# uber-research/UPSNet

Hardware: NVIDIA H100
Metric: panoptic images/sec at 1024x2048 (higher is better)
Workload: dtype bf16x3

## Files before the change

### include/upsnet_b200.h

```cpp
#ifndef UPSNET_B200_H_
#define UPSNET_B200_H_

#include <stddef.h>
#include <stdint.h>

#ifdef __cplusplus
extern "C" {
#endif

#define UPSNET_E_BADARG (-1)
#define UPSNET_E_UNSUPPORTED (-2)
#define UPSNET_E_WORKSPACE (-3)

#define UPSNET_LAYOUT_NCHW 0
#define UPSNET_LAYOUT_NHWC 1
#define UPSNET_LAYOUT_FLAT_PAIR 2

#define UPSNET_DTYPE_F32 0
#define UPSNET_DTYPE_BF16 1
#define UPSNET_DTYPE_PAIR 2

#define UPSNET_EPI_RELU 1
#define UPSNET_EPI_RES_UP2 2
#define UPSNET_EPI_STEM_PAIR 8
#define UPSNET_EPI_NO_TMA 4
#define UPSNET_EPI_PAIR_GROUP(G) ((((G) / 64) & 0xfff) << 8)
#define UPSNET_EPI_SIGMOID_FROM(c) ((((c) + 1) & 0x3ff) << 20)

#define UPSNET_PREC_FP32_SIMT 0
#define UPSNET_PREC_BF16X3 1
#define UPSNET_PREC_BF16 2

int upsnet_version(int *n_sm);

int upsnet_roi_align_forward(const void *feat, int B, int C, int H, int W, int layout, int dtype,
                             const float *rois, int R, int PH, int PW, int sampling_ratio,
                             float spatial_scale, void *out, void *stream);

int upsnet_roi_align_fpn_forward(const void *const feats[4], const int Hs[4], const int Ws[4],
                                 const float scales[4], int B, int C, int layout, int dtype,
                                 const float *rois, int R, int PH, int PW, int sampling_ratio,
                                 void *out, int *levels_out, void *stream);

int upsnet_nms_workspace_bytes(int S, int max_seg_len, size_t *bytes);
int upsnet_nms_segmented(const float *boxes, const int *seg_offsets, int S, int max_seg_len,
                         float thresh, int *keep_out, int *keep_cnt, void *workspace,
                         size_t workspace_bytes, void *stream);
int upsnet_nms_host(int *keep_out, int *num_out, const float *boxes_host, int boxes_num,
                    int boxes_dim, float thresh, int device_id);

int upsnet_dcn_forward(const float *x, const float *offset, const float *mask,
                       const float *weight, const float *bias, float *y, int N, int Cin, int H,
                       int W, int Cout, int kh, int kw, int stride_h, int stride_w, int pad_h,
                       int pad_w, int dil_h, int dil_w, int deformable_groups, int epi_flags,
                       int precision, void *stream);

int upsnet_conv2d_forward(const float *x, const float *weight, const float *bias,
                          const float *residual, float *y, int N, int Cin, int H, int W,
                          int Cout, int kh, int kw, int stride_h, int stride_w, int pad_h,
                          int pad_w, int dil_h, int dil_w, int epi_flags, int precision,
                          void *stream);

int upsnet_igemm_packed_weight_bytes(int Cout, int Cin, int kh, int kw, size_t *bytes);
int upsnet_igemm_pack_weight(const float *weight, int Cout, int Cin, int kh, int kw, void *packed,
                             void *stream);
int upsnet_igemm_forward(const void *x_nhwc, const float *offset, const float *mask,
                         const void *packed, const float *bias, const void *residual, void *y,
                         int N, int H, int W, int Cin, int Cout, int kh, int kw, int stride_h,
                         int stride_w, int pad_h, int pad_w, int dil_h, int dil_w, int out_layout,
                         int x_dtype, int y_dtype, int epi_flags, int precision, void *stream);
int upsnet_tma_set_tile_n(int bn);

int upsnet_dcn_packed_weight_bytes(int Cout, int Cin, int kh, int kw, size_t *bytes);
int upsnet_dcn_pack_weight(const float *weight, int Cout, int Cin, int kh, int kw, void *packed, void *stream);
int upsnet_dcn_pair_forward(const void *x_pair, const float *offset, const float *mask, const void *packed,
                            const float *bias, void *y_pair, int N, int H, int W, int Cin, int Cout, int kh, int kw,
                            int pad_h, int pad_w, int dil_h, int dil_w, int epi_flags, void *stream);
int upsnet_dcn_set_tile_n(int bn);

int upsnet_panoptic_workspace_bytes(int n, int H, int W, int num_thing, size_t *bytes);
int upsnet_panoptic_workspace_min_bytes(int n, int H, int W, int num_thing, size_t *bytes);
int upsnet_panoptic_head(const float *fcn, int S, int H, int W, const float *boxes,
                         const float *cls_prob, const float *mask_logit, const int64_t *cls_idx,
                         int n, const int *n_dev, int num_stuff, double fraction_threshold, int64_t *keep_out,
                         int *k_out, int64_t *labels, int64_t *sem_labels, void *workspace,
                         size_t workspace_bytes, void *stream);
int upsnet_panoptic_head_up4(const float *score, int S, int Hs, int Ws, const float *boxes,
                             const float *cls_prob, const float *mask_logit, const int64_t *cls_idx,
                             int n, const int *n_dev, int num_stuff, double fraction_threshold, int64_t *keep_out,
                             int *k_out, int64_t *labels, int64_t *sem_labels, void *workspace,
                             size_t workspace_bytes, void *stream);

int upsnet_mask_removal(const float *boxes, const float *cls_prob, const float *mask_logit,
                        const int64_t *cls_idx, int n, const int *n_dev, int H, int W, int num_thing,
                        double fraction_threshold, int64_t *keep_out, int *k_out, float *mask_energy,
                        void *workspace, size_t workspace_bytes, void *stream);

int upsnet_stem_workspace_bytes(int N, int H, int W, int kh, int kw, int pad, size_t *bytes);
int upsnet_stem_packed_weight_bytes(int Cout, int kh, size_t *bytes);
int upsnet_stem_pack_weight(const float *weight, int Cout, int Cin, int kh, int kw, void *packed,
                            void *stream);
int upsnet_stem_forward(const float *x, const void *packed_w, const float *bias, void *y, int N, int Cin,
                        int H, int W, int Cout, int kh, int kw, int pad, int epi_flags, void *workspace,
                        size_t workspace_bytes, void *stream);

int upsnet_maxpool2d_nhwc(const void *x, void *y, int N, int H, int W, int C, int k, int stride,
                          int pad, int dtype, void *stream);

int upsnet_upsample_bilinear_nchw(const float *x, float *y, int planes, int H, int W, int factor,
                                  void *stream);

int upsnet_fcn_score_fuse(const float *s2, const float *s3, const float *s4, const float *s5, float *out,
                          int planes, int H, int W, void *stream);

int upsnet_rpn_decode(const float *const *deltas, const long long *const *top_idx, const int *k,
                      const int *hs, const int *ws, const int *strides, const double *base_anchors,
                      int L, int A, float im_h, float im_w, float *boxes_out, void *stream);

int upsnet_rpn_topk_workspace_bytes(int L, size_t *bytes);
int upsnet_rpn_topk(const float *const *probs, const int *hs, const int *ws, int L, int A,
                    int pre_nms_top_n, float *out_scores, long long *out_idx, void *workspace,
                    size_t workspace_bytes, void *stream);

int upsnet_rpn_collect(const int *keep, const int *keep_cnt, const int *seg_offsets, const float *boxes,
                       const float *scores, int S, int max_seg_len, int post_nms_top_n, float *rois,
                       float *out_scores, unsigned char *valid, void *stream);

int upsnet_maskroi_prepare(const float *rois, const unsigned char *roi_valid, const float *bbox_delta,
                           const float *cls_prob, int R, int C, int class_agnostic, float score_thresh,
                           const float weights[4], float im_h, float im_w, float *sc_out, int *cls_out,
                           float *bx_out, int *offs_out, void *stream);

int upsnet_maskroi_finish(const int *keep, const int *keep_cnt, const int *seg_offsets, const float *sc,
                          const int *cls, const float *bx, int nseg, int max_seg_len, int top_n, int cap,
                          float *out_sc, float *out_bx, long long *out_cls, int *n_out, void *stream);

int upsnet_unified_pan_workspace_bytes(int num_seg_classes, size_t *bytes);
int upsnet_unified_pan_result(const long long *seg, const long long *pan, const long long *cls_inds, int k,
                              const int *k_dev, int H, int W, int num_seg_classes, int num_classes,
                              int stuff_area_limit, unsigned char *pan_2ch, int *err_out, void *workspace,
                              size_t workspace_bytes, void *stream);

int upsnet_prep_image(const unsigned char *image_hwc, int h, int w, double scale, int out_h, int out_w, int pad_h,
                      int pad_w, const double pixel_means[3], float *blob, void *stream);

int upsnet_label_restore(const long long *src0, const long long *src1, int Hp, int Wp, int h, int w, double fx,
                         int out_h, int out_w, long long *dst0, long long *dst1, void *stream);

#define UPSNET_PQ_MAX_GT 4096
#define UPSNET_PQ_MAX_PAIRS 65536
#define UPSNET_PQ_MAX_PRED 2048
#define UPSNET_PQ_E_PRED_CATEGORY 1
#define UPSNET_PQ_E_GT_COUNT 2
#define UPSNET_PQ_E_PAIRS 4
#define UPSNET_PQ_E_GT_TABLE 8
#define UPSNET_PQ_E_PRED_COUNT 16
#define UPSNET_PQ_E_MATCHES 32
int upsnet_pq_workspace_bytes(size_t *bytes);
int upsnet_pq_update(const unsigned char *pan_2ch, const unsigned char *gt_rgb, int H, int W, const long long *gt_table,
                     int num_gt, const unsigned char *cat_flags, long long *acc_counts, double *acc_iou, int *err,
                     void *workspace, size_t workspace_bytes, void *stream);

#define UPSNET_SSEG_MAX_CLASSES 224
int upsnet_sseg_update(const void *pred, int pred_bytes, int pred_pitch, const int *row_src, const int *col_src,
                       const unsigned char *gt, int H, int W, int num_classes, long long *acc, void *stream);

#define UPSNET_COCOEVAL_MAX_DET 2048
#define UPSNET_COCOEVAL_MAX_GT 1024
#define UPSNET_COCOEVAL_MAX_GT_CAT 192
#define UPSNET_COCOEVAL_MAX_CATEGORIES 256
#define UPSNET_COCOEVAL_MAX_IMAGES (1 << 17)
#define UPSNET_COCOEVAL_E_DET_COUNT 1
#define UPSNET_COCOEVAL_E_GT_COUNT 2
#define UPSNET_COCOEVAL_E_GT_CAT 4
#define UPSNET_COCOEVAL_E_CLASS 8
#define UPSNET_COCOEVAL_E_RECORDS 16
#define UPSNET_COCOEVAL_E_RLE_SIZE 32
typedef struct {
  float score;
  int category;
  int image;
  int rank;
  unsigned long long matched, ignored;
} upsnet_coco_record;
int upsnet_cocoeval_workspace_bytes(int n, int cap, long long gt_counts_total, size_t *bytes);
int upsnet_cocoeval_image(int segm, const float *boxes, const float *scores, const int64_t *cls_inds, int n,
                          const int *n_dev, const uint32_t *counts, int cap, const int *run_len, int H, int W,
                          const double *gt_table, int num_gt, const uint32_t *gt_counts, const int64_t *gt_offsets,
                          int num_categories, const int *class_to_k, int image_slot, upsnet_coco_record *records,
                          int record_cap, int *n_records, long long *npig, int *err, void *workspace,
                          size_t workspace_bytes, void *stream);
int upsnet_cocoeval_accumulate_workspace_bytes(int n_records, size_t *bytes);
int upsnet_cocoeval_accumulate(const upsnet_coco_record *records, int n_records, const int *image_rank,
                               const long long *npig, int num_categories, double *precision, double *recall,
                               double *scores, void *workspace, size_t workspace_bytes, void *stream);

#define UPSNET_COMBINED_MAX_DET 2048
#define UPSNET_COMBINED_E_RUN_LEN 1
#define UPSNET_COMBINED_E_RLE_SIZE 2
#define UPSNET_COMBINED_E_DET_COUNT 4
int upsnet_combined_pan_workspace_bytes(int n, int H, int W, size_t *bytes);
int upsnet_combined_pan_result(const void *sem, int sem_elem_size, int H, int W, const float *scores,
                               const int64_t *cls_inds, int n, const int *n_dev, const uint32_t *counts, int cap,
                               const int *run_len, int num_seg_classes, int num_classes, float score_threshold,
                               float fraction_threshold, int stuff_area_limit, unsigned char *pan_2ch, int *err,
                               void *workspace, size_t workspace_bytes, void *stream);

int upsnet_im_post_workspace_bytes(int n, int cap, size_t *bytes);
int upsnet_im_post_rle(const float *mask_probs, int C, int M, const float *boxes, const int64_t *cls_inds, int n,
                       const int *n_dev, int H, int W, uint32_t *counts, int cap, int *run_len, int *overflow,
                       void *workspace, size_t workspace_bytes, void *stream);

int upsnet_dcn_im2col(const float *x, const float *offset, const float *mask, int Cin, int H, int W, int kh, int kw,
                      int stride_h, int stride_w, int pad_h, int pad_w, int dil_h, int dil_w, float *col, void *stream);
int upsnet_dcn_col2im(const float *dcol, const float *offset, const float *mask, int Cin, int H, int W, int kh, int kw,
                      int stride_h, int stride_w, int pad_h, int pad_w, int dil_h, int dil_w, float *dx, void *stream);
int upsnet_dcn_col2im_coord(const float *dcol, const float *x, const float *offset, const float *mask, int Cin, int H,
                            int W, int kh, int kw, int stride_h, int stride_w, int pad_h, int pad_w, int dil_h, int dil_w,
                            float *doffset, float *dmask, void *stream);

int upsnet_roi_align_backward(const float *dout, const float *rois, int R, int B, int C, int H, int W, int PH, int PW,
                              int sampling_ratio, float spatial_scale, float *dfeat, void *stream);

#ifdef __cplusplus
}
#endif
#endif
```

### upsnet_b200/_lib.py

```python
import ctypes as C
import os

import torch

_HERE = os.path.dirname(os.path.abspath(__file__))
LIB_PATH = os.path.join(_HERE, "libupsnet_b200.so")
_lib = None

LAYOUT_NCHW, LAYOUT_NHWC = 0, 1
EPI_RELU = 1
EPI_RES_UP2 = 2
EPI_NO_TMA = 4
EPI_STEM_PAIR = 8


def EPI_SIGMOID_FROM(c):
    return ((int(c) + 1) & 0x3ff) << 20
PREC_FP32_SIMT, PREC_BF16X3, PREC_BF16 = 0, 1, 2
DTYPE_F32, DTYPE_BF16, DTYPE_PAIR = 0, 1, 2
LAYOUT_FLAT_PAIR = 2

_ERR = {-1: "bad argument", -2: "unsupported configuration", -3: "workspace too small"}


class UpsnetError(RuntimeError):
    pass


def lib():
    global _lib
    if _lib is None:
        if not os.path.exists(LIB_PATH):
            from . import build as _build
            _build.build()
        L = C.CDLL(LIB_PATH)
        vp, i, f, d, sz = C.c_void_p, C.c_int, C.c_float, C.c_double, C.c_size_t
        L.upsnet_version.argtypes = [C.POINTER(i)]
        L.upsnet_roi_align_forward.argtypes = [vp, i, i, i, i, i, i, vp, i, i, i, i, f, vp, vp]
        L.upsnet_roi_align_fpn_forward.argtypes = [C.POINTER(vp), C.POINTER(i), C.POINTER(i), C.POINTER(f),
                                                   i, i, i, i, vp, i, i, i, i, vp, vp, vp]
        L.upsnet_nms_workspace_bytes.argtypes = [i, i, C.POINTER(sz)]
        L.upsnet_nms_segmented.argtypes = [vp, vp, i, i, f, vp, vp, vp, sz, vp]
        L.upsnet_nms_host.argtypes = [vp, vp, vp, i, i, f, i]
        L.upsnet_dcn_forward.argtypes = [vp] * 6 + [i] * 16 + [vp]
        L.upsnet_conv2d_forward.argtypes = [vp] * 5 + [i] * 15 + [vp]
        L.upsnet_igemm_packed_weight_bytes.argtypes = [i, i, i, i, C.POINTER(sz)]
        L.upsnet_igemm_pack_weight.argtypes = [vp, i, i, i, i, vp, vp]
        L.upsnet_igemm_forward.argtypes = [vp] * 7 + [i] * 18 + [vp]
        L.upsnet_dcn_packed_weight_bytes.argtypes = [i, i, i, i, C.POINTER(sz)]
        L.upsnet_dcn_pack_weight.argtypes = [vp, i, i, i, i, vp, vp]
        L.upsnet_dcn_pair_forward.argtypes = [vp] * 6 + [i] * 12 + [vp]
        L.upsnet_dcn_set_tile_n.argtypes = [i]
        L.upsnet_tma_set_tile_n.argtypes = [i]
        L.upsnet_panoptic_workspace_bytes.argtypes = [i, i, i, i, C.POINTER(sz)]
        L.upsnet_panoptic_workspace_min_bytes.argtypes = [i, i, i, i, C.POINTER(sz)]
        L.upsnet_panoptic_head.argtypes = [vp, i, i, i, vp, vp, vp, vp, i, vp, i, d, vp, vp, vp, vp, vp, sz, vp]
        L.upsnet_panoptic_head_up4.argtypes = [vp, i, i, i, vp, vp, vp, vp, i, vp, i, d, vp, vp, vp, vp, vp, sz, vp]
        L.upsnet_mask_removal.argtypes = [vp, vp, vp, vp, i, vp, i, i, i, d, vp, vp, vp, vp, sz, vp]
        L.upsnet_rpn_decode.argtypes = [C.POINTER(vp), C.POINTER(vp), C.POINTER(i), C.POINTER(i), C.POINTER(i),
                                        C.POINTER(i), vp, i, i, f, f, vp, vp]
        L.upsnet_maskroi_prepare.argtypes = [vp, vp, vp, vp, i, i, i, f, C.POINTER(f), f, f, vp, vp, vp, vp, vp]
        L.upsnet_maskroi_finish.argtypes = [vp] * 6 + [i] * 4 + [vp] * 5
        L.upsnet_maxpool2d_nhwc.argtypes = [vp, vp] + [i] * 8 + [vp]
        L.upsnet_upsample_bilinear_nchw.argtypes = [vp, vp, i, i, i, i, vp]
        L.upsnet_rpn_topk_workspace_bytes.argtypes = [i, C.POINTER(sz)]
        L.upsnet_stem_workspace_bytes.argtypes = [i] * 6 + [C.POINTER(sz)]
        L.upsnet_stem_packed_weight_bytes.argtypes = [i, i, C.POINTER(sz)]
        L.upsnet_stem_pack_weight.argtypes = [vp, i, i, i, i, vp, vp]
        L.upsnet_stem_forward.argtypes = [vp] * 4 + [i] * 9 + [vp, sz, vp]
        L.upsnet_rpn_collect.argtypes = [vp] * 5 + [i] * 3 + [vp] * 4
        L.upsnet_rpn_topk.argtypes = [C.POINTER(vp), C.POINTER(i), C.POINTER(i), i, i, i, vp, vp, vp, sz, vp]
        L.upsnet_dcn_im2col.argtypes = [vp, vp, vp] + [i] * 11 + [vp, vp]
        L.upsnet_dcn_col2im.argtypes = [vp, vp, vp] + [i] * 11 + [vp, vp]
        L.upsnet_dcn_col2im_coord.argtypes = [vp, vp, vp, vp] + [i] * 11 + [vp, vp, vp]
        L.upsnet_roi_align_backward.argtypes = [vp, vp] + [i] * 8 + [f, vp, vp]
        L.upsnet_fcn_score_fuse.argtypes = [vp, vp, vp, vp, vp, i, i, i, vp]
        L.upsnet_unified_pan_workspace_bytes.argtypes = [i, C.POINTER(sz)]
        L.upsnet_unified_pan_result.argtypes = [vp, vp, vp, i, vp, i, i, i, i, i, vp, vp, vp, sz, vp]
        L.upsnet_im_post_workspace_bytes.argtypes = [i, i, C.POINTER(sz)]
        L.upsnet_im_post_rle.argtypes = [vp, i, i, vp, vp, i, vp, i, i, vp, i, vp, vp, vp, sz, vp]
        L.upsnet_prep_image.argtypes = [vp, i, i, d, i, i, i, i, C.POINTER(d), vp, vp]
        L.upsnet_label_restore.argtypes = [vp, vp, i, i, i, i, d, i, i, vp, vp, vp]
        L.upsnet_pq_workspace_bytes.argtypes = [C.POINTER(sz)]
        L.upsnet_pq_update.argtypes = [vp, vp, i, i, vp, i, vp, vp, vp, vp, vp, sz, vp]
        L.upsnet_sseg_update.argtypes = [vp, i, i, vp, vp, vp, i, i, i, vp, vp]
        L.upsnet_cocoeval_workspace_bytes.argtypes = [i, i, C.c_longlong, C.POINTER(sz)]
        L.upsnet_cocoeval_image.argtypes = [i, vp, vp, vp, i, vp, vp, i, vp, i, i, vp, i, vp, vp, i, vp, i, vp, i, vp, vp,
                                            vp, vp, sz, vp]
        L.upsnet_cocoeval_accumulate_workspace_bytes.argtypes = [i, C.POINTER(sz)]
        L.upsnet_cocoeval_accumulate.argtypes = [vp, i, vp, vp, i, vp, vp, vp, vp, sz, vp]
        L.upsnet_combined_pan_workspace_bytes.argtypes = [i, i, i, C.POINTER(sz)]
        L.upsnet_combined_pan_result.argtypes = [vp, i, i, i, vp, vp, i, vp, vp, i, vp, i, i, f, f, i, vp, vp, vp, sz, vp]
        _lib = L
    return _lib


EXPORTED_SYMBOLS = [
    "upsnet_version", "upsnet_roi_align_forward", "upsnet_roi_align_fpn_forward",
    "upsnet_nms_workspace_bytes", "upsnet_nms_segmented", "upsnet_nms_host", "upsnet_dcn_forward",
    "upsnet_conv2d_forward", "upsnet_igemm_packed_weight_bytes", "upsnet_igemm_pack_weight",
    "upsnet_igemm_forward", "upsnet_panoptic_workspace_bytes", "upsnet_panoptic_workspace_min_bytes", "upsnet_panoptic_head", "upsnet_panoptic_head_up4", "upsnet_mask_removal",
    "upsnet_rpn_decode", "upsnet_maskroi_prepare", "upsnet_maskroi_finish", "upsnet_maxpool2d_nhwc", "upsnet_upsample_bilinear_nchw", "upsnet_rpn_topk_workspace_bytes", "upsnet_rpn_topk", "upsnet_rpn_collect", "upsnet_stem_workspace_bytes",
    "upsnet_stem_packed_weight_bytes", "upsnet_stem_pack_weight", "upsnet_stem_forward",
    "upsnet_dcn_im2col", "upsnet_dcn_col2im", "upsnet_dcn_col2im_coord", "upsnet_roi_align_backward",
    "upsnet_dcn_packed_weight_bytes", "upsnet_dcn_pack_weight", "upsnet_dcn_pair_forward", "upsnet_dcn_set_tile_n", "upsnet_tma_set_tile_n",
    "upsnet_fcn_score_fuse", "upsnet_unified_pan_workspace_bytes", "upsnet_unified_pan_result", "upsnet_prep_image", "upsnet_im_post_workspace_bytes", "upsnet_im_post_rle",
    "upsnet_label_restore", "upsnet_pq_workspace_bytes", "upsnet_pq_update",
    "upsnet_sseg_update", "upsnet_cocoeval_workspace_bytes", "upsnet_cocoeval_image",
    "upsnet_cocoeval_accumulate_workspace_bytes", "upsnet_cocoeval_accumulate",
    "upsnet_combined_pan_workspace_bytes", "upsnet_combined_pan_result",
]


def check(rc, what):
    if rc == 0:
        return
    if rc < 0:
        raise UpsnetError("%s: %s (%d)" % (what, _ERR.get(rc, "error"), rc))
    raise UpsnetError("%s: CUDA error %d" % (what, rc))


def stream_ptr(device=None):
    return C.c_void_p(torch.cuda.current_stream(device).cuda_stream)


def ptr(t):
    return C.c_void_p(t.data_ptr()) if t is not None else C.c_void_p(None)


def require_cuda(*tensors):
    for t in tensors:
        if t is not None and not t.is_cuda:
            raise UpsnetError("upsnet_b200 ops are CUDA-only (sm_90a); got a %s tensor" % t.device)


def f32c(t):
    if t.dtype != torch.float32:
        t = t.float()
    return t.contiguous()
```

### upsnet_b200/csrc/capi.cu

```cuda
#include "common.cuh"
#include "tc_params.cuh"

namespace ups {
struct ConvParams {
  const float* x; const float* offset; const float* mask; const float* weight;
  const float* bias; const float* residual; float* y;
  int N, Cin, H, W, Cout, kh, kw, sh, sw, ph, pw, dh, dw, dg, Ho, Wo, relu;
};
int launch_igemm_simt(const ConvParams& p, cudaStream_t stream);

}

extern "C" int upsnet_version(int* n_sm) {
  if (n_sm) {
    int dev = 0, sms = 0;
    if (cudaGetDevice(&dev) == cudaSuccess &&
        cudaDeviceGetAttribute(&sms, cudaDevAttrMultiProcessorCount, dev) == cudaSuccess)
      *n_sm = sms;
    else
      *n_sm = -1;
  }
  return 90;
}

static int conv_common(const float* x, const float* offset, const float* mask, const float* weight,
                       const float* bias, const float* residual, float* y, int N, int Cin, int H,
                       int W, int Cout, int kh, int kw, int sh, int sw, int ph, int pw, int dh,
                       int dw, int dg, int epi_flags, int precision, void* stream) {
  if (!x || !weight || !y) return UPSNET_E_BADARG;
  if (N <= 0 || Cin <= 0 || H <= 0 || W <= 0 || Cout <= 0 || kh <= 0 || kw <= 0 || sh <= 0 ||
      sw <= 0 || ph < 0 || pw < 0 || dh <= 0 || dw <= 0 || dg <= 0 || Cin % dg != 0)
    return UPSNET_E_BADARG;
  ups::ConvParams p;
  p.x = x; p.offset = offset; p.mask = mask; p.weight = weight; p.bias = bias;
  p.residual = residual; p.y = y;
  p.N = N; p.Cin = Cin; p.H = H; p.W = W; p.Cout = Cout; p.kh = kh; p.kw = kw; p.sh = sh;
  p.sw = sw; p.ph = ph; p.pw = pw; p.dh = dh; p.dw = dw; p.dg = dg;
  p.Ho = ups::conv_out_size(H, ph, dh, kh, sh);
  p.Wo = ups::conv_out_size(W, pw, dw, kw, sw);
  p.relu = (epi_flags & UPSNET_EPI_RELU) ? 1 : 0;
  if (p.Ho <= 0 || p.Wo <= 0) return UPSNET_E_BADARG;
  if ((size_t)Cin * H * W >= (1ull << 31)) return UPSNET_E_UNSUPPORTED;
  switch (precision) {
    case UPSNET_PREC_FP32_SIMT:
      return ups::launch_igemm_simt(p, (cudaStream_t)stream);
    default:
      return UPSNET_E_UNSUPPORTED;
  }
}

extern "C" int upsnet_dcn_forward(const float* x, const float* offset, const float* mask,
                                  const float* weight, const float* bias, float* y, int N, int Cin,
                                  int H, int W, int Cout, int kh, int kw, int stride_h,
                                  int stride_w, int pad_h, int pad_w, int dil_h, int dil_w,
                                  int deformable_groups, int epi_flags, int precision,
                                  void* stream) {
  if (!offset) return UPSNET_E_BADARG;
  return conv_common(x, offset, mask, weight, bias, nullptr, y, N, Cin, H, W, Cout, kh, kw,
                     stride_h, stride_w, pad_h, pad_w, dil_h, dil_w, deformable_groups, epi_flags,
                     precision, stream);
}

extern "C" int upsnet_conv2d_forward(const float* x, const float* weight, const float* bias,
                                     const float* residual, float* y, int N, int Cin, int H, int W,
                                     int Cout, int kh, int kw, int stride_h, int stride_w,
                                     int pad_h, int pad_w, int dil_h, int dil_w, int epi_flags,
                                     int precision, void* stream) {
  return conv_common(x, nullptr, nullptr, weight, bias, residual, y, N, Cin, H, W, Cout, kh, kw,
                     stride_h, stride_w, pad_h, pad_w, dil_h, dil_w, 1, epi_flags, precision,
                     stream);
}

extern "C" int upsnet_igemm_packed_weight_bytes(int Cout, int Cin, int kh, int kw, size_t* bytes) {
  if (!bytes || Cout <= 0 || Cin <= 0 || kh <= 0 || kw <= 0) return UPSNET_E_BADARG;
  if (!ups::tc_supported(Cin, kh, kw, 1)) return UPSNET_E_UNSUPPORTED;
  *bytes = ups::tc_packed_weight_bytes(Cout, Cin, kh, kw);
  return 0;
}

extern "C" int upsnet_igemm_pack_weight(const float* weight, int Cout, int Cin, int kh, int kw,
                                        void* packed, void* stream) {
  if (!weight || !packed || Cout <= 0 || Cin <= 0 || kh <= 0 || kw <= 0) return UPSNET_E_BADARG;
  if (!ups::tc_supported(Cin, kh, kw, 1)) return UPSNET_E_UNSUPPORTED;
  return ups::tc_pack_weight(weight, Cout, Cin, kh, kw, packed, (cudaStream_t)stream);
}

extern "C" int upsnet_igemm_forward(const void* x_nhwc, const float* offset, const float* mask,
                                    const void* packed, const float* bias, const void* residual,
                                    void* y, int N, int H, int W, int Cin, int Cout, int kh, int kw,
                                    int stride_h, int stride_w, int pad_h, int pad_w, int dil_h,
                                    int dil_w, int out_layout, int x_dtype, int y_dtype, int epi_flags,
                                    int precision, void* stream) {
  if (!x_nhwc || !packed || !y) return UPSNET_E_BADARG;
  if (N <= 0 || Cin <= 0 || H <= 0 || W <= 0 || Cout <= 0 || kh <= 0 || kw <= 0 || stride_h <= 0 ||
      stride_w <= 0 || pad_h < 0 || pad_w < 0 || dil_h <= 0 || dil_w <= 0)
    return UPSNET_E_BADARG;
  if (precision != UPSNET_PREC_BF16X3 && precision != UPSNET_PREC_BF16) return UPSNET_E_BADARG;
  if (out_layout != UPSNET_LAYOUT_NCHW && out_layout != UPSNET_LAYOUT_NHWC) return UPSNET_E_BADARG;
  if (mask && !offset) return UPSNET_E_BADARG;
  if ((size_t)H * W >= (1ull << 31)) return UPSNET_E_UNSUPPORTED;
  ups::TcParams p{};
  p.x = x_nhwc; p.offset = offset; p.mask = mask; p.bias = bias; p.residual = residual; p.y = y;
  p.N = N; p.H = H; p.W = W; p.Cin = Cin; p.Cout = Cout; p.kh = kh; p.kw = kw; p.sh = stride_h;
  p.sw = stride_w; p.ph = pad_h; p.pw = pad_w; p.dh = dil_h; p.dw = dil_w;
  p.Ho = ups::conv_out_size(H, pad_h, dil_h, kh, stride_h);
  p.Wo = ups::conv_out_size(W, pad_w, dil_w, kw, stride_w);
  if (p.Ho <= 0 || p.Wo <= 0) return UPSNET_E_BADARG;
  p.relu = (epi_flags & UPSNET_EPI_RELU) ? 1 : 0;
  p.out_nhwc = out_layout == UPSNET_LAYOUT_NHWC;
  p.res_up2 = (epi_flags & UPSNET_EPI_RES_UP2) ? 1 : 0;
  p.no_tma = (epi_flags & UPSNET_EPI_NO_TMA) ? 1 : 0;
  if (p.res_up2 && (!residual || !p.out_nhwc || (p.Ho & 1) || (p.Wo & 1))) return UPSNET_E_BADARG;
  p.x3 = precision == UPSNET_PREC_BF16X3;
  if (x_dtype < UPSNET_DTYPE_F32 || x_dtype > UPSNET_DTYPE_PAIR || y_dtype < UPSNET_DTYPE_F32 || y_dtype > UPSNET_DTYPE_PAIR)
    return UPSNET_E_BADARG;
  p.x_bf16 = x_dtype == UPSNET_DTYPE_BF16;
  p.y_bf16 = y_dtype == UPSNET_DTYPE_BF16;
  p.x_pair = x_dtype == UPSNET_DTYPE_PAIR;
  p.y_pair = y_dtype == UPSNET_DTYPE_PAIR;
  p.pair_group = 64 * ((epi_flags >> 8) & 0xfff);
  p.sig_from = ((epi_flags >> 20) & 0x3ff) - 1;
  if (p.sig_from >= 0 && (p.y_pair || p.y_bf16 || p.residual)) return UPSNET_E_UNSUPPORTED;
  if (p.x_bf16 && p.x3) return UPSNET_E_UNSUPPORTED;
  if ((p.x_pair || p.y_pair) && !p.x3) return UPSNET_E_UNSUPPORTED;
  if (p.y_pair && !p.out_nhwc) return UPSNET_E_BADARG;
  return ups::launch_igemm_tc(p, packed, (cudaStream_t)stream);
}
```

### upsnet_b200/csrc/detection.cu

```cuda
#include <cfloat>

#include "common.cuh"

namespace ups {

__device__ __forceinline__ float4 decode_clip(float x1, float y1, float x2, float y2, float dx, float dy, float dw, float dh,
                                              float xform_clip, float im_h, float im_w) {
  const float w = __fadd_rn(__fsub_rn(x2, x1), 1.0f), h = __fadd_rn(__fsub_rn(y2, y1), 1.0f);
  const float cx = __fadd_rn(x1, __fmul_rn(0.5f, w)), cy = __fadd_rn(y1, __fmul_rn(0.5f, h));
  dw = fminf(dw, xform_clip);
  dh = fminf(dh, xform_clip);
  const float pcx = __fadd_rn(__fmul_rn(dx, w), cx), pcy = __fadd_rn(__fmul_rn(dy, h), cy);
  const float pw = __fmul_rn(expf(dw), w), ph = __fmul_rn(expf(dh), h);
  float4 o;
  o.x = __fsub_rn(pcx, __fmul_rn(0.5f, pw));
  o.y = __fsub_rn(pcy, __fmul_rn(0.5f, ph));
  o.z = __fsub_rn(__fadd_rn(pcx, __fmul_rn(0.5f, pw)), 1.0f);
  o.w = __fsub_rn(__fadd_rn(pcy, __fmul_rn(0.5f, ph)), 1.0f);
  const float mx = __fsub_rn(im_w, 1.0f), my = __fsub_rn(im_h, 1.0f);
  o.x = fminf(fmaxf(o.x, 0.f), mx);
  o.y = fminf(fmaxf(o.y, 0.f), my);
  o.z = fminf(fmaxf(o.z, 0.f), mx);
  o.w = fminf(fmaxf(o.w, 0.f), my);
  return o;
// ... 473 lines not shown
    acc += p.lv[l].k;
    if (p.lv[l].blocks > max_blocks) max_blocks = p.lv[l].blocks;
  }
  cudaStream_t st = (cudaStream_t)stream;
  UPS_CUDA(cudaMemsetAsync(p.hist, 0, (size_t)L * kTkBins * 4, st));
  UPS_CUDA(cudaMemsetAsync(p.ticket, 0, (size_t)L * 4 * 4, st));
  const dim3 grid((unsigned)max_blocks, (unsigned)L);
  const int shifts[5] = {43, 32, 22, 11, 0}, nbits[5] = {11, 11, 10, 11, 11};
  for (int ps = 0; ps < 5; ++ps) {
    topk_pass_kernel<<<grid, kTkThreads, 0, st>>>(p, shifts[ps], nbits[ps], ps == 0 ? 1 : 0);
    UPS_CHECK_LAUNCH();
  }
  topk_gather_kernel<<<grid, kTkThreads, 0, st>>>(p);
  UPS_CHECK_LAUNCH();
  topk_sort_kernel<<<L, 1024, 0, st>>>(p);
  UPS_CHECK_LAUNCH();
  return 0;
}

namespace ups {

constexpr int kColMaxCand = 8192, kColMaxPost = 2048, kColBins = 4096;

__global__ void __launch_bounds__(1024, 1)
rpn_collect_kernel(const int* __restrict__ keep, const int* __restrict__ cnt, const int* __restrict__ offs,
                   const float* __restrict__ boxes, const float* __restrict__ scores, int S, int max_len, int post,
                   float* __restrict__ rois, float* __restrict__ out_scores, unsigned char* __restrict__ ok) {
  extern __shared__ unsigned long long ck[];
  unsigned long long* sel = ck + kColMaxCand;
  __shared__ unsigned int hist[kColBins];
  __shared__ int seg_base[kMaxLevels + 1];
  __shared__ unsigned long long s_prefix;
  __shared__ int s_need, s_nsel;
  const int tid = threadIdx.x;
  if (tid == 0) {
    int acc = 0;
    for (int s = 0; s < S; ++s) { seg_base[s] = acc; acc += min(min(max(cnt[s], 0), max_len), post); }
    seg_base[S] = min(acc, kColMaxCand);
    s_nsel = 0;
  }
  __syncthreads();
  const int C = seg_base[S];
  for (int s = 0; s < S; ++s) {
    const int b = seg_base[s], n = min(seg_base[s + 1], kColMaxCand) - b, o = offs[s];
    for (int j = tid; j < n; j += 1024) {
      const int g = keep[(size_t)s * max_len + j] + o;
      ck[b + j] = ((unsigned long long)orderable(scores[g]) << 13) | (unsigned long long)(8191 - (b + j));
    }
  }
  __syncthreads();
  unsigned long long kth = 0ull;
  if (C > post) {
    if (tid == 0) { s_prefix = 0ull; s_need = post; }
    __syncthreads();
    for (int pass = 0; pass < 4; ++pass) {
      const int shift = 36 - 12 * pass;
      const unsigned long long mask_hi = pass == 0 ? 0ull : (~0ull << (shift + 12));
      for (int b = tid; b < kColBins; b += 1024) hist[b] = 0;
      __syncthreads();
      const unsigned long long pref = s_prefix;
      for (int i = tid; i < C; i += 1024)
        if ((ck[i] & mask_hi) == pref) atomicAdd(&hist[(unsigned int)(ck[i] >> shift) & (kColBins - 1)], 1u);
      __syncthreads();
      if (tid < 32) {
        const int need = s_need, per = kColBins / 32;
        unsigned int mine = 0;
        for (int b = 0; b < per; ++b) mine += hist[kColBins - 1 - (tid * per + b)];
        unsigned int incl = mine;
#pragma unroll
        for (int o = 1; o < 32; o <<= 1) {
          const unsigned int y = __shfl_up_sync(0xffffffffu, incl, o);
          if (tid >= o) incl += y;
        }
        const unsigned int excl = incl - mine;
        if (excl < (unsigned int)need && incl >= (unsigned int)need) {
          unsigned int acc = excl;
          int d = 0;
          for (int b = 0; b < per; ++b) {
            const int bin = kColBins - 1 - (tid * per + b);
            if (acc + hist[bin] >= (unsigned int)need) { d = bin; break; }
            acc += hist[bin];
          }
          s_need = need - (int)acc;
          s_prefix = pref | ((unsigned long long)d << shift);
        }
      }
      __syncthreads();
    }
    kth = s_prefix;
  }
  for (int i = tid; i < C; i += 1024)
    if (ck[i] >= kth) {
      const int pos = atomicAdd(&s_nsel, 1);
      if (pos < kColMaxPost) sel[pos] = ck[i];
    }
  __syncthreads();
  const int nsel = min(s_nsel, min(post, kColMaxPost));
  int sortN = 64;
  while (sortN < nsel) sortN <<= 1;
  for (int i = nsel + tid; i < sortN; i += 1024) sel[i] = 0ull;
  __syncthreads();
  for (int k = 2; k <= sortN; k <<= 1)
    for (int j = k >> 1; j > 0; j >>= 1) {
      for (int t = tid; t < sortN / 2; t += 1024) {
        const int lo = ((t / j) * (j << 1)) + (t % j), hi = lo + j;
        const unsigned long long a = sel[lo], b = sel[hi];
        const bool desc = (lo & k) == 0;
        if ((a < b) == desc) { sel[lo] = b; sel[hi] = a; }
      }
      __syncthreads();
    }
  for (int i = tid; i < post; i += 1024) {
    float4 bx = make_float4(0.f, 0.f, 0.f, 0.f);
    float sc = 0.f;
    unsigned char live = 0;
    if (i < nsel) {
      const int fp = 8191 - (int)(sel[i] & 8191ull);
      int s = 0;
      while (s + 1 < S && fp >= seg_base[s + 1]) ++s;
      const int g = keep[(size_t)s * max_len + (fp - seg_base[s])] + offs[s];
      bx = reinterpret_cast<const float4*>(boxes)[g];
      sc = scores[g];
      live = 1;
    }
    rois[(size_t)i * 5] = 0.f;
    rois[(size_t)i * 5 + 1] = bx.x; rois[(size_t)i * 5 + 2] = bx.y;
    rois[(size_t)i * 5 + 3] = bx.z; rois[(size_t)i * 5 + 4] = bx.w;
    out_scores[i] = sc;
    ok[i] = live;
  }
}

}

extern "C" int upsnet_rpn_collect(const int* keep, const int* keep_cnt, const int* seg_offsets, const float* boxes,
                                  const float* scores, int S, int max_seg_len, int post_nms_top_n, float* rois,
                                  float* out_scores, unsigned char* valid, void* stream) {
  using namespace ups;
  if (!keep || !keep_cnt || !seg_offsets || !boxes || !scores || !rois || !out_scores || !valid) return UPSNET_E_BADARG;
  if (S <= 0 || S > kMaxLevels || max_seg_len <= 0 || post_nms_top_n <= 0) return UPSNET_E_BADARG;
  if (post_nms_top_n > kColMaxPost || (long long)S * (max_seg_len < post_nms_top_n ? max_seg_len : post_nms_top_n) > kColMaxCand)
    return UPSNET_E_UNSUPPORTED;
  if (((uintptr_t)boxes) & 15) return UPSNET_E_BADARG;
  const size_t smem = (size_t)(kColMaxCand + kColMaxPost) * 8;
  static ups::PerDeviceOnce configured;
  if (configured.need()) {
    UPS_CUDA(cudaFuncSetAttribute(rpn_collect_kernel, cudaFuncAttributeMaxDynamicSharedMemorySize, (int)smem));
  }
  rpn_collect_kernel<<<1, 1024, smem, (cudaStream_t)stream>>>(keep, keep_cnt, seg_offsets, boxes, scores, S, max_seg_len,
                                                               post_nms_top_n, rois, out_scores, valid);
  UPS_CHECK_LAUNCH();
  return 0;
}
```

### upsnet_b200/csrc/igemm_tma.cu

```cuda
#include <cuda.h>
#include <cuda_bf16.h>
#include <cstdlib>

#include "common.cuh"
#include "tc_ptx.cuh"
#include "tc_params.cuh"

namespace ups {

constexpr int TM_EPI_WARPS = 8;
constexpr int TM_WARP_TMA = 8, TM_WARP_RES = 9;
constexpr int TM_THREADS = 10 * 32;
constexpr int TM_MAX_STAGES = 8;
constexpr int TM_SLAB_BYTES = 128 * 128;
constexpr int TM_MMA_BF16 = 0, TM_MMA_WIDE = 1;

struct TmaGeom {
  const float* bias;
  int N, Ho, Wo, Cout, Cin;
  int kw, KHW, ph, pw, dh, dw;
  int bw, bh, bn;
  int tiles_w, tiles_h, tiles_n, n_tiles;
  int BN, stages, relu, has_res;
  int res_up2;
  int direct, y_bf16, out_nhwc;
  void* y;
  int stem;
  int sig_from;
  int x3;
  int x_lo;
  int w_lo;
  int pg;
  int res_inplace;
  int opairs;
  int wide;
};

__device__ __forceinline__ int pair_chan(int n, int G) { return (n / G) * 2 * G + (n % G); }

struct TmaSmem {
  uint32_t stages, out, res, acc, a_bytes, b_bytes, stage_bytes, total;
  uint32_t a_half, b_half;
  uint32_t oslabs, res_slab;
};
template <int N, int W>
__device__ __forceinline__ void acc_stage_sw(const float (&d)[N / 2], float* buf, int row0) {
  const int t = threadIdx.x & 127, l = t & 31;
  const int r = row0 + 16 * (t >> 5) + (l >> 2);
#pragma unroll
  for (int i = 0; i < W / 8; ++i) {
    const int c = 8 * i + 2 * (l & 3);
#pragma unroll
    for (int h = 0; h < 2; ++h) {
      const int rr = r + 8 * h;
      const int pc = ((((c >> 2) ^ (rr & 7))) << 2) | (c & 3);
      *reinterpret_cast<float2*>(buf + (size_t)rr * W + pc) = make_float2(d[4 * i + 2 * h], d[4 * i + 2 * h + 1]);
    }
  }
}
__device__ __forceinline__ void acc_ld16_sw(uint32_t rowaddr, int row, int col, uint32_t (&r)[16]) {
#pragma unroll
  for (int i = 0; i < 4; ++i) {
    const uint32_t a = rowaddr + ((uint32_t)(((col >> 2) + i) ^ (row & 7)) << 4);
    asm volatile("ld.shared.v4.b32 {%0, %1, %2, %3}, [%4];"
                 : "=r"(r[4 * i]), "=r"(r[4 * i + 1]), "=r"(r[4 * i + 2]), "=r"(r[4 * i + 3]) : "r"(a));
  }
}
__host__ __device__ inline TmaSmem tma_smem_layout(int BN, int stages, bool has_res, bool direct, bool x3, bool res_up2,
                                                  bool res_inplace, int opairs) {
  TmaSmem s;
  const uint32_t mul = x3 ? 2u : 1u;
  s.a_half = 128 * 128; s.b_half = (uint32_t)BN * 128;
  s.a_bytes = s.a_half * mul;
  s.b_bytes = s.b_half * mul;
  s.stage_bytes = s.a_bytes + s.b_bytes;
  s.stages = 1024;
  s.out = s.stages + s.stage_bytes * (uint32_t)stages;
  s.res_slab = (x3 && res_up2) ? 4096u : (uint32_t)TM_SLAB_BYTES;
  if (x3) {
    s.oslabs = direct ? 0u : (res_inplace ? 2u * (uint32_t)(BN / 64) : (uint32_t)opairs);
    s.res = s.out + s.oslabs * 2u * TM_SLAB_BYTES;
    s.acc = s.res + ((has_res && !res_inplace) ? 2u * (uint32_t)(BN / 64) * 2u * s.res_slab : 0u);
  } else {
    s.oslabs = 0;
    const uint32_t out_slabs = direct ? 0 : (BN == 64 ? 1 : 2);
    s.res = s.out + out_slabs * TM_SLAB_BYTES;
    s.acc = s.res + (has_res ? 2u * (uint32_t)(BN / 64) * TM_SLAB_BYTES : 0u);
  }
  s.total = s.acc + ((x3 && !direct) ? 0u : 128u * (uint32_t)BN * 4u);
  return s;
}

template <int N, int MMA>
__global__ void __launch_bounds__(TM_THREADS, 1)
igemm_tma_kernel(const __grid_constant__ CUtensorMap tm_x, const __grid_constant__ CUtensorMap tm_w,
                 const __grid_constant__ CUtensorMap tm_y, const __grid_constant__ CUtensorMap tm_r, const TmaGeom g) {
  extern __shared__ __align__(1024) uint8_t smem_dyn[];
  const uint32_t raw = smem_u32(smem_dyn);
  const uint32_t base = (raw + 1023u) & ~1023u;
  uint8_t* sm = smem_dyn + (base - raw);
  const TmaSmem L = tma_smem_layout(g.BN, g.stages, g.has_res != 0, g.direct != 0, g.x3 != 0, g.res_up2 != 0, g.res_inplace != 0,
                                    g.opairs);
  const uint32_t bar_full = base, bar_empty = base + 8 * TM_MAX_STAGES;
  const uint32_t bar_rfull = bar_empty + 8 * TM_MAX_STAGES, bar_rempty = bar_rfull + 16;

  const int tid = threadIdx.x, warp = tid >> 5, lane = tid & 31;
  const int cchunks = g.Cin / 64;
  const int num_kb = g.KHW * cchunks;
  const long long m_tiles = (long long)g.tiles_w * g.tiles_h * g.tiles_n;
  const long long num_tiles = m_tiles * g.n_tiles;
  const uint32_t box_bytes = (uint32_t)(g.bw * g.bh * g.bn) * 128u;

  if (tid == 0) {
    for (int s = 0; s < g.stages; ++s) {
      mbar_init(bar_full + 8 * s, 1);
      mbar_init(bar_empty + 8 * s, TM_EPI_WARPS);
    }
    for (int b = 0; b < 2; ++b) {
      mbar_init(bar_rfull + 8 * b, 1);
      mbar_init(bar_rempty + 8 * b, g.res_inplace ? 1 : TM_EPI_WARPS);
    }
    fence_mbar_init();
  } else if (warp == TM_WARP_TMA && lane == 0) {
    prefetch_tmap(&tm_x);
    prefetch_tmap(&tm_w);
    prefetch_tmap(&tm_y);
    if (g.has_res || (g.stem && g.x3)) prefetch_tmap(&tm_r);
  }
  __syncthreads();

  if (warp == TM_WARP_TMA) {
    if (lane == 0) {
      uint32_t s = 0, ph = 0;
      uint32_t a_dst = base + L.stages;
      const uint32_t tx_bytes = (g.x3 ? 2u * box_bytes : box_bytes) + L.b_bytes;
      for (long long tile = blockIdx.x; tile < num_tiles; tile += gridDim.x) {
        const int nt = (int)(tile % g.n_tiles);
        const long long mt = tile / g.n_tiles;
        const int w0 = (int)(mt % g.tiles_w) * g.bw;
        const int h0 = (int)((mt / g.tiles_w) % g.tiles_h) * g.bh;
        const int i0 = (int)(mt / ((long long)g.tiles_w * g.tiles_h)) * g.bn;
        const int n0 = nt * g.BN;
        int kbr = 0, cc = 0, kj = 0;
        int cw = w0 - g.pw, ch = h0 - g.ph;
        for (int kb = 0; kb < num_kb; ++kb) {
          const uint32_t bf = bar_full + 8 * s;
          mbar_wait(bar_empty + 8 * s, ph ^ 1u);
          mbar_arrive_expect_tx(bf, tx_bytes);
          if (g.stem)
            tma_load_5d(a_dst, &tm_x, bf, 0, w0, kbr & 1, h0 + (kbr >> 1), i0);
          else
            tma_load_4d(a_dst, &tm_x, bf, cc * 64, cw, ch, i0);
          tma_load_2d(a_dst + L.a_bytes, &tm_w, bf, kbr * 64, n0);
          if (g.x3) {
            if (g.stem)
              tma_load_5d(a_dst + L.a_half, &tm_r, bf, 0, w0, kbr & 1, h0 + (kbr >> 1), i0);
            else
              tma_load_4d(a_dst + L.a_half, &tm_x, bf, g.x_lo + cc * 64, cw, ch, i0);
            tma_load_2d(a_dst + L.a_bytes + L.b_half, &tm_w, bf, kbr * 64, g.w_lo + n0);
          }
          ++kbr;
          if (++cc == cchunks) {
            cc = 0; cw += g.dw;
            if (++kj == g.kw) { kj = 0; cw = w0 - g.pw; ch += g.dh; }
          }
          a_dst += L.stage_bytes;
          if (++s == (uint32_t)g.stages) { s = 0; ph ^= 1u; a_dst = base + L.stages; }
        }
      }
    }
    __syncwarp();
  } else if (warp == TM_WARP_RES) {
    if (lane == 0 && g.has_res) {
      uint32_t ti_local = 0;
      const int slabs = g.BN / 64;
      for (long long tile = blockIdx.x; tile < num_tiles; tile += gridDim.x, ++ti_local) {
        const int nt = (int)(tile % g.n_tiles);
        const long long mt = tile / g.n_tiles;
        const int w0 = (int)(mt % g.tiles_w) * g.bw;
        const int h0 = (int)((mt / g.tiles_w) % g.tiles_h) * g.bh;
        const int i0 = (int)(mt / ((long long)g.tiles_w * g.tiles_h)) * g.bn;
        const uint32_t rb = ti_local & 1u, ruse = ti_local >> 1;
        const uint32_t rdst = base + L.res + rb * (uint32_t)slabs * TM_SLAB_BYTES;
        mbar_wait(bar_rempty + 8 * rb, (ruse & 1u) ^ 1u);
        if (g.x3) {
          const uint32_t lo_off = g.res_inplace ? (uint32_t)TM_SLAB_BYTES : L.res_slab;
          const uint32_t pdst = g.res_inplace ? base + L.out + rb * (uint32_t)slabs * 2u * TM_SLAB_BYTES
                                              : base + L.res + rb * (uint32_t)slabs * 2u * L.res_slab;
          mbar_arrive_expect_tx(bar_rfull + 8 * rb, (g.res_up2 ? box_bytes / 4 : box_bytes) * (uint32_t)slabs * 2u);
          for (int s = 0; s < slabs; ++s) {
            const int c = pair_chan(nt * g.BN + s * 64, g.pg);
            tma_load_4d(pdst + (uint32_t)s * 2u * lo_off, &tm_r, bar_rfull + 8 * rb, c, w0 >> g.res_up2, h0 >> g.res_up2, i0);
            tma_load_4d(pdst + (uint32_t)s * 2u * lo_off + lo_off, &tm_r, bar_rfull + 8 * rb, c + g.pg, w0 >> g.res_up2,
                        h0 >> g.res_up2, i0);
          }
          continue;
        }
        mbar_arrive_expect_tx(bar_rfull + 8 * rb, (g.res_up2 ? box_bytes / 4 : box_bytes) * (uint32_t)slabs);
        for (int s = 0; s < slabs; ++s)
          tma_load_4d(rdst + s * TM_SLAB_BYTES, &tm_r, bar_rfull + 8 * rb, nt * g.BN + s * 64, w0 >> g.res_up2,
                      h0 >> g.res_up2, i0);
      }
    }
    __syncwarp();
  } else {
    const int wg = warp >> 2;
    const uint32_t dhi = wg_desc_hi(1024);
    const uint32_t a_row0 = (uint32_t)wg * 64u * 128u;
    const uint32_t ah16 = L.a_half >> 4;
    float* accbuf = reinterpret_cast<float*>(sm + L.acc);
    constexpr int SW = MMA == TM_MMA_WIDE ? N / 2 : N;
    const bool staged = MMA != TM_MMA_WIDE || g.direct;
    float d[N / 2];
    uint32_t s = 0, ph = 0;
    auto mainloop = [&]() {
      int prev = -1;
      for (int kb = 0; kb < num_kb; ++kb) {
        mbar_wait(bar_full + 8 * s, ph);
        const uint32_t st0 = base + L.stages + s * L.stage_bytes;
        const uint32_t a = wg_desc_lo(st0 + a_row0), b = wg_desc_lo(st0 + L.a_bytes);
        wgmma_fence();
#pragma unroll
        for (uint32_t k = 0; k < 4; ++k) {
          const uint32_t acc = (kb | k) ? 1u : 0u;
          if constexpr (MMA == TM_MMA_WIDE) {
            Wgmma<N>::mma(d, wg_desc(a + 2 * k, dhi), wg_desc(b + 2 * k, dhi), acc);
            Wgmma<N / 2>::mma(*reinterpret_cast<float(*)[N / 4]>(&d[0]), wg_desc(a + ah16 + 2 * k, dhi), wg_desc(b + 2 * k, dhi), 1u);
          } else {
            Wgmma<N>::mma(d, wg_desc(a + 2 * k, dhi), wg_desc(b + 2 * k, dhi), acc);
          }
        }
        wgmma_commit();
        wgmma_wait<1>();
        wgmma_fence_acc(d);
        if (prev >= 0 && lane == 0) mbar_arrive(bar_empty + 8 * prev);
        prev = (int)s;
        if (++s == (uint32_t)g.stages) { s = 0; ph ^= 1u; }
      }
      wgmma_wait<0>();
      wgmma_fence_acc(d);
      if (prev >= 0 && lane == 0) mbar_arrive(bar_empty + 8 * prev);
      if constexpr (MMA == TM_MMA_WIDE) {
#pragma unroll
        for (int i = 0; i < N / 4; ++i) { d[i] += d[N / 4 + i]; d[N / 4 + i] = 0.f; }
      }
      if (staged) {
        named_bar(3, 256);
        acc_stage_sw<N, SW>(d, accbuf, wg * 64);
        named_bar(3, 256);
      }
    };
    const int q = warp & 3, half = warp >> 2;
    const int row = q * 32 + lane;
    const uint32_t trow = smem_u32(accbuf + (size_t)row * SW);
    const int units = g.BN / 32;
    const int upw = units >= 4 ? units / 2 : 1;
    const int bar_id = g.BN == 64 ? 1 : 1 + half;
    const int bar_cnt = g.BN == 64 ? 256 : 128;
    const bool leader = (g.BN == 64 ? warp == 0 : q == 0) && lane == 0;
    const uint32_t out_slab = base + L.out + (g.BN == 64 ? 0u : (uint32_t)half * TM_SLAB_BYTES);
    const uint32_t sw_row = (uint32_t)row * 128u;
    const uint32_t rx = (uint32_t)(row & 7);
// ... 121 lines not shown
          float o[32];
  #pragma unroll
          for (int e = 0; e < 16; ++e) { o[e] = __uint_as_float(v0[e]); o[16 + e] = __uint_as_float(v1[e]); }
          if (g.bias) {
            const float4* bp = reinterpret_cast<const float4*>(g.bias + n0 + u * 32);
  #pragma unroll
            for (int e = 0; e < 8; ++e) {
              const float4 b4 = __ldg(bp + e);
              o[4 * e] += b4.x; o[4 * e + 1] += b4.y; o[4 * e + 2] += b4.z; o[4 * e + 3] += b4.w;
            }
          }
          if (g.has_res) {
            const uint32_t rs = base + L.res + (buf * (uint32_t)(g.BN / 64) + (uint32_t)slab) * TM_SLAB_BYTES + rs_row;
  #pragma unroll
            for (int c = 0; c < 4; ++c) {
              const uint4 rv = lds128(rs + (((jb + c) ^ rrx) << 4));
              const uint32_t rw[4] = {rv.x, rv.y, rv.z, rv.w};
  #pragma unroll
              for (int e = 0; e < 4; ++e) {
                o[c * 8 + 2 * e] += __uint_as_float(rw[e] << 16);
                o[c * 8 + 2 * e + 1] += __uint_as_float(rw[e] & 0xffff0000u);
              }
            }
          }
          if (g.relu) {
  #pragma unroll
            for (int e = 0; e < 32; ++e) o[e] = fmaxf(o[e], 0.f);
          }
  #pragma unroll
          for (int c = 0; c < 4; ++c) {
            uint4 w;
            w.x = pack_bf16x2(o[c * 8], o[c * 8 + 1]); w.y = pack_bf16x2(o[c * 8 + 2], o[c * 8 + 3]);
            w.z = pack_bf16x2(o[c * 8 + 4], o[c * 8 + 5]); w.w = pack_bf16x2(o[c * 8 + 6], o[c * 8 + 7]);
            sts128(out_slab + sw_row + (((jb + c) ^ rx) << 4), w);
          }
          if ((u & 1) == 1 || g.BN == 64) {
            fence_proxy_async();
            named_bar(bar_id, bar_cnt);
            if (leader) {
              tma_store_4d(&tm_y, out_slab, n0 + slab * 64, w0, h0, i0);
              bulk_commit();
            }
          }
        }
        __syncwarp();
        if (lane == 0 && g.has_res) mbar_arrive(bar_rempty + 8 * buf);
      }
    }
    if (leader || (g.x3 && warp == 0 && lane == 0)) bulk_wait0();
  }
}

static bool encode_bf16(EncodeTiledFn enc, CUtensorMap* tm, const void* ptr, int rank, const cuuint64_t* dims,
                        const cuuint32_t* box, const cuuint64_t* byte_strides = nullptr) {
  cuuint64_t strides[5];
  cuuint64_t acc = 2;
  for (int i = 0; i + 1 < rank; ++i) { acc *= dims[i]; strides[i] = byte_strides ? byte_strides[i] : acc; }
  const cuuint32_t es[5] = {1, 1, 1, 1, 1};
  return enc(tm, CU_TENSOR_MAP_DATA_TYPE_BFLOAT16, (cuuint32_t)rank, const_cast<void*>(ptr), dims, strides, box, es,
             CU_TENSOR_MAP_INTERLEAVE_NONE, CU_TENSOR_MAP_SWIZZLE_128B, CU_TENSOR_MAP_L2_PROMOTION_L2_256B,
             CU_TENSOR_MAP_FLOAT_OOB_FILL_NONE) == CUDA_SUCCESS;
}

static void tma_pick_box(int N, int Ho, int Wo, int kh, int kw, int dh, int dw, bool even, int* bw_o, int* bh_o, int* bn_o) {
  long long best_tiles = -1, best_halo = 0;
  int bbw = 1, bbh = 1, bbn = 1;
  const int wmax = Wo < 128 ? Wo : 128;
  for (int bw = 1; bw <= wmax; ++bw) {
    if (Wo > 32 && (bw & (bw - 1))) continue;
    if (even && (bw & 1)) continue;
    const int hmax = (128 / bw) < Ho ? (128 / bw) : Ho;
    for (int bh = 1; bh <= hmax; ++bh) {
      if (even && (bh & 1)) continue;
      int bn = 128 / (bw * bh);
      if (bn > N) bn = N;
      if (bn < 1) continue;
      const long long tiles = (long long)((Wo + bw - 1) / bw) * ((Ho + bh - 1) / bh) * ((N + bn - 1) / bn);
      const long long halo = (long long)(bw + (kw - 1) * dw) * (bh + (kh - 1) * dh) * bn;
      if (best_tiles < 0 || tiles < best_tiles || (tiles == best_tiles && (halo < best_halo || (halo == best_halo && bw > bbw)))) {
        best_tiles = tiles; best_halo = halo; bbw = bw; bbh = bh; bbn = bn;
      }
    }
  }
  *bw_o = bbw; *bh_o = bbh; *bn_o = bbn;
}

template <int N, int MMA>
static int tma_launch_n(dim3 grid, size_t smem, cudaStream_t stream, const CUtensorMap& tm_x, const CUtensorMap& tm_w,
                        const CUtensorMap& tm_y, const CUtensorMap& tm_r, const TmaGeom& g) {
  static ups::PerDeviceOnce configured;
  if (configured.need())
    UPS_CUDA(cudaFuncSetAttribute(igemm_tma_kernel<N, MMA>, cudaFuncAttributeMaxDynamicSharedMemorySize, 227 * 1024));
  igemm_tma_kernel<N, MMA><<<grid, TM_THREADS, smem, stream>>>(tm_x, tm_w, tm_y, tm_r, g);
  UPS_CHECK_LAUNCH();
  return 0;
}
static int tma_launch(int BN, dim3 grid, size_t smem, cudaStream_t stream, const CUtensorMap& tm_x, const CUtensorMap& tm_w,
                      const CUtensorMap& tm_y, const CUtensorMap& tm_r, const TmaGeom& g) {
  if (g.wide) {
    if (BN == 32) return tma_launch_n<64, TM_MMA_WIDE>(grid, smem, stream, tm_x, tm_w, tm_y, tm_r, g);
    if (BN == 64) return tma_launch_n<128, TM_MMA_WIDE>(grid, smem, stream, tm_x, tm_w, tm_y, tm_r, g);
    if (BN == 128) return tma_launch_n<256, TM_MMA_WIDE>(grid, smem, stream, tm_x, tm_w, tm_y, tm_r, g);
  } else {
    if (BN == 32) return tma_launch_n<32, TM_MMA_BF16>(grid, smem, stream, tm_x, tm_w, tm_y, tm_r, g);
    if (BN == 64) return tma_launch_n<64, TM_MMA_BF16>(grid, smem, stream, tm_x, tm_w, tm_y, tm_r, g);
    if (BN == 128) return tma_launch_n<128, TM_MMA_BF16>(grid, smem, stream, tm_x, tm_w, tm_y, tm_r, g);
  }
  return UPSNET_E_UNSUPPORTED;
}

static bool tma_fit(int BN, bool has_res, bool direct, bool pair, bool res_up2, bool res_inplace, int* stages, int* opairs,
                    TmaSmem* L) {
  const uint32_t cap = 227 * 1024 - 1024;
  auto lay = [&](int st, int op) { return tma_smem_layout(BN, st, has_res, direct, pair, res_up2, res_inplace, op); };
  int st = TM_MAX_STAGES, op = 2;
  while (st > 2 && lay(st, op).total > cap) --st;
  if (pair && !direct && !res_inplace && (st < 4 || lay(st, op).total > cap)) {
    int st1 = 4;
    while (st1 > 2 && lay(st1, 1).total > cap) --st1;
    if (st1 > st || lay(st, op).total > cap) { st = st1; op = 1; }
  }
  *stages = st; *opairs = op; *L = lay(st, op);
  return L->total <= cap;
}

static int g_tma_force_bn = 0;

int launch_igemm_tma(const TcParams& p, const void* packed, cudaStream_t stream) {
  if (p.no_tma || p.offset) return UPSNET_E_UNSUPPORTED;
  const bool pair = p.x_pair != 0;
  if (pair != (p.x3 != 0) || (!pair && !p.x_bf16)) return UPSNET_E_UNSUPPORTED;
  if (p.y_pair && (!pair || !p.out_nhwc || (p.Cout % 64) != 0)) return UPSNET_E_UNSUPPORTED;
  if (pair && p.y_bf16) return UPSNET_E_UNSUPPORTED;
  const int pg = p.y_pair ? (p.pair_group > 0 ? p.pair_group : p.Cout) : 0;
  if (p.y_pair && ((pg % 64) != 0 || (p.Cout % pg) != 0)) return UPSNET_E_UNSUPPORTED;
  const bool direct = (!p.y_bf16 && !p.y_pair) || !p.out_nhwc || (p.Cout % 64) != 0;
  if (p.sig_from >= 0 && !direct) return UPSNET_E_UNSUPPORTED;
  if (direct && (p.residual || p.Cout > 256)) return UPSNET_E_UNSUPPORTED;
  if (p.res_up2 && (!p.residual || (p.Ho & 1) || (p.Wo & 1))) return UPSNET_E_UNSUPPORTED;
  const bool strided = p.sh != 1 || p.sw != 1;
  if (strided && (p.kh != 1 || p.kw != 1 || p.ph != 0 || p.pw != 0)) return UPSNET_E_UNSUPPORTED;
  if ((p.Cin % 64) || (!direct && (p.Cout % 64)) || p.kh * p.kw > 49) return UPSNET_E_UNSUPPORTED;
  if ((((uintptr_t)p.x) & 15) || (((uintptr_t)p.y) & 15) || (((uintptr_t)packed) & 15) || (p.residual && (((uintptr_t)p.residual) & 15)))
    return UPSNET_E_UNSUPPORTED;
  if (p.bias && (((uintptr_t)p.bias) & 15)) return UPSNET_E_UNSUPPORTED;
  EncodeTiledFn enc = tma_encoder();
  if (!enc) return UPSNET_E_UNSUPPORTED;
  const int sms = num_sms();
  TmaGeom g{};
  g.bias = p.bias;
  g.N = p.N; g.Ho = p.Ho; g.Wo = p.Wo; g.Cout = p.Cout; g.Cin = p.Cin;
  g.kw = p.kw; g.KHW = p.kh * p.kw; g.ph = p.ph; g.pw = p.pw; g.dh = p.dh; g.dw = p.dw;
  g.relu = p.relu; g.has_res = p.residual ? 1 : 0; g.res_up2 = p.res_up2 ? 1 : 0; g.sig_from = p.sig_from;
  tma_pick_box(p.N, p.Ho, p.Wo, p.kh, p.kw, p.dh, p.dw, g.res_up2 != 0, &g.bw, &g.bh, &g.bn);
  g.tiles_w = (p.Wo + g.bw - 1) / g.bw;
  g.tiles_h = (p.Ho + g.bh - 1) / g.bh;
  g.tiles_n = (p.N + g.bn - 1) / g.bn;
  const long long m_tiles = (long long)g.tiles_w * g.tiles_h * g.tiles_n;
  const int Cout_pad = cout_pad(p.Cout);
  int BN = (Cout_pad % 128 == 0) ? 128 : (Cout_pad % 64 == 0 ? 64 : 32);
  g.x3 = pair ? 1 : 0; g.x_lo = p.Cin; g.w_lo = Cout_pad; g.pg = pg;
  g.res_inplace = (pair && g.has_res && !g.res_up2) ? 1 : 0;
  g.opairs = 2;
  if (g_tma_force_bn && Cout_pad % g_tma_force_bn == 0) {
    BN = g_tma_force_bn;
  } else {
    while (BN > 64 && m_tiles * (Cout_pad / BN) < 88) BN /= 2;
  }
  g.direct = direct ? 1 : 0; g.y_bf16 = p.y_bf16; g.out_nhwc = p.out_nhwc; g.y = p.y;
  TmaSmem L;
  bool ok = tma_fit(BN, g.has_res != 0, direct, pair, g.res_up2 != 0, g.res_inplace != 0, &g.stages, &g.opairs, &L);
  while (BN > 64 && (!ok || (pair && g.stages < 3))) {
    BN /= 2;
    ok = tma_fit(BN, g.has_res != 0, direct, pair, g.res_up2 != 0, g.res_inplace != 0, &g.stages, &g.opairs, &L);
  }
  if (!ok) return UPSNET_E_UNSUPPORTED;
  g.BN = BN;
  g.n_tiles = Cout_pad / BN;

  const int Kp = g.KHW * p.Cin;
  CUtensorMap tm_x, tm_w, tm_y, tm_r;
  {
    const cuuint64_t xm = pair ? 2 : 1;
    const cuuint64_t dx[4] = {(cuuint64_t)p.Cin * xm, (cuuint64_t)(strided ? p.Wo : p.W), (cuuint64_t)(strided ? p.Ho : p.H),
                              (cuuint64_t)p.N};
    const cuuint64_t sx[3] = {(cuuint64_t)p.sw * p.Cin * 2 * xm, (cuuint64_t)p.sh * p.W * p.Cin * 2 * xm,
                              (cuuint64_t)p.H * p.W * p.Cin * 2 * xm};
    const cuuint64_t dy[4] = {(cuuint64_t)p.Cout * xm, (cuuint64_t)p.Wo, (cuuint64_t)p.Ho, (cuuint64_t)p.N};
    const cuuint64_t dwt[2] = {(cuuint64_t)Kp, (cuuint64_t)Cout_pad * xm};
    const cuuint32_t box[4] = {64, (cuuint32_t)g.bw, (cuuint32_t)g.bh, (cuuint32_t)g.bn};
    const cuuint32_t boxw[2] = {64, (cuuint32_t)BN};
    if (!encode_bf16(enc, &tm_x, p.x, 4, dx, box, sx)) return UPSNET_E_UNSUPPORTED;
    if (!encode_bf16(enc, &tm_w, packed, 2, dwt, boxw)) return UPSNET_E_UNSUPPORTED;
    if (direct) {
      tm_y = tm_x;
      tm_r = tm_x;
    } else {
    if (!encode_bf16(enc, &tm_y, p.y, 4, dy, box)) return UPSNET_E_UNSUPPORTED;
    if (g.res_up2) {
      const cuuint64_t dr[4] = {(cuuint64_t)p.Cout * xm, (cuuint64_t)(p.Wo / 2), (cuuint64_t)(p.Ho / 2), (cuuint64_t)p.N};
      const cuuint32_t boxr[4] = {64, (cuuint32_t)(g.bw / 2), (cuuint32_t)(g.bh / 2), (cuuint32_t)g.bn};
      if (!encode_bf16(enc, &tm_r, p.residual, 4, dr, boxr)) return UPSNET_E_UNSUPPORTED;
    } else if (!encode_bf16(enc, &tm_r, p.residual ? p.residual : p.y, 4, dy, box)) {
      return UPSNET_E_UNSUPPORTED;
    }
    }
  }
  const long long num_tiles = m_tiles * g.n_tiles;
  if (num_tiles <= 0) return 0;
  g.wide = pair ? 1 : 0;
  dim3 grid((unsigned)(num_tiles < sms ? num_tiles : sms));
  return tma_launch(BN, grid, L.total + 1024, stream, tm_x, tm_w, tm_y, tm_r, g);
}


__global__ void stem_pack_image_kernel(const float* __restrict__ x, uint4* __restrict__ xp, uint4* __restrict__ xp_lo, int N, int C,
                                       int H, int W, int pad, int Hp, int Wp) {
  const long long total = (long long)N * Hp * Wp;
  for (long long t = (long long)blockIdx.x * blockDim.x + threadIdx.x; t < total; t += (long long)gridDim.x * blockDim.x) {
    const int c = (int)(t % Wp);
    const long long rest = t / Wp;
    const int r = (int)(rest % Hp), n = (int)(rest / Hp);
    const int hi = r - pad, wi = c - pad;
    float v[8] = {0.f, 0.f, 0.f, 0.f, 0.f, 0.f, 0.f, 0.f};
    if (hi >= 0 && hi < H && wi >= 0 && wi < W)
      for (int ch = 0; ch < C; ++ch) v[ch] = __ldg(x + (((size_t)n * C + ch) * H + hi) * W + wi);
    uint4 o;
    o.x = pack_bf16x2(v[0], v[1]); o.y = pack_bf16x2(v[2], v[3]); o.z = pack_bf16x2(v[4], v[5]); o.w = pack_bf16x2(v[6], v[7]);
    xp[t] = o;
    if (xp_lo) {
      uint4 l;
      l.x = pack_bf16x2(v[0] - __uint_as_float(o.x << 16), v[1] - __uint_as_float(o.x & 0xffff0000u));
      l.y = pack_bf16x2(v[2] - __uint_as_float(o.y << 16), v[3] - __uint_as_float(o.y & 0xffff0000u));
      l.z = pack_bf16x2(v[4] - __uint_as_float(o.z << 16), v[5] - __uint_as_float(o.z & 0xffff0000u));
      l.w = pack_bf16x2(v[6] - __uint_as_float(o.w << 16), v[7] - __uint_as_float(o.w & 0xffff0000u));
      xp_lo[t] = l;
    }
  }
}

__global__ void stem_pack_weight_kernel(const float* __restrict__ w, int Cout, int Cin, int kh, int kw,
                                        __nv_bfloat16* __restrict__ packed) {
  const int total = Cout * kh * 64;
  for (int i = blockIdx.x * blockDim.x + threadIdx.x; i < total; i += gridDim.x * blockDim.x) {
    const int c = i & 7, kx = (i >> 3) & 7, ky = (i >> 6) % kh, co = i / (64 * kh);
    const float v = (c < Cin && kx < kw) ? w[(((size_t)co * Cin + c) * kh + ky) * kw + kx] : 0.f;
    const __nv_bfloat16 h = __float2bfloat16_rn(v);
    packed[i] = h;
    packed[total + i] = __float2bfloat16_rn(v - __bfloat162float(h));
  }
}

static void stem_geometry(int H, int W, int kh, int kw, int pad, int* Ho, int* Wo, int* Hp, int* Wp) {
  *Ho = (H + 2 * pad - kh) / 2 + 1;
  *Wo = (W + 2 * pad - kw) / 2 + 1;
  *Hp = 2 * (*Ho + (kh >> 1));
  *Wp = 2 * *Wo + 8;
}

}

extern "C" int upsnet_tma_set_tile_n(int bn) {
  if (bn != 0 && bn != 64 && bn != 128) return UPSNET_E_BADARG;
  ups::g_tma_force_bn = bn;
  return 0;
}

extern "C" int upsnet_stem_workspace_bytes(int N, int H, int W, int kh, int kw, int pad, size_t* bytes) {
  if (!bytes || N <= 0 || H <= 0 || W <= 0 || kh <= 0 || kw <= 0 || kw > 8 || pad < 0) return UPSNET_E_BADARG;
  int Ho, Wo, Hp, Wp;
  ups::stem_geometry(H, W, kh, kw, pad, &Ho, &Wo, &Hp, &Wp);
  if (Ho <= 0 || Wo <= 0) return UPSNET_E_BADARG;
  *bytes = (size_t)N * Hp * Wp * 16 * 2;
  return 0;
}

extern "C" int upsnet_stem_packed_weight_bytes(int Cout, int kh, size_t* bytes) {
  if (!bytes || Cout <= 0 || kh <= 0) return UPSNET_E_BADARG;
  *bytes = (size_t)Cout * kh * 64 * 2 * 2;
  return 0;
}

extern "C" int upsnet_stem_pack_weight(const float* weight, int Cout, int Cin, int kh, int kw, void* packed, void* stream) {
  if (!weight || !packed || Cout <= 0 || Cin <= 0 || Cin > 8 || kh <= 0 || kw <= 0 || kw > 8) return UPSNET_E_BADARG;
  const int total = Cout * kh * 64;
  ups::stem_pack_weight_kernel<<<(total + 255) / 256, 256, 0, (cudaStream_t)stream>>>(weight, Cout, Cin, kh, kw,
                                                                                         (__nv_bfloat16*)packed);
  UPS_CHECK_LAUNCH();
  return 0;
}

extern "C" int upsnet_stem_forward(const float* x, const void* packed_w, const float* bias, void* y, int N, int Cin, int H,
                                   int W, int Cout, int kh, int kw, int pad, int epi_flags, void* workspace,
                                   size_t workspace_bytes, void* stream) {
  using namespace ups;
  if (!x || !packed_w || !y || !workspace) return UPSNET_E_BADARG;
  if (N <= 0 || Cin <= 0 || Cin > 8 || H <= 0 || W <= 0 || kh <= 0 || kw <= 0 || kw > 8 || pad < 0) return UPSNET_E_BADARG;
  if ((Cout % 64) || Cout > 256 || kh > 16) return UPSNET_E_UNSUPPORTED;
  if ((((uintptr_t)y) & 15) || (((uintptr_t)packed_w) & 15) || (((uintptr_t)workspace) & 15)) return UPSNET_E_BADARG;
  if (bias && (((uintptr_t)bias) & 15)) return UPSNET_E_UNSUPPORTED;
  int Ho, Wo, Hp, Wp;
  stem_geometry(H, W, kh, kw, pad, &Ho, &Wo, &Hp, &Wp);
  if (Ho <= 0 || Wo <= 0) return UPSNET_E_BADARG;
  const bool pair = (epi_flags & UPSNET_EPI_STEM_PAIR) != 0;
  const size_t plane_bytes = (size_t)N * Hp * Wp * 16;
  if (workspace_bytes < plane_bytes * (pair ? 2 : 1)) return UPSNET_E_WORKSPACE;
// ... 50 lines not shown
```

### upsnet_b200/csrc/roi_align.cu

```cuda
#include <cuda_bf16.h>

#include "common.cuh"

namespace ups {

struct FpnFeats {
  const void* p[4];
  int H[4], W[4];
  float scale[4];
  int nlevels;
};

__device__ __forceinline__ int fpn_level_of(float x1, float y1, float x2, float y2) {
  const float w = x2 - x1 + 1.f, h = y2 - y1 + 1.f;
  const float x = __fadd_rn(__fdiv_rn(__fsqrt_rn(__fmul_rn(w, h)), 224.f), 1e-6f);
  const float t1 = __uint_as_float(0x3f000000u);
  const float t2 = __uint_as_float(0x3f800000u);
  const float t3 = __uint_as_float(0x3fffffffu);
  return (x >= t1) + (x >= t2) + (x >= t3);
}

struct SamplePos {
  int o00, o01, o10, o11;
  float w00, w01, w10, w11;
// ... 73 lines not shown
  const float* base = reinterpret_cast<const float*>(f.p[lv]) + (size_t)b * H * W * C;
  for (int c = threadIdx.x * VEC; c < C; c += blockDim.x * VEC) {
    for (int pw = 0; pw < PW; ++pw) {
      float acc[VEC];
#pragma unroll
      for (int v = 0; v < VEC; ++v) acc[v] = 0.f;
      for (int iy = 0; iy < gh; ++iy) {
        const float y = rsh + ph * bsh + (float)(iy + .5f) * bsh / (float)gh;
        for (int ix = 0; ix < gw; ++ix) {
          const float x = rsw + pw * bsw + (float)(ix + .5f) * bsw / (float)gw;
          const SamplePos s = roi_sample(H, W, y, x);
          if (VEC == 4) {
            const float4 v00 = __ldg((const float4*)(base + (size_t)s.o00 * C + c));
            const float4 v01 = __ldg((const float4*)(base + (size_t)s.o01 * C + c));
            const float4 v10 = __ldg((const float4*)(base + (size_t)s.o10 * C + c));
            const float4 v11 = __ldg((const float4*)(base + (size_t)s.o11 * C + c));
            acc[0] += (s.w00 * v00.x + s.w01 * v01.x + s.w10 * v10.x + s.w11 * v11.x);
            acc[1 % VEC] += (s.w00 * v00.y + s.w01 * v01.y + s.w10 * v10.y + s.w11 * v11.y);
            acc[2 % VEC] += (s.w00 * v00.z + s.w01 * v01.z + s.w10 * v10.z + s.w11 * v11.z);
            acc[3 % VEC] += (s.w00 * v00.w + s.w01 * v01.w + s.w10 * v10.w + s.w11 * v11.w);
          } else {
            acc[0] += (s.w00 * __ldg(base + (size_t)s.o00 * C + c) +
                       s.w01 * __ldg(base + (size_t)s.o01 * C + c) +
                       s.w10 * __ldg(base + (size_t)s.o10 * C + c) +
                       s.w11 * __ldg(base + (size_t)s.o11 * C + c));
          }
        }
      }
      float* o = out + (((size_t)n * PH + ph) * PW + pw) * C + c;
      if (VEC == 4) {
        float4 v;
        v.x = acc[0] / inv_count_div; v.y = acc[1 % VEC] / inv_count_div;
        v.z = acc[2 % VEC] / inv_count_div; v.w = acc[3 % VEC] / inv_count_div;
        *(float4*)o = v;
      } else {
        o[0] = acc[0] / inv_count_div;
      }
    }
  }
}

__global__ void __launch_bounds__(256)
roi_align_nhwc_bf16_kernel(FpnFeats f, int C, const float* __restrict__ rois, int R, int PH, int PW, int sr,
                           __nv_bfloat16* __restrict__ out, int* __restrict__ levels_out) {
  const int n = blockIdx.x / PH, ph = blockIdx.x % PH;
  const float* r = rois + (size_t)n * 5;
  const int b = (int)roundf(r[0]);
  const float rx1 = r[1], ry1 = r[2], rx2 = r[3], ry2 = r[4];
  const int lv = f.nlevels > 1 ? fpn_level_of(rx1, ry1, rx2, ry2) : 0;
  if (levels_out && ph == 0 && threadIdx.x == 0) levels_out[n] = lv;
  const int H = f.H[lv], W = f.W[lv];
  const float sc = f.scale[lv];
  const float rsw = rx1 * sc, rsh = ry1 * sc, rew = rx2 * sc, reh = ry2 * sc;
  const float rw = fmaxf(rew - rsw, 1.f), rh = fmaxf(reh - rsh, 1.f);
  const float bsh = rh / (float)PH, bsw = rw / (float)PW;
  const int gh = sr > 0 ? sr : (int)ceilf(rh / PH), gw = sr > 0 ? sr : (int)ceilf(rw / PW);
  const float cnt = (float)(gh * gw);
  const __nv_bfloat16* base = reinterpret_cast<const __nv_bfloat16*>(f.p[lv]) + (size_t)b * H * W * C;
  for (int c = threadIdx.x * 4; c < C; c += blockDim.x * 4) {
    for (int pw = 0; pw < PW; ++pw) {
      float acc[4] = {0.f, 0.f, 0.f, 0.f};
      for (int iy = 0; iy < gh; ++iy) {
        const float y = rsh + ph * bsh + (float)(iy + .5f) * bsh / (float)gh;
        for (int ix = 0; ix < gw; ++ix) {
          const float x = rsw + pw * bsw + (float)(ix + .5f) * bsw / (float)gw;
          const SamplePos s = roi_sample(H, W, y, x);
          const uint2 v00 = __ldg(reinterpret_cast<const uint2*>(base + (size_t)s.o00 * C + c));
          const uint2 v01 = __ldg(reinterpret_cast<const uint2*>(base + (size_t)s.o01 * C + c));
          const uint2 v10 = __ldg(reinterpret_cast<const uint2*>(base + (size_t)s.o10 * C + c));
          const uint2 v11 = __ldg(reinterpret_cast<const uint2*>(base + (size_t)s.o11 * C + c));
          const uint32_t a[2] = {v00.x, v00.y}, bq[2] = {v01.x, v01.y}, d[2] = {v10.x, v10.y}, e[2] = {v11.x, v11.y};
#pragma unroll
          for (int q = 0; q < 2; ++q) {
            acc[2 * q] += (s.w00 * __uint_as_float(a[q] << 16) + s.w01 * __uint_as_float(bq[q] << 16) +
                           s.w10 * __uint_as_float(d[q] << 16) + s.w11 * __uint_as_float(e[q] << 16));
            acc[2 * q + 1] += (s.w00 * __uint_as_float(a[q] & 0xffff0000u) + s.w01 * __uint_as_float(bq[q] & 0xffff0000u) +
                               s.w10 * __uint_as_float(d[q] & 0xffff0000u) + s.w11 * __uint_as_float(e[q] & 0xffff0000u));
          }
        }
      }
      __nv_bfloat162 o0 = __floats2bfloat162_rn(acc[0] / cnt, acc[1] / cnt), o1 = __floats2bfloat162_rn(acc[2] / cnt, acc[3] / cnt);
      uint2 w;
      w.x = *reinterpret_cast<uint32_t*>(&o0); w.y = *reinterpret_cast<uint32_t*>(&o1);
      *reinterpret_cast<uint2*>(out + (((size_t)n * PH + ph) * PW + pw) * C + c) = w;
    }
  }
}

constexpr int kRoiMaxSamples = 1024;
__global__ void __launch_bounds__(256)
roi_align_nhwc_bf16_roi_kernel(FpnFeats f, int C, const float* __restrict__ rois, int R, int PH, int PW, int sr,
                               __nv_bfloat16* __restrict__ out, int* __restrict__ levels_out) {
  __shared__ int4 s_off[kRoiMaxSamples];
  __shared__ float4 s_w[kRoiMaxSamples];
  const int n = blockIdx.x;
  const float* r = rois + (size_t)n * 5;
  const int b = (int)roundf(r[0]);
  const float rx1 = r[1], ry1 = r[2], rx2 = r[3], ry2 = r[4];
  const int lv = f.nlevels > 1 ? fpn_level_of(rx1, ry1, rx2, ry2) : 0;
  if (levels_out && threadIdx.x == 0) levels_out[n] = lv;
  const int H = f.H[lv], W = f.W[lv];
  const float sc = f.scale[lv];
  const float rsw = rx1 * sc, rsh = ry1 * sc, rew = rx2 * sc, reh = ry2 * sc;
  const float rw = fmaxf(rew - rsw, 1.f), rh = fmaxf(reh - rsh, 1.f);
  const float bsh = rh / (float)PH, bsw = rw / (float)PW;
  const int gh = sr, gw = sr;
  const float cnt = (float)(gh * gw);
  const int per_bin = gh * gw, nsamp = PH * PW * per_bin;
  for (int t = threadIdx.x; t < nsamp; t += blockDim.x) {
    const int bin = t / per_bin, q = t - bin * per_bin;
    const int ph = bin / PW, pw = bin - ph * PW, iy = q / gw, ix = q - iy * gw;
    const float y = rsh + ph * bsh + (float)(iy + .5f) * bsh / (float)gh;
    const float x = rsw + pw * bsw + (float)(ix + .5f) * bsw / (float)gw;
    const SamplePos sp = roi_sample(H, W, y, x);
    s_off[t] = make_int4(sp.o00 * C, sp.o01 * C, sp.o10 * C, sp.o11 * C);
    s_w[t] = make_float4(sp.w00, sp.w01, sp.w10, sp.w11);
  }
  __syncthreads();
  const __nv_bfloat16* base = reinterpret_cast<const __nv_bfloat16*>(f.p[lv]) + (size_t)b * H * W * C;
  const int warp = threadIdx.x >> 5, lane = threadIdx.x & 31, nwarp = blockDim.x >> 5;
  for (int bin = warp; bin < PH * PW; bin += nwarp) {
    for (int c = lane * 8; c < C; c += 256) {
      float acc[8] = {0.f, 0.f, 0.f, 0.f, 0.f, 0.f, 0.f, 0.f};
      for (int q = 0; q < per_bin; ++q) {
        const int4 o = s_off[bin * per_bin + q];
        const float4 w = s_w[bin * per_bin + q];
        const uint4 v00 = __ldg(reinterpret_cast<const uint4*>(base + o.x + c));
        const uint4 v01 = __ldg(reinterpret_cast<const uint4*>(base + o.y + c));
        const uint4 v10 = __ldg(reinterpret_cast<const uint4*>(base + o.z + c));
        const uint4 v11 = __ldg(reinterpret_cast<const uint4*>(base + o.w + c));
        const uint32_t a[4] = {v00.x, v00.y, v00.z, v00.w}, bq[4] = {v01.x, v01.y, v01.z, v01.w};
        const uint32_t d[4] = {v10.x, v10.y, v10.z, v10.w}, e[4] = {v11.x, v11.y, v11.z, v11.w};
#pragma unroll
        for (int k = 0; k < 4; ++k) {
          acc[2 * k] += (w.x * __uint_as_float(a[k] << 16) + w.y * __uint_as_float(bq[k] << 16) +
                         w.z * __uint_as_float(d[k] << 16) + w.w * __uint_as_float(e[k] << 16));
          acc[2 * k + 1] += (w.x * __uint_as_float(a[k] & 0xffff0000u) + w.y * __uint_as_float(bq[k] & 0xffff0000u) +
                             w.z * __uint_as_float(d[k] & 0xffff0000u) + w.w * __uint_as_float(e[k] & 0xffff0000u));
        }
      }
      uint4 wv;
      __nv_bfloat162 o0 = __floats2bfloat162_rn(acc[0] / cnt, acc[1] / cnt), o1 = __floats2bfloat162_rn(acc[2] / cnt, acc[3] / cnt);
      __nv_bfloat162 o2 = __floats2bfloat162_rn(acc[4] / cnt, acc[5] / cnt), o3 = __floats2bfloat162_rn(acc[6] / cnt, acc[7] / cnt);
      wv.x = *reinterpret_cast<uint32_t*>(&o0); wv.y = *reinterpret_cast<uint32_t*>(&o1);
      wv.z = *reinterpret_cast<uint32_t*>(&o2); wv.w = *reinterpret_cast<uint32_t*>(&o3);
      *reinterpret_cast<uint4*>(out + ((size_t)n * PH * PW + bin) * C + c) = wv;
    }
  }
}

__global__ void __launch_bounds__(256)
roi_align_nhwc_pair_roi_kernel(FpnFeats f, int C, const float* __restrict__ rois, int R, int PH, int PW, int sr,
                               __nv_bfloat16* __restrict__ out, long long roi_stride, int pix_stride, long long lo_off,
                               int* __restrict__ levels_out) {
  __shared__ int4 s_off[kRoiMaxSamples];
  __shared__ float4 s_w[kRoiMaxSamples];
  const int n = blockIdx.x;
  const float* r = rois + (size_t)n * 5;
  const int b = (int)roundf(r[0]);
  const float rx1 = r[1], ry1 = r[2], rx2 = r[3], ry2 = r[4];
  const int lv = f.nlevels > 1 ? fpn_level_of(rx1, ry1, rx2, ry2) : 0;
  if (levels_out && threadIdx.x == 0) levels_out[n] = lv;
  const int H = f.H[lv], W = f.W[lv];
  const float sc = f.scale[lv];
  const float rsw = rx1 * sc, rsh = ry1 * sc, rew = rx2 * sc, reh = ry2 * sc;
  const float rw = fmaxf(rew - rsw, 1.f), rh = fmaxf(reh - rsh, 1.f);
  const float bsh = rh / (float)PH, bsw = rw / (float)PW;
  const int gh = sr, gw = sr;
  const float cnt = (float)(gh * gw);
  const int per_bin = gh * gw, nsamp = PH * PW * per_bin;
  for (int t = threadIdx.x; t < nsamp; t += blockDim.x) {
    const int bin = t / per_bin, q = t - bin * per_bin;
    const int ph = bin / PW, pw = bin - ph * PW, iy = q / gw, ix = q - iy * gw;
    const float y = rsh + ph * bsh + (float)(iy + .5f) * bsh / (float)gh;
    const float x = rsw + pw * bsw + (float)(ix + .5f) * bsw / (float)gw;
    const SamplePos sp = roi_sample(H, W, y, x);
    s_off[t] = make_int4(sp.o00 * 2 * C, sp.o01 * 2 * C, sp.o10 * 2 * C, sp.o11 * 2 * C);
    s_w[t] = make_float4(sp.w00, sp.w01, sp.w10, sp.w11);
  }
  __syncthreads();
  const __nv_bfloat16* base = reinterpret_cast<const __nv_bfloat16*>(f.p[lv]) + (size_t)b * H * W * 2 * C;
  const int warp = threadIdx.x >> 5, lane = threadIdx.x & 31, nwarp = blockDim.x >> 5;
  for (int bin = warp; bin < PH * PW; bin += nwarp) {
    for (int c = lane * 8; c < C; c += 256) {
      float acc[8] = {0.f, 0.f, 0.f, 0.f, 0.f, 0.f, 0.f, 0.f};
      for (int q = 0; q < per_bin; ++q) {
        const int4 o = s_off[bin * per_bin + q];
        const float4 w = s_w[bin * per_bin + q];
        const __nv_bfloat16* p0 = base + o.x + c; const __nv_bfloat16* p1 = base + o.y + c;
        const __nv_bfloat16* p2 = base + o.z + c; const __nv_bfloat16* p3 = base + o.w + c;
        const uint4 h0 = __ldg(reinterpret_cast<const uint4*>(p0)), l0 = __ldg(reinterpret_cast<const uint4*>(p0 + C));
        const uint4 h1 = __ldg(reinterpret_cast<const uint4*>(p1)), l1 = __ldg(reinterpret_cast<const uint4*>(p1 + C));
        const uint4 h2 = __ldg(reinterpret_cast<const uint4*>(p2)), l2 = __ldg(reinterpret_cast<const uint4*>(p2 + C));
        const uint4 h3 = __ldg(reinterpret_cast<const uint4*>(p3)), l3 = __ldg(reinterpret_cast<const uint4*>(p3 + C));
        const uint32_t A[4] = {h0.x, h0.y, h0.z, h0.w}, a[4] = {l0.x, l0.y, l0.z, l0.w};
        const uint32_t B[4] = {h1.x, h1.y, h1.z, h1.w}, bq[4] = {l1.x, l1.y, l1.z, l1.w};
        const uint32_t D[4] = {h2.x, h2.y, h2.z, h2.w}, d[4] = {l2.x, l2.y, l2.z, l2.w};
        const uint32_t E[4] = {h3.x, h3.y, h3.z, h3.w}, e[4] = {l3.x, l3.y, l3.z, l3.w};
#pragma unroll
        for (int k = 0; k < 4; ++k) {
          acc[2 * k] += (w.x * (__uint_as_float(A[k] << 16) + __uint_as_float(a[k] << 16)) +
                         w.y * (__uint_as_float(B[k] << 16) + __uint_as_float(bq[k] << 16)) +
                         w.z * (__uint_as_float(D[k] << 16) + __uint_as_float(d[k] << 16)) +
                         w.w * (__uint_as_float(E[k] << 16) + __uint_as_float(e[k] << 16)));
          acc[2 * k + 1] += (w.x * (__uint_as_float(A[k] & 0xffff0000u) + __uint_as_float(a[k] & 0xffff0000u)) +
                             w.y * (__uint_as_float(B[k] & 0xffff0000u) + __uint_as_float(bq[k] & 0xffff0000u)) +
                             w.z * (__uint_as_float(D[k] & 0xffff0000u) + __uint_as_float(d[k] & 0xffff0000u)) +
                             w.w * (__uint_as_float(E[k] & 0xffff0000u) + __uint_as_float(e[k] & 0xffff0000u)));
        }
      }
      uint32_t hw[4], lw[4];
#pragma unroll
      for (int k = 0; k < 4; ++k) {
        const float u = acc[2 * k] / cnt, v = acc[2 * k + 1] / cnt;
        __nv_bfloat162 hh = __floats2bfloat162_rn(u, v);
        hw[k] = *reinterpret_cast<uint32_t*>(&hh);
        __nv_bfloat162 ll = __floats2bfloat162_rn(u - __uint_as_float(hw[k] << 16), v - __uint_as_float(hw[k] & 0xffff0000u));
        lw[k] = *reinterpret_cast<uint32_t*>(&ll);
      }
      __nv_bfloat16* op = out + (size_t)n * roi_stride + (size_t)bin * pix_stride + c;
      *reinterpret_cast<uint4*>(op) = make_uint4(hw[0], hw[1], hw[2], hw[3]);
      *reinterpret_cast<uint4*>(op + lo_off) = make_uint4(lw[0], lw[1], lw[2], lw[3]);
    }
  }
}

static int launch_roi_align(const FpnFeats& f, int B, int C, int layout, int dtype, const float* rois, int R,
                            int PH, int PW, int sr, void* out_v, int* levels_out,
                            cudaStream_t stream) {
  if (R < 0 || C <= 0 || PH <= 0 || PW <= 0 || B <= 0) return UPSNET_E_BADARG;
  if (R == 0) return 0;
  if (dtype == UPSNET_DTYPE_PAIR) {
    if (layout != UPSNET_LAYOUT_NHWC && layout != UPSNET_LAYOUT_FLAT_PAIR) return UPSNET_E_UNSUPPORTED;
    if (sr <= 0 || (C & 7) || (long long)PH * PW * sr * sr > kRoiMaxSamples || (((uintptr_t)out_v) & 15)) return UPSNET_E_UNSUPPORTED;
    for (int l = 0; l < f.nlevels; ++l)
      if ((((uintptr_t)f.p[l]) & 15) || (long long)f.H[l] * f.W[l] * 2 * C >= (1ll << 31)) return UPSNET_E_UNSUPPORTED;
    const long long plane = (long long)PH * PW * C;
    const bool flat = layout == UPSNET_LAYOUT_FLAT_PAIR;
    roi_align_nhwc_pair_roi_kernel<<<R, 256, 0, stream>>>(f, C, rois, R, PH, PW, sr, (__nv_bfloat16*)out_v, 2 * plane,
                                                          flat ? C : 2 * C, flat ? plane : (long long)C, levels_out);
    UPS_CHECK_LAUNCH();
    return 0;
  }
  if (dtype == UPSNET_DTYPE_BF16) {
    if (layout != UPSNET_LAYOUT_NHWC || (C & 3)) return UPSNET_E_UNSUPPORTED;
    for (int l = 0; l < f.nlevels; ++l) if (((uintptr_t)f.p[l]) & 7) return UPSNET_E_BADARG;
    if (((uintptr_t)out_v) & 7) return UPSNET_E_BADARG;
    bool wide = sr > 0 && (C & 7) == 0 && (long long)PH * PW * sr * sr <= kRoiMaxSamples && (((uintptr_t)out_v) & 15) == 0;
    for (int l = 0; l < f.nlevels; ++l) wide = wide && (((uintptr_t)f.p[l]) & 15) == 0 && (long long)f.H[l] * f.W[l] * C < (1ll << 31);
    if (wide) {
      roi_align_nhwc_bf16_roi_kernel<<<R, 256, 0, stream>>>(f, C, rois, R, PH, PW, sr, (__nv_bfloat16*)out_v, levels_out);
      UPS_CHECK_LAUNCH();
      return 0;
    }
    const int threads = C / 4 < 32 ? 32 : (C / 4 > 256 ? 256 : (C / 4 + 31) / 32 * 32);
    roi_align_nhwc_bf16_kernel<<<R * PH, threads, 0, stream>>>(f, C, rois, R, PH, PW, sr, (__nv_bfloat16*)out_v, levels_out);
    UPS_CHECK_LAUNCH();
    return 0;
  }
  if (dtype != UPSNET_DTYPE_F32) return UPSNET_E_BADARG;
  float* out = reinterpret_cast<float*>(out_v);
  if (layout == UPSNET_LAYOUT_NCHW) {
    const long long total = (long long)R * C * PH * PW;
    long long blocks = (total + 255) / 256;
    if (blocks > kNumSMs * 64) blocks = kNumSMs * 64;
    roi_align_nchw_kernel<<<(int)blocks, 256, 0, stream>>>(f, C, rois, R, PH, PW, sr, out,
                                                           levels_out);
  } else if (layout == UPSNET_LAYOUT_NHWC) {
    bool vec4 = (C % 4 == 0);
    for (int l = 0; l < f.nlevels; ++l) vec4 = vec4 && (((uintptr_t)f.p[l] & 15) == 0);
    vec4 = vec4 && (((uintptr_t)out & 15) == 0);
    if (vec4) {
      int threads = C / 4 < 32 ? 32 : (C / 4 > 256 ? 256 : (C / 4 + 31) / 32 * 32);
      roi_align_nhwc_kernel<4><<<R * PH, threads, 0, stream>>>(f, C, rois, R, PH, PW, sr, out,
                                                              levels_out);
    } else {
      int threads = C < 32 ? 32 : (C > 256 ? 256 : (C + 31) / 32 * 32);
      roi_align_nhwc_kernel<1><<<R * PH, threads, 0, stream>>>(f, C, rois, R, PH, PW, sr, out,
                                                              levels_out);
    }
  } else {
    return UPSNET_E_BADARG;
  }
  UPS_CHECK_LAUNCH();
  return 0;
}

}

extern "C" int upsnet_roi_align_forward(const void* feat, int B, int C, int H, int W, int layout, int dtype,
                                        const float* rois, int R, int PH, int PW,
                                        int sampling_ratio, float spatial_scale, void* out,
                                        void* stream) {
  if (!feat || !out || (!rois && R > 0)) return UPSNET_E_BADARG;
  ups::FpnFeats f{};
  f.p[0] = feat; f.H[0] = H; f.W[0] = W; f.scale[0] = spatial_scale; f.nlevels = 1;
  return ups::launch_roi_align(f, B, C, layout, dtype, rois, R, PH, PW, sampling_ratio, out, nullptr,
                               (cudaStream_t)stream);
}

extern "C" int upsnet_roi_align_fpn_forward(const void* const feats[4], const int Hs[4],
                                            const int Ws[4], const float scales[4], int B, int C,
                                            int layout, int dtype, const float* rois, int R, int PH, int PW,
                                            int sampling_ratio, void* out, int* levels_out,
                                            void* stream) {
  if (!feats || !Hs || !Ws || !scales || !out || (!rois && R > 0)) return UPSNET_E_BADARG;
  ups::FpnFeats f{};
  for (int l = 0; l < 4; ++l) {
    if (!feats[l]) return UPSNET_E_BADARG;
    f.p[l] = feats[l]; f.H[l] = Hs[l]; f.W[l] = Ws[l]; f.scale[l] = scales[l];
  }
  f.nlevels = 4;
  return ups::launch_roi_align(f, B, C, layout, dtype, rois, R, PH, PW, sampling_ratio, out, levels_out,
                               (cudaStream_t)stream);
}
```

### upsnet_b200/csrc/tc_params.cuh

```cuda
#pragma once
#include <cuda.h>
#include <cuda_runtime.h>
#include <cstdint>

namespace ups {

inline int cout_pad(int Cout) { return Cout <= 32 ? 32 : (Cout + 63) / 64 * 64; }

typedef CUresult (*EncodeTiledFn)(CUtensorMap*, CUtensorMapDataType, cuuint32_t, void*, const cuuint64_t*, const cuuint64_t*,
                                  const cuuint32_t*, const cuuint32_t*, CUtensorMapInterleave, CUtensorMapSwizzle,
                                  CUtensorMapL2promotion, CUtensorMapFloatOOBfill);

inline EncodeTiledFn tma_encoder() {
  static EncodeTiledFn fn = nullptr;
  static bool tried = false;
  if (!tried) {
    void* p = nullptr;
    cudaDriverEntryPointQueryResult qr = cudaDriverEntryPointSymbolNotFound;
    if (cudaGetDriverEntryPoint("cuTensorMapEncodeTiled", &p, cudaEnableDefault, &qr) == cudaSuccess &&
        qr == cudaDriverEntryPointSuccess)
      fn = reinterpret_cast<EncodeTiledFn>(p);
    else
      (void)cudaGetLastError();
    tried = true;
  }
  return fn;
}

struct TcParams {
  const void* x;
  const float* offset;
  const float* mask;
  const uint16_t* w_hi;
  const uint16_t* w_lo;
  const float* bias; const void* residual; void* y;
  int N, H, W, Cin, Cout, Cout_pad, kh, kw, sh, sw, ph, pw, dh, dw, Ho, Wo;
  int relu, out_nhwc, BN, stages, x3;
  int x_bf16, y_bf16;
  int x_pair, y_pair;
  int sig_from;
  int pair_group;
  int res_up2;
  int no_tma;
  int tile_w, tile_h;
};

size_t tc_packed_weight_bytes(int Cout, int Cin, int kh, int kw);
int tc_pack_weight(const float* w, int Cout, int Cin, int kh, int kw, void* packed, cudaStream_t stream);
bool tc_supported(int Cin, int kh, int kw, int dg);
int launch_igemm_tc(TcParams p, const void* packed, cudaStream_t stream);
int launch_igemm_tma(const TcParams& p, const void* packed, cudaStream_t stream);

}
```

### upsnet_b200/model.py

```python
import math

import numpy as np
import torch
import torch.nn as nn
import torch.nn.functional as F

from . import operators as ops
from .detection import MaskROI, ProposalGenerator, StaticMaskROI, StaticProposalGenerator
from .operators import DeformConv, DeformConvWithOffset


class UPSNetConfig:

    def __init__(self, **kw):
        self.num_classes = 9
        self.num_seg_classes = 19
        self.backbone_with_dconv = 100
        self.backbone_with_dilation = False
        self.backbone_with_dpyramid = False
        self.fpn_feature_dim = 256
        self.fpn_with_gap = False
        self.fcn_num_layers = 2
        self.num_anchors = 3
        self.anchor_scales = (8,)
# ... 139 lines not shown

    def __init__(self, blocks, cfg):
        super().__init__()
        d = cfg.backbone_with_dconv
        self.conv1 = Stem()
        self.res2 = ResBlock(64, blocks[0])
        self.res3 = ResBlock(128, blocks[1], 2, deformable=d <= 3, with_dpyramid=cfg.backbone_with_dpyramid)
        self.res4 = ResBlock(256, blocks[2], 2, deformable=d <= 4, with_dpyramid=cfg.backbone_with_dpyramid)
        s5, d5 = (1, 2) if cfg.backbone_with_dilation else (2, 1)
        self.res5 = ResBlock(512, blocks[3], s5, d5, deformable=d <= 5)

    def forward(self, x):
        c1 = self.conv1(x)
        r2 = self.res2(c1)
        r3 = self.res3(r2)
        r4 = self.res4(r3)
        return r2, r3, r4, self.res5(r4)


class FPN(nn.Module):

    def __init__(self, feature_dim, with_gap):
        super().__init__()
        self.feature_dim = feature_dim
        if with_gap:
            self.fpn_gap = nn.Linear(2048, feature_dim)
        for name, cin in (("fpn_p5_1x1", 2048), ("fpn_p4_1x1", 1024), ("fpn_p3_1x1", 512), ("fpn_p2_1x1", 256)):
            setattr(self, name, nn.Conv2d(cin, feature_dim, 1))
        for name in ("fpn_p5", "fpn_p4", "fpn_p3", "fpn_p2"):
            setattr(self, name, nn.Conv2d(feature_dim, feature_dim, 3, padding=1))
        for m in self.modules():
            if isinstance(m, nn.Conv2d):
                nn.init.kaiming_uniform_(m.weight.data, a=1)
                m.bias.data.zero_()

    @staticmethod
    def _c(m, x, residual=None, padding=0, up2=False):
        return ops.conv2d(x, m.weight, m.bias, padding=padding, residual=residual, residual_up2=up2)

    def forward(self, res2, res3, res4, res5):
        p5_1x1 = self._c(self.fpn_p5_1x1, res5)
        if hasattr(self, "fpn_gap"):
            gap = ops.linear(res5.float().mean(dim=(2, 3)), self.fpn_gap.weight, self.fpn_gap.bias, out_dtype=torch.float32)
            if isinstance(p5_1x1, ops.Pair):
                p5_1x1 = ops.Pair.from_float(p5_1x1.float() + gap.view(-1, self.feature_dim, 1, 1))
            else:
                p5_1x1 = p5_1x1 + gap.view(-1, self.feature_dim, 1, 1).to(p5_1x1.dtype)
        p4_plus = self._c(self.fpn_p4_1x1, res4, residual=p5_1x1, up2=True)
        p3_plus = self._c(self.fpn_p3_1x1, res3, residual=p4_plus, up2=True)
        p2_plus = self._c(self.fpn_p2_1x1, res2, residual=p3_plus, up2=True)
        p5 = self._c(self.fpn_p5, p5_1x1, padding=1)
        p4 = self._c(self.fpn_p4, p4_plus, padding=1)
        p3 = self._c(self.fpn_p3, p3_plus, padding=1)
        p2 = self._c(self.fpn_p2, p2_plus, padding=1)
        p6 = ops.subsample2(p5)
        return p2, p3, p4, p5, p6


class RPN(nn.Module):

    def __init__(self, num_anchors, input_dim):
        super().__init__()
        self.num_anchors = num_anchors
        self.conv_proposal = nn.Sequential(nn.Conv2d(input_dim, input_dim, 3, padding=1), nn.ReLU(inplace=True))
        self.cls_score = nn.Conv2d(input_dim, num_anchors, 1)
        self.bbox_pred = nn.Conv2d(input_dim, num_anchors * 4, 1)
        for m in (self.conv_proposal[0], self.cls_score, self.bbox_pred):
            nn.init.normal_(m.weight.data, 0, 0.01)
            m.bias.data.zero_()
        self._f = None

    def prepare(self):
        self._f = (torch.cat([self.cls_score.weight, self.bbox_pred.weight, self.cls_score.weight]).detach().contiguous(),
                   torch.cat([self.cls_score.bias, self.bbox_pred.bias, self.cls_score.bias]).detach().contiguous())

    def forward(self, x):
        c = self.conv_proposal[0]
        t = ops.conv2d(x, c.weight, c.bias, padding=1, relu=True)
        A = self.num_anchors
        both = ops.conv2d(t, self._f[0], self._f[1], out_format="nchw", sigmoid_from=5 * A).float()
        return both[:, :A], both[:, A:5 * A], both[:, 5 * A:]


class RCNN(nn.Module):

    def __init__(self, num_classes, num_reg_classes, pool_size=7, dim_in=256, dim_hidden=1024):
        super().__init__()
        self.pool_size = pool_size
        self.roi_pooling = ops.FPNRoIAlign(pool_size, pool_size, [1.0 / 4, 1.0 / 8, 1.0 / 16, 1.0 / 32])
        self.fc6 = nn.Sequential(nn.Linear(pool_size ** 2 * dim_in, dim_hidden), nn.ReLU(inplace=True))
        self.fc7 = nn.Sequential(nn.Linear(dim_hidden, dim_hidden), nn.ReLU(inplace=True))
        self.cls_score = nn.Linear(dim_hidden, num_classes)
        self.bbox_pred = nn.Linear(dim_hidden, num_reg_classes * 4)
        for m in (self.fc6[0], self.fc7[0]):
            nn.init.kaiming_uniform_(m.weight.data, a=1)
            m.bias.data.fill_(0)
        nn.init.normal_(self.cls_score.weight.data, 0, 0.01)
        self.cls_score.bias.data.fill_(0)
        nn.init.normal_(self.bbox_pred.weight.data, 0, 0.001)
        self.bbox_pred.bias.data.fill_(0)
        self.num_classes = num_classes
        self._f = None

    def prepare(self):
        self._f = (torch.cat([self.cls_score.weight, self.bbox_pred.weight]).detach().contiguous(),
                   torch.cat([self.cls_score.bias, self.bbox_pred.bias]).detach().contiguous())
        w6 = self.fc6[0].weight.detach()
        ps = self.pool_size
        self._w6_nhwc = w6.view(w6.shape[0], -1, ps, ps).permute(0, 2, 3, 1).reshape(w6.shape[0], -1).contiguous()

    def forward(self, feat, rois):
        if isinstance(feat[0], ops.Pair):
            ps = self.pool_size
            pool = ops.fpn_roi_align(list(feat), rois, ps, ps, self.roi_pooling.spatial_scale, layout="flat_pair")
            fc6 = ops.linear(pool, self._w6_nhwc, self.fc6[0].bias, relu=True)
            fc7 = ops.linear(fc6, self.fc7[0].weight, self.fc7[0].bias, relu=True)
            both = ops.linear(fc7, self._f[0], self._f[1], out_dtype=torch.float32).float()
            return {"cls_score": both[:, :self.num_classes].contiguous(),
                    "bbox_pred": both[:, self.num_classes:].contiguous(), "fc_feat": fc7}
        pool = self.roi_pooling(feat, rois)
        nhwc = pool.permute(0, 2, 3, 1)
        if self._f is not None and nhwc.is_contiguous() and not pool.is_contiguous():
            fc6 = ops.linear(nhwc.reshape(pool.size(0), -1), self._w6_nhwc, self.fc6[0].bias, relu=True)
        else:
            fc6 = ops.linear(pool.reshape(pool.size(0), -1), self.fc6[0].weight, self.fc6[0].bias, relu=True)
        fc7 = ops.linear(fc6, self.fc7[0].weight, self.fc7[0].bias, relu=True)
        both = ops.linear(fc7, self._f[0], self._f[1], out_dtype=torch.float32).float()
        return {"cls_score": both[:, :self.num_classes].contiguous(),
                "bbox_pred": both[:, self.num_classes:].contiguous(), "fc_feat": fc7}


class MaskBranch(nn.Module):

    def __init__(self, num_classes, mask_size=28, dim_in=256, dim_hidden=256):
        super().__init__()
        self.roi_pooling = ops.FPNRoIAlign(mask_size // 2, mask_size // 2, [1.0 / 4, 1.0 / 8, 1.0 / 16, 1.0 / 32])
        for i, cin in enumerate((dim_in, dim_hidden, dim_hidden, dim_hidden), start=1):
            setattr(self, "mask_conv%d" % i, nn.Sequential(nn.Conv2d(cin, dim_hidden, 3, 1, 1), nn.ReLU(inplace=True)))
        self.mask_deconv1 = nn.Sequential(nn.ConvTranspose2d(dim_hidden, dim_hidden, 2, 2, 0), nn.ReLU(inplace=True))
        self.mask_score = nn.Conv2d(dim_hidden, num_classes, 1)
        for m in self.modules():
            if isinstance(m, (nn.Conv2d, nn.ConvTranspose2d)):
                nn.init.kaiming_normal_(m.weight.data, mode="fan_in")
                m.bias.data.zero_()
        self._f = None

    def prepare(self):
        w = self.mask_deconv1[0].weight
        cin, cout = w.shape[0], w.shape[1]
        w1 = w.permute(2, 3, 1, 0).reshape(4 * cout, cin, 1, 1).detach().contiguous()
        b1 = self.mask_deconv1[0].bias.repeat(4).detach().contiguous()
        self._f = (w1, b1, cout)

    def forward(self, feat, rois):
        x = self.roi_pooling(feat, rois)
        for i in range(1, 5):
            c = getattr(self, "mask_conv%d" % i)[0]
            x = ops.conv2d(x, c.weight, c.bias, padding=1, relu=True)
        w1, b1, cout = self._f
        if isinstance(x, ops.Pair):
            yv = ops.conv2d(x, w1, b1, relu=True, pair_group=cout)
            n, _, h, w4 = yv.shape
            w = w4 // 4
            z = ops.conv2d(yv, self.mask_score.weight, self.mask_score.bias, out_format="nhwc", out_dtype=torch.float32)
            K = z.shape[1]
            z = z.permute(0, 2, 3, 1).reshape(n, h, w, 2, 2, K)
            return z.permute(0, 5, 1, 3, 2, 4).reshape(n, K, 2 * h, 2 * w)
        y = ops.conv2d(x, w1, b1, relu=True)
        n, _, h, w = y.shape
        if y.is_contiguous(memory_format=torch.channels_last) and y.dim() == 4:
            yv = y.permute(0, 2, 3, 1).reshape(n, h, w * 4, cout).permute(0, 3, 1, 2)
            z = ops.conv2d(yv, self.mask_score.weight, self.mask_score.bias, out_format="nhwc",
                           out_dtype=torch.float32)
            K = z.shape[1]
            z = z.permute(0, 2, 3, 1).reshape(n, h, w, 2, 2, K)
            return z.permute(0, 5, 1, 3, 2, 4).reshape(n, K, 2 * h, 2 * w)
        y = y.reshape(n, 2, 2, cout, h, w).permute(0, 3, 4, 1, 5, 2).reshape(n, cout, 2 * h, 2 * w)
        return ops.conv2d(y, self.mask_score.weight, self.mask_score.bias, out_format="nchw")


class FCNSubNet(nn.Module):

    def __init__(self, in_channels, out_channels, num_layers):
        super().__init__()
        assert num_layers >= 2
        self.num_layers = num_layers
        self.conv = nn.ModuleList()
        for i in range(num_layers):
            if i == num_layers - 2:
                layer = DeformConvWithOffset(in_channels, out_channels, 3, stride=1, padding=1, dilation=1)
                in_channels = out_channels
            else:
                layer = DeformConvWithOffset(in_channels, in_channels, 3, stride=1, padding=1, dilation=1)
            self.conv.append(nn.Sequential(layer, nn.ReLU(inplace=True)))
        for m in self.modules():
            if isinstance(m, nn.Conv2d):
                m.weight.data.fill_(0)
                m.bias.data.fill_(0)
            elif isinstance(m, DeformConv):
                nn.init.kaiming_normal_(m.weight.data)
                if m.bias is not None:
                    m.bias.data.fill_(0)

    def forward(self, x):
        for i in range(self.num_layers):
            l = self.conv[i][0]
            offset = ops.conv2d(x, l.conv_offset.weight, l.conv_offset.bias, 1, 1, 1, out_format="nchw")
            x = ops.deform_conv(x, offset, l.conv.weight, l.conv.bias, l.conv.stride, l.conv.padding,
                                l.conv.dilation, l.conv.deformable_groups, relu=True)
        return x


class FCNHead(nn.Module):

    def __init__(self, in_channels, num_classes, num_layers, upsample_rate=4):
        super().__init__()
        self.fcn_subnet = FCNSubNet(in_channels, 128, num_layers)
        self.upsample_rate = upsample_rate
        self.score = nn.Conv2d(512, num_classes, 1)
        nn.init.normal_(self.score.weight.data, 0, 0.01)
        self.score.bias.data.zero_()
        self.overlap_levels = False
        self._streams = None
        self._f = None

    def prepare(self):
        w = self.score.weight.detach()
        self._f = [w[:, 128 * l:128 * (l + 1)].contiguous() for l in range(4)]

    def _subnets(self, p2, p3, p4, p5):
        if not (p2.is_cuda and self.overlap_levels):
            return tuple(self.fcn_subnet(p) for p in (p2, p3, p4, p5))
        cur = torch.cuda.current_stream(p2.device)
        if self._streams is None:
            self._streams = [torch.cuda.Stream(device=p2.device) for _ in range(2)]
        fork = torch.cuda.Event()
        fork.record(cur)
        outs, joins = {}, []
        for st, (name, p) in zip(self._streams, (("p4", p4), ("p5", p5))):
            st.wait_event(fork)
            with torch.cuda.stream(st):
                outs[name] = self.fcn_subnet(p)
                ev = torch.cuda.Event()
                ev.record(st)
            joins.append(ev)
            if not torch.cuda.is_current_stream_capturing():
                outs[name].record_stream(cur)
        o2 = self.fcn_subnet(p2)
        o3 = self.fcn_subnet(p3)
        for ev in joins:
            cur.wait_event(ev)
        return o2, o3, outs["p4"], outs["p5"]

    def forward(self, p2, p3, p4, p5, score_only=False):
        p2, p3, p4, p5 = self._subnets(p2, p3, p4, p5)
        if self._f is not None:
            score = ops.conv2d(p2, self._f[0], self.score.bias, out_format="nchw").float()
            parts = [ops.conv2d(feat, self._f[l], None, out_format="nchw").float() for l, feat in enumerate((p3, p4, p5), start=1)]
            if score.is_cuda and score.shape[2] % 8 == 0 and score.shape[3] % 8 == 0 and \
                    all(tuple(s_.shape[2:]) == (score.shape[2] >> l, score.shape[3] >> l) for l, s_ in enumerate(parts, start=1)):
                score = ops.fcn_score_fuse(score, *parts)
            else:
                for l, s_l in enumerate(parts, start=1):
                    score = score + F.interpolate(s_l, None, 2 ** l, mode="bilinear", align_corners=False)
            ret = {"fcn_score": score}
            if self.upsample_rate != 1 and not (score_only and self.upsample_rate == 4):
                ret["fcn_output"] = ops.upsample_bilinear(score, self.upsample_rate)
            return ret
        p3 = F.interpolate(p3, None, 2, mode="bilinear", align_corners=False)
        p4 = F.interpolate(p4, None, 4, mode="bilinear", align_corners=False)
        p5 = F.interpolate(p5, None, 8, mode="bilinear", align_corners=False)
        feat = torch.cat([p2, p3, p4, p5], dim=1)
        score = ops.conv2d(feat, self.score.weight, self.score.bias, out_format="nchw")
        ret = {"fcn_score": score, "fcn_feat": feat}
        if self.upsample_rate != 1:
            ret["fcn_output"] = F.interpolate(score, None, self.upsample_rate, mode="bilinear", align_corners=False)
        return ret


class resnet_upsnet(nn.Module):

    def __init__(self, backbone_depth, cfg=None):
        super().__init__()
        cfg = cfg or UPSNetConfig()
        self.cfg = cfg
        self.num_classes, self.num_seg_classes = cfg.num_classes, cfg.num_seg_classes
        self.num_reg_classes = cfg.num_classes
        self.resnet_backbone = ResNetBackbone(backbone_depth, cfg)
        self.fpn = FPN(cfg.fpn_feature_dim, cfg.fpn_with_gap)
        self.rpn = RPN(cfg.num_anchors, cfg.fpn_feature_dim)
        self.rcnn = RCNN(self.num_classes, self.num_reg_classes, dim_in=cfg.fpn_feature_dim)
        self.mask_branch = MaskBranch(self.num_classes, cfg.mask_size, dim_in=cfg.fpn_feature_dim)
        self.fcn_head = FCNHead(cfg.fpn_feature_dim, self.num_seg_classes, cfg.fcn_num_layers)
        self.enable_void = cfg.panoptic_box_keep_fraction < 1
        assert self.enable_void, "all shipped configs enable the void channel"
        self.pyramid_proposal = ProposalGenerator(cfg.rpn_feat_stride, cfg.anchor_scales, cfg.anchor_ratios,
                                                  cfg.rpn_pre_nms_top_n, cfg.rpn_post_nms_top_n,
                                                  cfg.rpn_nms_thresh, cfg.rpn_min_size)
        self.mask_roi = MaskROI(cfg.max_det, self.num_classes, cfg.nms_thresh, False, cfg.score_thresh,
                                cfg.bbox_reg_weights)
        self.mask_roi_panoptic = MaskROI(cfg.max_det, self.num_classes, 0.5, True, cfg.panoptic_score_thresh,
                                         cfg.bbox_reg_weights)
        self.panoptic_head = ops.PanopticHead(self.num_seg_classes, self.num_classes, 0.3)
        self.pyramid_proposal_static = StaticProposalGenerator(cfg.rpn_feat_stride, cfg.anchor_scales,
                                                               cfg.anchor_ratios, cfg.rpn_pre_nms_top_n,
                                                               cfg.rpn_post_nms_top_n, cfg.rpn_nms_thresh,
                                                               cfg.rpn_min_size)
        self.mask_roi_static = StaticMaskROI(cfg.max_det, self.num_classes, cfg.nms_thresh, False, cfg.score_thresh,
                                             cfg.bbox_reg_weights)
        self.mask_roi_panoptic_static = StaticMaskROI(cfg.max_det, self.num_classes, 0.5, True,
                                                      cfg.panoptic_score_thresh, cfg.bbox_reg_weights)
        self.static_engine = True
        self.use_cuda_graph = True
        self.overlap_heads = True
        self._side = {}
        self._graphs = {}
        self.max_graphs = 6
        self._prepared = False
        self.eval()

    def prepare(self):
        for m in self.modules():
            if m is not self and hasattr(m, "prepare"):
                m.prepare()
        self._prepared = True
        return self

    def _apply(self, fn, *a, **kw):
        r = super()._apply(fn, *a, **kw)
        self._prepared = False
        self._graphs = {}
        return r

    _COCO2CITY_THING = {0: 0, 1: 1, 2: -1, 3: 3, 4: 8, 5: 6, 6: 7, 7: 4, 8: 2}
    _COCO2CITY_SEG = {0: 20, 1: 43, 2: 49, 3: 51, 4: 37, 5: -1, 6: 62, 7: -1, 8: 36, 9: -1, 10: 39, 11: 53, 12: -1, 13: 55,
                      14: 60, 15: 58, 16: 59, 17: 56, 18: 54}

    @staticmethod
    def name_mapping(name, resume=False):
        if resume:
            return name[len("module."):] if name.startswith("module.") else name
        if name.startswith("conv1") or name.startswith("bn1"):
            return "resnet_backbone.conv1." + name
        return name.replace("layer1", "resnet_backbone.res2.layers").replace("layer2", "resnet_backbone.res3.layers") \
                   .replace("layer3", "resnet_backbone.res4.layers").replace("layer4", "resnet_backbone.res5.layers")

    def load_state_dict(self, state_dict, strict=True, resume=None, **kw):
        if resume is None:
            r = super().load_state_dict(state_dict, strict=strict, **kw)
        else:
            r = self._load_reference_style(dict(state_dict), bool(resume))
        self._prepared = False
        self._graphs = {}
        return r

    def _load_reference_style(self, state_dict, resume):
        import warnings
        own = self.state_dict()
        k = "rcnn.cls_score.weight"
        if k in state_dict and own[k].shape[0] == 9 and state_dict[k].shape[0] == 81:
            for wn in ("rcnn.cls_score.weight", "rcnn.cls_score.bias", "rcnn.bbox_pred.weight", "rcnn.bbox_pred.bias",
                       "mask_branch.mask_score.weight", "mask_branch.mask_score.bias"):
                src = state_dict[wn].float()
                mean, std = src.mean().item(), src.std().item()
                src = src.view(*([81, -1] + list(src.shape[1:])))
                blobs = (np.random.randn(*([9] + list(src.shape[1:]))) * std + mean).astype(np.float32)
                for i in range(9):
                    c = self._COCO2CITY_THING[i]
                    if c >= 0:
                        blobs[i] = src[c].cpu().numpy()
                state_dict[wn] = torch.from_numpy(blobs.reshape([-1] + list(src.shape[2:])))
        k = "fcn_head.score.weight"
        if k in own and k in state_dict and own[k].shape[0] == 19 and state_dict[k].shape[0] == 133:
            for wn in ("fcn_head.score.weight", "fcn_head.score.bias"):
                src = state_dict[wn].float()
                mean, std = src.mean().item(), src.std().item()
                blobs = (np.random.randn(*([19] + list(src.shape[1:]))) * std + mean).astype(np.float32)
                for i in range(19):
                    c = self._COCO2CITY_SEG[i]
                    if c >= 0:
                        blobs[i] = src[c].cpu().numpy()
                state_dict[wn] = torch.from_numpy(blobs)
        seen = set()
        with torch.no_grad():
            for name, param in state_dict.items():
                name = self.name_mapping(name, resume)
                seen.add(name)
                if name not in own:
                    warnings.warn('unexpected key "{}" in state_dict'.format(name))
                    continue
                if own[name].shape == param.shape:
                    own[name].copy_(param)
                else:
                    warnings.warn("While copying the parameter named {}, whose dimensions in the models are {} and whose "
                                  "dimensions in the checkpoint are {}, ...".format(name, own[name].size(), param.size()))
        missing = set(own.keys()) - seen
        if missing:
            warnings.warn('missing keys in state_dict: "{}"'.format(missing))
        return None

    def _forward_static(self, x, im_info):
        res2, res3, res4, res5 = self.resnet_backbone(x)
        p2, p3, p4, p5, p6 = self.fpn(res2, res3, res4, res5)
        rpn_cls_prob, rpn_bbox_pred = [], []
        for feat in (p2, p3, p4, p5, p6):
            _, bbox, prob = self.rpn(feat)
            rpn_cls_prob.append(prob)
            rpn_bbox_pred.append(bbox)
        fork = x.is_cuda and self.overlap_heads
        if fork:
            cur = torch.cuda.current_stream(x.device)
            side = self._side_stream(x.device)
            ev = torch.cuda.Event()
            ev.record(cur)
            side.wait_event(ev)
            with torch.cuda.stream(side):
                fcn_output, fcn_score = self._semantic(p2, p3, p4, p5, x.is_cuda)
                done = torch.cuda.Event()
                done.record(side)
            if not torch.cuda.is_current_stream_capturing():
                for t_ in (fcn_output, fcn_score):
                    if t_ is not None:
                        t_.record_stream(cur)
        rois, _, roi_valid = self.pyramid_proposal_static(rpn_cls_prob, rpn_bbox_pred, im_info)
        if not fork:
            fcn_output, fcn_score = self._semantic(p2, p3, p4, p5, x.is_cuda)
        feats = [p2, p3, p4, p5]
        rcnn_output = self.rcnn(feats, rois)
        cls_prob = F.softmax(rcnn_output["cls_score"].float(), dim=1)
        bbox_pred = rcnn_output["bbox_pred"].float()
        if fork:
            side2 = self._side_stream(x.device, 1)
            ev2 = torch.cuda.Event()
            ev2.record(cur)
            side2.wait_event(ev2)
            with torch.cuda.stream(side2):
                s2, b2, c2, n2 = self.mask_roi_panoptic_static(rois, roi_valid, bbox_pred, cls_prob, im_info, side=True)
                done2 = torch.cuda.Event()
                done2.record(side2)
            if not torch.cuda.is_current_stream_capturing():
                for t_ in (s2, b2, c2, n2, self.mask_roi_panoptic_static.last_flags):
                    t_.record_stream(cur)
        s1, b1, c1, n1 = self.mask_roi_static(rois, roi_valid, bbox_pred, cls_prob, im_info)
        if fork:
            cur.wait_event(done2)
        else:
            s2, b2, c2, n2 = self.mask_roi_panoptic_static(rois, roi_valid, bbox_pred, cls_prob, im_info)
        logits = self.mask_branch(feats, torch.cat([b1, b2], 0)).float()
        mask_prob = torch.sigmoid(logits[:b1.shape[0]])
        ms = self.cfg.mask_size
        mask_score = logits[b1.shape[0]:].gather(1, c2.view(-1, 1, 1, 1).expand(-1, -1, ms, ms))
        if fork:
            cur.wait_event(done)
        keep, labels, sem, k = ops.panoptic_fuse(fcn_score if fcn_score is not None else fcn_output, b2[:, 1:], s2, mask_score, c2,
                                                 self.panoptic_head.num_stuff, self.panoptic_head.fraction_threshold,
                                                 want_sem=True, n_dev=n2.reshape(1), up4=fcn_score is not None)
        counts = torch.cat([n1.reshape(1).to(torch.int32), n2.reshape(1).to(torch.int32), k.reshape(1)])
        trunc = torch.stack([self.mask_roi_static.last_flags.reshape(()).to(torch.int32),
                             self.mask_roi_panoptic_static.last_flags.reshape(()).to(torch.int32)])
        out = {"cls_probs": s1, "pred_boxes": b1, "mask_probs": mask_prob, "cls_inds": c1, "fcn_outputs": sem,
               "panoptic_outputs": labels, "p_scores": s2, "p_cls": c2, "p_boxes": b2, "p_mask_score": mask_score,
               "keep": keep, "counts": counts, "trunc_flags": trunc, "fcn_output": fcn_output}
        if getattr(self, "keep_intermediates", False):
            out["dbg"] = {"fpn": [f.float().contiguous() for f in (p2, p3, p4, p5, p6)],
                          "rpn_cls_prob": [t_.float() for t_ in rpn_cls_prob], "rpn_bbox_pred": [t_.float() for t_ in rpn_bbox_pred],
                          "rois": rois, "roi_valid": roi_valid, "cls_score": rcnn_output["cls_score"].float(),
                          "bbox_pred": bbox_pred, "mask_logits": logits}
        return out

    def _semantic(self, p2, p3, p4, p5, on_gpu=True):
        head = self.fcn_head
        fuse_up = on_gpu and head._f is not None and head.upsample_rate == 4
        if not fuse_up:
            return head(p2, p3, p4, p5)["fcn_output"].float(), None
        ret = head(p2, p3, p4, p5, score_only=not getattr(self, "keep_intermediates", False))
        score = ret["fcn_score"].float().contiguous()
        fo = ret.get("fcn_output")
        return (None if fo is None else fo.float()), score

    def _side_stream(self, dev, idx=0):
        key = (str(dev), idx, ops.WS_SLOT["i"])
        if key not in self._side:
            self._side[key] = torch.cuda.Stream(device=dev)
        return self._side[key]

    def _run_static(self, x, im_info, lane=0):
        prev_slot = ops.WS_SLOT["i"]
        ops.WS_SLOT["i"] = int(lane)
        try:
            return self._run_static_lane(x, im_info, int(lane))
        finally:
            ops.WS_SLOT["i"] = prev_slot

    def _run_static_lane(self, x, im_info, lane):
        if not (self.use_cuda_graph and x.is_cuda):
            return self._forward_static(x, im_info), None
        key = (tuple(x.shape), str(x.device), ops._PRECISION["conv"], bool(getattr(self, "keep_intermediates", False)),
               tuple(float(v) for v in im_info), lane)
        ent = self._graphs.get(key)
        if ent is None:
            static_x = torch.empty(x.shape, dtype=torch.float32, device=x.device)
            static_x.copy_(x)
            cur = torch.cuda.current_stream(x.device)
            side = torch.cuda.Stream(device=x.device)
            side.wait_stream(cur)
            with torch.cuda.stream(side):
                for _ in range(2):
                    self._forward_static(static_x, im_info)
            cur.wait_stream(side)
            torch.cuda.synchronize(x.device)
            graph = torch.cuda.CUDAGraph()
            l0 = ops.STATS["launches"]
            with torch.cuda.graph(graph):
                out = self._forward_static(static_x, im_info)
            ent = (graph, static_x, out, ops.STATS["launches"] - l0)
            while len(self._graphs) >= self.max_graphs:
                self._graphs.pop(next(iter(self._graphs)))
            self._graphs[key] = ent
        else:
            self._graphs[key] = self._graphs.pop(key)
        graph, static_x, out, n_launch = ent
        static_x.copy_(x, non_blocking=True)
        graph.replay()
        ops.STATS["launches"] += n_launch
        return out, graph

    @torch.no_grad()
    def forward(self, data, label=None):
        if label is not None:
            raise NotImplementedError("training forward (BASELINE config #4) is outside this round's scope")
        if not self._prepared:
            self.prepare()
        x = data["data"]
        im_info = np.asarray(data["im_info"], dtype=np.float32).reshape(-1, 3)
        assert x.shape[0] == 1 and im_info.shape[0] == 1, "one image per device (SURVEY F9)"
        if self.static_engine:
            out, graph = self._run_static(x, im_info[0])
            n1, n2, k = (int(v) for v in out["counts"].tolist())
            keep = out["keep"][:k]
            cp = (lambda t: t.clone()) if graph is not None else (lambda t: t)
            results = {"cls_probs": cp(out["cls_probs"][:n1]), "pred_boxes": cp(out["pred_boxes"][:n1]),
                       "mask_probs": cp(out["mask_probs"][:n1]), "cls_inds": cp(out["cls_inds"][:n1]),
                       "fcn_outputs": cp(out["fcn_outputs"]), "panoptic_cls_inds": out["p_cls"][:n2][keep],
                       "panoptic_cls_probs": out["p_scores"][:n2][keep], "panoptic_outputs": cp(out["panoptic_outputs"])}
            if getattr(self, "keep_intermediates", False):
                results["_intermediates"] = {"fcn_output": cp(out["fcn_output"]), "pmask_rois": cp(out["p_boxes"][:n2]),
                                             "pcls_prob": cp(out["p_scores"][:n2]),
                                             "pmask_score": cp(out["p_mask_score"][:n2]),
                                             "pcls_idx": cp(out["p_cls"][:n2]), "keep_inds": cp(keep)}
                for k_, v_ in out.get("dbg", {}).items():
                    results["_intermediates"][k_] = [cp(t_) for t_ in v_] if isinstance(v_, list) else cp(v_)
            return results
        res2, res3, res4, res5 = self.resnet_backbone(x)
        p2, p3, p4, p5, p6 = self.fpn(res2, res3, res4, res5)
        rpn_cls_prob, rpn_bbox_pred = [], []
        for feat in (p2, p3, p4, p5, p6):
            _, bbox, prob = self.rpn(feat)
            rpn_cls_prob.append(prob)
            rpn_bbox_pred.append(bbox)
        rois, _ = self.pyramid_proposal(rpn_cls_prob, rpn_bbox_pred, im_info[0])
        fcn_output = self.fcn_head(p2, p3, p4, p5)
        feats = [p2, p3, p4, p5]
        rcnn_output = self.rcnn(feats, rois)
        cls_prob = F.softmax(rcnn_output["cls_score"], dim=1)
        bbox_pred = rcnn_output["bbox_pred"]

        cls_prob_all, mask_rois, cls_idx = self.mask_roi(rois, bbox_pred, cls_prob, im_info[0])
        mask_prob = torch.sigmoid(self.mask_branch(feats, mask_rois))
        results = {"cls_probs": cls_prob_all, "pred_boxes": mask_rois, "mask_probs": mask_prob, "cls_inds": cls_idx}

        pcls_prob, pmask_rois, pcls_idx = self.mask_roi_panoptic(rois, bbox_pred, cls_prob, im_info[0])
        mask_score = self.mask_branch(feats, pmask_rois)
        ms = self.cfg.mask_size
        mask_score = mask_score.gather(1, pcls_idx.view(-1, 1, 1, 1).expand(-1, -1, ms, ms))
        pan = self.panoptic_head(fcn_output["fcn_output"], pmask_rois, pcls_prob, mask_score, pcls_idx, want_sem=True)
        keep = pan["keep_inds"]
        results.update({"fcn_outputs": pan["fcn_outputs"], "panoptic_cls_inds": pcls_idx[keep],
                        "panoptic_cls_probs": pcls_prob[keep], "panoptic_outputs": pan["panoptic_outputs"]})
        if getattr(self, "keep_intermediates", False):
            results["_intermediates"] = {"fcn_output": fcn_output["fcn_output"], "rois": rois, "cls_prob": cls_prob,
                                         "bbox_pred": bbox_pred, "pmask_rois": pmask_rois, "pcls_prob": pcls_prob,
                                         "pmask_score": mask_score, "pcls_idx": pcls_idx, "keep_inds": keep}
        return results


def resnet_50_upsnet(cfg=None):
    return resnet_upsnet([3, 4, 6, 3], cfg)


def resnet_101_upsnet(cfg=None):
    return resnet_upsnet([3, 4, 23, 3], cfg)
```

### upsnet_b200/operators.py

```python
import ctypes as C
import math

import numpy as np
import torch
import torch.nn as nn
from torch.nn.modules.utils import _pair
from torch.nn.parameter import Parameter

from . import _lib
from ._lib import check, f32c, lib, ptr, require_cuda, stream_ptr

_PRECISION = {"conv": _lib.PREC_FP32_SIMT}
DCN_WINDOW = {"on": True, "min_pixels": 4096}
USE_TMA = {"on": True}


def set_precision(name):
    _PRECISION["conv"] = {"fp32": _lib.PREC_FP32_SIMT, "bf16x3": _lib.PREC_BF16X3, "bf16": _lib.PREC_BF16}[name]


def _stream():
    return {_lib.PREC_BF16: "bf16", _lib.PREC_BF16X3: "pair"}.get(_PRECISION["conv"], "f32")


# ... 57 lines not shown

    def __init__(self, kind, n_kernels, work, device):
        self.kind, self.n, self.work, self.device = kind, n_kernels, work, device
        self.ev = None

    def __enter__(self):
        STATS["launches"] += self.n
        if STATS["trace"] is not None:
            self.ev = (torch.cuda.Event(enable_timing=True), torch.cuda.Event(enable_timing=True))
            self.ev[0].record(torch.cuda.current_stream(self.device))
        return self

    def __exit__(self, *exc):
        if self.ev is not None:
            self.ev[1].record(torch.cuda.current_stream(self.device))
            STATS["trace"].append((self.kind, self.ev[0], self.ev[1], self.work))
        return False


def _conv_out(n, pad, dil, k, stride):
    return (n + 2 * pad - (dil * (k - 1) + 1)) // stride + 1


def _nhwc(x):
    xp = x.permute(0, 2, 3, 1)
    return xp if xp.is_contiguous() else xp.contiguous()


import weakref


def _per_weight(cache, weight, make, device=None, versioned=True):
    hit = cache.get(id(weight))
    if (hit is not None and hit[0]() is weight and (not versioned or hit[1] == weight._version) and
            (device is None or hit[2] is None or hit[2].device == device)):
        return hit[2]
    value = make()
    wid = id(weight)
    cache[wid] = (weakref.ref(weight, lambda _r, _k=wid: cache.pop(_k, None)), weight._version, value)
    return value


_packed_cache = {}


def _packed_weight(weight):
    return _per_weight(_packed_cache, weight, lambda: _pack_igemm(weight), device=weight.device)


def _pack_igemm(weight):
    Cout, Cin, kh, kw = weight.shape
    nbytes = C.c_size_t(0)
    check(lib().upsnet_igemm_packed_weight_bytes(Cout, Cin, kh, kw, C.byref(nbytes)), "igemm_packed_weight_bytes")
    buf = torch.empty(nbytes.value, dtype=torch.uint8, device=weight.device)
    w = f32c(weight.detach())
    with torch.cuda.device(weight.device):
        check(lib().upsnet_igemm_pack_weight(ptr(w), Cout, Cin, kh, kw, ptr(buf), stream_ptr(weight.device)),
              "igemm_pack_weight")
    STATS["launches"] += 1
    return buf


_dcn_packed_cache = {}


def _packed_weight_dcn(weight):
    return _per_weight(_dcn_packed_cache, weight, lambda: _pack_dcn(weight), device=weight.device)


def _pack_dcn(weight):
    Cout, Cin, kh, kw = weight.shape
    nbytes = C.c_size_t(0)
    rc = lib().upsnet_dcn_packed_weight_bytes(Cout, Cin, kh, kw, C.byref(nbytes))
    buf = None
    if rc == 0:
        buf = torch.empty(nbytes.value, dtype=torch.uint8, device=weight.device)
        w = f32c(weight.detach())
        with torch.cuda.device(weight.device):
            check(lib().upsnet_dcn_pack_weight(ptr(w), Cout, Cin, kh, kw, ptr(buf), stream_ptr(weight.device)), "dcn_pack_weight")
        STATS["launches"] += 1
    elif rc != -2:
        check(rc, "dcn_packed_weight_bytes")
    return buf


def _dcn_window(x, offset, mask, weight, bias, padding, dilation, relu):
    N, Cin, H, W = x.shape
    if N * H * W < DCN_WINDOW["min_pixels"]:
        return None
    packed = _packed_weight_dcn(weight)
    if packed is None:
        return None
    Cout, _, kh, kw = weight.shape
    ph, pw = padding; dh, dw = dilation
    Ho, Wo = _conv_out(H, ph, dh, kh, 1), _conv_out(W, pw, dw, kw, 1)
    store = torch.empty((N, Ho, Wo, 2 * Cout), device=x.device, dtype=torch.bfloat16)
    work = {"flops": 2.0 * N * Ho * Wo * Cout * Cin * kh * kw * 3, "algo_flops": 2.0 * N * Ho * Wo * Cout * Cin * kh * kw,
            "shape": "N%d %dx%d Cin%d->Cout%d k%d s1 pair->pair (window)" % (N, H, W, Cin, Cout, kh),
            "bytes": float(x.store.numel() * 2 + 4 * weight.numel() + store.numel() * 2 + offset.numel() * 4)}
    with torch.cuda.device(x.device), _Timed("dcn", 1, work, x.device):
        rc = lib().upsnet_dcn_pair_forward(ptr(x.store), ptr(offset), ptr(mask), ptr(packed), ptr(bias), ptr(store), N, H, W,
                                           Cin, Cout, kh, kw, ph, pw, dh, dw, _lib.EPI_RELU if relu else 0, stream_ptr(x.device))
    if rc == -2:
        return None
    check(rc, "dcn_pair_forward")
    return Pair(store)


_stem_cache = {}
_stem_ws = None


def stem_conv(x, weight, bias, padding, relu=True, pair=False):
    global _stem_ws
    require_cuda(x, weight, bias)
    x = f32c(x)
    N, Cin, H, W = x.shape
    Cout, _, kh, kw = weight.shape
    dev = x.device

    def pack():
        nb = C.c_size_t(0)
        check(lib().upsnet_stem_packed_weight_bytes(Cout, kh, C.byref(nb)), "stem_packed_weight_bytes")
        packed = torch.empty(nb.value, dtype=torch.uint8, device=dev)
        with torch.cuda.device(dev):
            check(lib().upsnet_stem_pack_weight(ptr(f32c(weight.detach())), Cout, Cin, kh, kw, ptr(packed), stream_ptr(dev)),
                  "stem_pack_weight")
        STATS["launches"] += 1
        return packed

    packed = _per_weight(_stem_cache, weight, pack, device=dev)
    nb = C.c_size_t(0)
    check(lib().upsnet_stem_workspace_bytes(N, H, W, kh, kw, int(padding), C.byref(nb)), "stem_workspace_bytes")
    if _stem_ws is None:
        _stem_ws = _Workspace()
    ws = _stem_ws.get(dev, nb.value)
    Ho, Wo = (H + 2 * padding - kh) // 2 + 1, (W + 2 * padding - kw) // 2 + 1
    store = torch.empty((N, Ho, Wo, Cout * (2 if pair else 1)), dtype=torch.bfloat16, device=dev)
    fl = 2.0 * N * Ho * Wo * Cout * Cin * kh * kw
    work = {"flops": fl * (3 if pair else 1), "algo_flops": fl,
            "shape": "N%d %dx%d Cin%d->Cout%d k%d s2 float32->%s (stem, TMA)" % (N, H, W, Cin, Cout, kh, "pair" if pair else "bfloat16"),
            "bytes": float(4 * x.numel() + 2 * store.numel())}
    with torch.cuda.device(dev), _Timed("conv2d", 2, work, dev):
        check(lib().upsnet_stem_forward(ptr(x), ptr(packed), ptr(None if bias is None else f32c(bias)), ptr(store), N, Cin, H, W,
                                        Cout, kh, kw, int(padding), (_lib.EPI_RELU if relu else 0) | (_lib.EPI_STEM_PAIR if pair else 0),
                                        ptr(ws), ws.numel(), stream_ptr(dev)), "stem_forward")
    return Pair(store) if pair else store.permute(0, 3, 1, 2)


def _tc_ok(Cin, kh, kw, dg, deform=False):
    return (Cin % 64 == 0 or (Cin <= 8 and not deform)) and dg == 1 and kh * kw <= 49


def _igemm_tc(kind, x, offset, mask, weight, bias, residual, stride, padding, dilation, relu, prec, out_format,
              out_dtype=None, residual_up2=False, pair_group=0, sigmoid_from=None):
    sh, sw = stride; ph, pw = padding; dh, dw = dilation
    N, Cin, H, W = x.shape
    Cout, _, kh, kw = weight.shape
    Ho, Wo = _conv_out(H, ph, dh, kh, sh), _conv_out(W, pw, dw, kw, sw)
    nhwc_out = out_format != "nchw"
    x3 = prec == _lib.PREC_BF16X3
    stream = _stream()
    pair_in = isinstance(x, Pair)
    if pair_in:
        assert x3, "Pair activations belong to precision bf16x3"
    elif x3 and stream == "pair" and Cin % 64 == 0:
        x = Pair.from_float(x)
        pair_in = True
    elif x3 and x.dtype != torch.float32:
        x = x.float()
    elif x.dtype not in (torch.float32, torch.bfloat16):
        x = x.float()
    dev = x.device
    pair_out = False
    if out_dtype is None:
        if x3 and stream == "pair" and nhwc_out and Cout % 8 == 0:
            pair_out = True
        else:
            out_dtype = torch.bfloat16 if (stream == "bf16" and prec == _lib.PREC_BF16 and nhwc_out) else torch.float32
    elif out_dtype == "pair":
        pair_out = True
    if pair_in:
        xs, x_dt = x.store, _lib.DTYPE_PAIR
    else:
        xs = f32c(x) if Cin % 64 else _nhwc(x)
        x_dt = _lib.DTYPE_BF16 if xs.dtype == torch.bfloat16 else _lib.DTYPE_F32
    packed = _packed_weight(weight)
    if pair_out:
        assert nhwc_out
        store = torch.empty((N, Ho, Wo, 2 * Cout), device=dev, dtype=torch.bfloat16)
        res = None
        if residual is not None:
            res = (residual if isinstance(residual, Pair) else Pair.from_float(residual)).store
        y_dt = _lib.DTYPE_PAIR
    elif nhwc_out:
        store = torch.empty((N, Ho, Wo, Cout), device=dev, dtype=out_dtype)
        res = None if residual is None else _nhwc(as_float(residual).to(out_dtype))
        y_dt = _lib.DTYPE_BF16 if out_dtype == torch.bfloat16 else _lib.DTYPE_F32
    else:
        store = torch.empty((N, Cout, Ho, Wo), device=dev, dtype=out_dtype)
        res = None if residual is None else as_float(residual).to(out_dtype).contiguous()
        y_dt = _lib.DTYPE_BF16 if out_dtype == torch.bfloat16 else _lib.DTYPE_F32
    xbytes = xs.numel() * xs.element_size()
    work = {"flops": 2.0 * N * Ho * Wo * Cout * Cin * kh * kw * (3 if x3 else 1),
            "algo_flops": 2.0 * N * Ho * Wo * Cout * Cin * kh * kw,
            "shape": "N%d %dx%d Cin%d->Cout%d k%d s%d %s->%s%s" % (N, H, W, Cin, Cout, kh, sh, "pair" if pair_in else str(xs.dtype)[6:],
                                                              "pair" if pair_out else str(out_dtype)[6:],
                                                              " +res" if residual is not None else ""),
            "bytes": float(xbytes + 4 * weight.numel() +
                           store.numel() * store.element_size() * (2 if residual is not None else 1))}
    flags = (_lib.EPI_RELU if relu else 0) | (_lib.EPI_RES_UP2 if residual_up2 else 0) | \
            (0 if USE_TMA["on"] else _lib.EPI_NO_TMA)
    if pair_group:
        assert pair_out and pair_group % 64 == 0 and Cout % pair_group == 0
        flags |= (pair_group // 64) << 8
    if sigmoid_from is not None:
        assert not pair_out and not nhwc_out and residual is None, "sigmoid epilogue: fp32 NCHW head outputs"
        flags |= _lib.EPI_SIGMOID_FROM(sigmoid_from)
    with torch.cuda.device(dev), _Timed(kind, 1, work, dev):
        check(lib().upsnet_igemm_forward(ptr(xs), ptr(offset), ptr(mask), ptr(packed), ptr(bias), ptr(res),
                                         ptr(store), N, H, W, Cin, Cout, kh, kw, sh, sw, ph, pw, dh, dw,
                                         _lib.LAYOUT_NHWC if nhwc_out else _lib.LAYOUT_NCHW, x_dt, y_dt, flags,
                                         prec, stream_ptr(dev)), kind)
    if pair_out:
        if pair_group:
            return Pair(store.view(N, Ho, Wo * (Cout // pair_group), 2 * pair_group))
        return Pair(store)
    return store.permute(0, 3, 1, 2) if nhwc_out else store


def conv2d(x, weight, bias=None, stride=1, padding=0, dilation=1, residual=None, relu=False, precision=None,
           out_format=None, out_dtype=None, residual_up2=False, pair_group=0, sigmoid_from=None):
    require_cuda(x, weight, bias, residual)
    prec = _PRECISION["conv"] if precision is None else precision
    if prec != _lib.PREC_FP32_SIMT and _tc_ok(weight.shape[1], weight.shape[2], weight.shape[3], 1):
        if residual_up2 and out_format == "nchw":
            residual, residual_up2 = torch.nn.functional.interpolate(as_float(residual), scale_factor=2, mode="nearest"), False
        return _igemm_tc("conv2d", x, None, None, weight, None if bias is None else f32c(bias), residual,
                         _pair(stride), _pair(padding), _pair(dilation), relu, prec, out_format, out_dtype,
                         residual_up2, pair_group, sigmoid_from)
    if sigmoid_from is not None:
        y = conv2d(x, weight, bias, stride, padding, dilation, residual, relu, precision, out_format, out_dtype, residual_up2)
        y[:, sigmoid_from:] = torch.sigmoid(y[:, sigmoid_from:])
        return y
    if isinstance(x, Pair):
        x = x.float()
    if isinstance(residual, Pair):
        residual = residual.float()
    if residual_up2:
        residual = torch.nn.functional.interpolate(residual, scale_factor=2, mode="nearest")
    x, weight = f32c(x), f32c(weight)
    bias = None if bias is None else f32c(bias)
    residual = None if residual is None else f32c(residual)
    sh, sw = _pair(stride); ph, pw = _pair(padding); dh, dw = _pair(dilation)
    N, Cin, H, W = x.shape
    Cout, Cin_w, kh, kw = weight.shape
    assert Cin_w == Cin, "groups != 1 is not supported"
    Ho, Wo = _conv_out(H, ph, dh, kh, sh), _conv_out(W, pw, dw, kw, sw)
    y = torch.empty((N, Cout, Ho, Wo), device=x.device, dtype=torch.float32)
    if residual is not None:
        assert residual.shape == y.shape
    prec = _lib.PREC_FP32_SIMT
    work = {"flops": 2.0 * N * Ho * Wo * Cout * Cin * kh * kw, "algo_flops": 2.0 * N * Ho * Wo * Cout * Cin * kh * kw,
            "bytes": 4.0 * (x.numel() + weight.numel() + y.numel() * (2 if residual is not None else 1))}
    with torch.cuda.device(x.device), _Timed("conv2d_simt", 1, work, x.device):
        check(lib().upsnet_conv2d_forward(ptr(x), ptr(weight), ptr(bias), ptr(residual), ptr(y), N, Cin, H, W,
                                          Cout, kh, kw, sh, sw, ph, pw, dh, dw, _lib.EPI_RELU if relu else 0,
                                          prec, stream_ptr(x.device)), "conv2d")
    return y


def linear(x, weight, bias=None, relu=False, precision=None, out_dtype=None):
    if isinstance(x, Pair):
        y = conv2d(x, _as_1x1(weight), bias, relu=relu, precision=precision, out_dtype=out_dtype)
        return y if isinstance(y, Pair) else y.reshape(y.shape[0], weight.shape[0])
    N, K = x.shape
    y = conv2d(x.reshape(N, K, 1, 1), _as_1x1(weight), bias, relu=relu, precision=precision, out_dtype=out_dtype)
    return y if isinstance(y, Pair) else y.reshape(N, weight.shape[0])


_view_cache = {}


def _as_1x1(weight):
    return _per_weight(_view_cache, weight, lambda: weight.reshape(weight.shape[0], weight.shape[1], 1, 1), versioned=False)


def deform_conv(data, offset, weight, bias=None, stride=1, padding=0, dilation=1, deformable_groups=1,
                mask=None, relu=False, precision=None, out_format=None, out_dtype=None):
    require_cuda(data, offset, weight, bias, mask)
    prec = _PRECISION["conv"] if precision is None else precision
    use_tc = prec != _lib.PREC_FP32_SIMT and _tc_ok(weight.shape[1], weight.shape[2], weight.shape[3], deformable_groups, True)
    offset = f32c(offset)
    bias = None if bias is None else f32c(bias)
    mask = None if mask is None else f32c(mask)
    sh, sw = _pair(stride); ph, pw = _pair(padding); dh, dw = _pair(dilation)
    if use_tc:
        N, Cin, H, W = data.shape
        kh, kw = weight.shape[2], weight.shape[3]
        Ho, Wo = _conv_out(H, ph, dh, kh, sh), _conv_out(W, pw, dw, kw, sw)
        assert tuple(offset.shape) == (N, 2 * kh * kw, Ho, Wo), offset.shape
        if mask is not None:
            assert tuple(mask.shape) == (N, kh * kw, Ho, Wo), mask.shape
        if (DCN_WINDOW["on"] and isinstance(data, Pair) and prec == _lib.PREC_BF16X3 and (sh, sw) == (1, 1) and
                out_format != "nchw" and out_dtype in (None, "pair") and _stream() == "pair"):
            y = _dcn_window(data, offset, mask, weight, bias, (ph, pw), (dh, dw), relu)
            if y is not None:
                return y
        return _igemm_tc("dcn", data, offset, mask, weight, bias, None, (sh, sw), (ph, pw), (dh, dw), relu, prec,
                         out_format, out_dtype)
    data, weight = f32c(as_float(data)), f32c(weight)
    N, Cin, H, W = data.shape
    Cout, Cin_w, kh, kw = weight.shape
    assert Cin_w == Cin, "groups != 1 is not supported (the reference ignores `groups`)"
    Ho, Wo = _conv_out(H, ph, dh, kh, sh), _conv_out(W, pw, dw, kw, sw)
    assert tuple(offset.shape) == (N, 2 * kh * kw * deformable_groups, Ho, Wo), offset.shape
    if mask is not None:
        assert tuple(mask.shape) == (N, kh * kw * deformable_groups, Ho, Wo), mask.shape
    y = torch.empty((N, Cout, Ho, Wo), device=data.device, dtype=torch.float32)
    prec = _lib.PREC_FP32_SIMT
    work = {"flops": 2.0 * N * Ho * Wo * Cout * Cin * kh * kw, "algo_flops": 2.0 * N * Ho * Wo * Cout * Cin * kh * kw,
            "bytes": 4.0 * (data.numel() + offset.numel() + weight.numel() + y.numel() +
                            (mask.numel() if mask is not None else 0))}
    with torch.cuda.device(data.device), _Timed("dcn_simt", 1, work, data.device):
        check(lib().upsnet_dcn_forward(ptr(data), ptr(offset), ptr(mask), ptr(weight), ptr(bias), ptr(y), N, Cin,
                                       H, W, Cout, kh, kw, sh, sw, ph, pw, dh, dw, deformable_groups,
                                       _lib.EPI_RELU if relu else 0, prec, stream_ptr(data.device)),
              "deform_conv")
    return y


def roi_align(features, rois, pooled_height, pooled_width, spatial_scale, sampling_ratio=2, layout="nchw"):
    require_cuda(features, rois)
    features, rois = f32c(features), f32c(rois)
    assert rois.dim() == 2 and rois.shape[1] == 5
    R = rois.shape[0]
    if layout == "nchw":
        B, Cc, H, W = features.shape
        out = torch.empty((R, Cc, pooled_height, pooled_width), device=features.device, dtype=torch.float32)
        lay = _lib.LAYOUT_NCHW
    else:
        B, H, W, Cc = features.shape
        out = torch.empty((R, pooled_height, pooled_width, Cc), device=features.device, dtype=torch.float32)
        lay = _lib.LAYOUT_NHWC
    if R == 0:
        return out
    with torch.cuda.device(features.device), _Timed("roi_align", 1, {"bytes": 4.0 * out.numel()}, features.device):
        check(lib().upsnet_roi_align_forward(ptr(features), B, Cc, H, W, lay, 0, ptr(rois), R, pooled_height,
                                             pooled_width, sampling_ratio, float(spatial_scale), ptr(out),
                                             stream_ptr(features.device)), "roi_align")
    return out


def max_pool2d(x, kernel_size, stride, padding):
    require_cuda(x)
    N, Cc, H, W = x.shape
    Ho = (H + 2 * padding - kernel_size) // stride + 1
    Wo = (W + 2 * padding - kernel_size) // stride + 1
    if isinstance(x, Pair):
        store = torch.empty((N, Ho, Wo, 2 * Cc), device=x.device, dtype=torch.bfloat16)
        with torch.cuda.device(x.device), _Timed("maxpool", 1, {"bytes": float((x.store.numel() + store.numel()) * 2)}, x.device):
            check(lib().upsnet_maxpool2d_nhwc(ptr(x.store), ptr(store), N, H, W, Cc, kernel_size, stride, padding,
                                              _lib.DTYPE_PAIR, stream_ptr(x.device)), "maxpool2d")
        return Pair(store)
    if x.dtype not in (torch.float32, torch.bfloat16):
        x = x.float()
    xs = _nhwc(x)
    store = torch.empty((N, Ho, Wo, Cc), device=x.device, dtype=x.dtype)
    with torch.cuda.device(x.device), _Timed("maxpool", 1, {"bytes": float((xs.numel() + store.numel()) * x.element_size())}, x.device):
        check(lib().upsnet_maxpool2d_nhwc(ptr(xs), ptr(store), N, H, W, Cc, kernel_size, stride, padding,
                                          1 if x.dtype == torch.bfloat16 else 0, stream_ptr(x.device)), "maxpool2d")
    return store.permute(0, 3, 1, 2)


def upsample_bilinear(x, factor):
    require_cuda(x)
    x = f32c(x)
    N, Cc, H, W = x.shape
    y = torch.empty((N, Cc, H * factor, W * factor), dtype=torch.float32, device=x.device)
    with torch.cuda.device(x.device), _Timed("upsample", 1, {"bytes": 4.0 * (x.numel() + y.numel())}, x.device):
        check(lib().upsnet_upsample_bilinear_nchw(ptr(x), ptr(y), N * Cc, H, W, int(factor), stream_ptr(x.device)), "upsample")
    return y


def fcn_score_fuse(s2, s3, s4, s5):
    require_cuda(s2, s3, s4, s5)
    s2, s3, s4, s5 = f32c(s2), f32c(s3), f32c(s4), f32c(s5)
    N, Cc, H, W = s2.shape
    assert s3.shape == (N, Cc, H // 2, W // 2) and s4.shape == (N, Cc, H // 4, W // 4) and s5.shape == (N, Cc, H // 8, W // 8)
    out = torch.empty_like(s2)
    with torch.cuda.device(s2.device), _Timed("upsample", 1, {"bytes": 4.0 * (2 * s2.numel() + s3.numel() + s4.numel() + s5.numel())}, s2.device):
        check(lib().upsnet_fcn_score_fuse(ptr(s2), ptr(s3), ptr(s4), ptr(s5), ptr(out), N * Cc, H, W, stream_ptr(s2.device)),
              "fcn_score_fuse")
    return out


def fpn_roi_align(feats, rois, pooled_height, pooled_width, spatial_scales, sampling_ratio=2, layout="nchw",
                  return_levels=False):
    assert len(feats) == 4 and len(spatial_scales) == 4
    require_cuda(rois, *feats)
    rois = f32c(rois)
    R = rois.shape[0]
    if isinstance(feats[0], Pair):
        assert all(isinstance(f, Pair) for f in feats) and layout in ("auto", "nhwc", "flat_pair") and not return_levels
        B, Cc = feats[0].shape[0], feats[0].shape[1]
        flat = layout == "flat_pair"
        if flat:
            out = torch.empty((R, 1, 1, 2 * pooled_height * pooled_width * Cc), device=rois.device, dtype=torch.bfloat16)
        else:
            out = torch.empty((R, pooled_height, pooled_width, 2 * Cc), device=rois.device, dtype=torch.bfloat16)
        if R > 0:
            fp = (C.c_void_p * 4)(*[f.store.data_ptr() for f in feats])
            hs = (C.c_int * 4)(*[f.shape[2] for f in feats]); ws = (C.c_int * 4)(*[f.shape[3] for f in feats])
            sc = (C.c_float * 4)(*[float(s_) for s_ in spatial_scales])
            with torch.cuda.device(rois.device), _Timed("roi_align_fpn", 1, {"bytes": 2.0 * out.numel()}, rois.device):
                check(lib().upsnet_roi_align_fpn_forward(fp, hs, ws, sc, B, Cc, _lib.LAYOUT_FLAT_PAIR if flat else _lib.LAYOUT_NHWC,
                                                         _lib.DTYPE_PAIR, ptr(rois), R, pooled_height, pooled_width,
                                                         sampling_ratio, ptr(out), ptr(None), stream_ptr(rois.device)),
                      "fpn_roi_align")
        return Pair(out)
    if layout == "auto":
        cl = all(f.dim() == 4 and f.permute(0, 2, 3, 1).is_contiguous() and not f.is_contiguous() for f in feats)
        if cl:
            out = fpn_roi_align([f.permute(0, 2, 3, 1) for f in feats], rois, pooled_height, pooled_width,
                                spatial_scales, sampling_ratio, "nhwc", return_levels)
            return (out[0].permute(0, 3, 1, 2), out[1]) if return_levels else out.permute(0, 3, 1, 2)
        layout = "nchw"
    bf16 = layout == "nhwc" and all(f.dtype == torch.bfloat16 for f in feats)
    feats = [f.contiguous() for f in feats] if bf16 else [f32c(f) for f in feats]
    odt = torch.bfloat16 if bf16 else torch.float32
    if layout == "nchw":
        B, Cc = feats[0].shape[0], feats[0].shape[1]
        Hs = [f.shape[2] for f in feats]; Ws = [f.shape[3] for f in feats]
        out = torch.empty((R, Cc, pooled_height, pooled_width), device=rois.device, dtype=torch.float32)
        lay = _lib.LAYOUT_NCHW
    else:
        B, Cc = feats[0].shape[0], feats[0].shape[3]
        Hs = [f.shape[1] for f in feats]; Ws = [f.shape[2] for f in feats]
        out = torch.empty((R, pooled_height, pooled_width, Cc), device=rois.device, dtype=odt)
        lay = _lib.LAYOUT_NHWC
    levels = torch.empty((R,), device=rois.device, dtype=torch.int32) if return_levels else None
    fp = (C.c_void_p * 4)(*[f.data_ptr() for f in feats])
    hs = (C.c_int * 4)(*Hs); ws = (C.c_int * 4)(*Ws)
    sc = (C.c_float * 4)(*[float(s) for s in spatial_scales])
    with torch.cuda.device(rois.device), _Timed("roi_align_fpn", 1, {"bytes": 4.0 * out.numel()}, rois.device):
        check(lib().upsnet_roi_align_fpn_forward(fp, hs, ws, sc, B, Cc, lay, 1 if bf16 else 0, ptr(rois), R, pooled_height,
                                                 pooled_width, sampling_ratio, ptr(out), ptr(levels),
                                                 stream_ptr(rois.device)), "fpn_roi_align")
    return (out, levels) if return_levels else out


import threading


class _WsSlot(threading.local):
    i = 0

    def __getitem__(self, k):
        assert k == "i"
        return self.i

    def __setitem__(self, k, v):
        assert k == "i"
        self.i = int(v)


WS_SLOT = _WsSlot()


class _Workspace:

    def __init__(self):
        self.buf = {}
        self.retired = []

    def get(self, device, nbytes):
        key = (device, WS_SLOT["i"])
        b = self.buf.get(key)
        if b is None or b.numel() < nbytes:
            if b is not None:
                self.retired.append(b)
                nbytes = max(int(nbytes), int(b.numel() * 1.5))
            b = torch.empty(max(int(nbytes), 1), dtype=torch.uint8, device=device)
            self.buf[key] = b
        return b


_nms_ws = _Workspace()
_nms_ws_side = _Workspace()
_pan_ws = _Workspace()


def nms_segmented(boxes_sorted, seg_offsets, max_seg_len, thresh, side=False):
    require_cuda(boxes_sorted, seg_offsets)
    boxes_sorted = f32c(boxes_sorted)
    assert seg_offsets.dtype == torch.int32
    S = seg_offsets.numel() - 1
    dev = boxes_sorted.device
    nbytes = C.c_size_t(0)
    check(lib().upsnet_nms_workspace_bytes(S, max_seg_len, C.byref(nbytes)), "nms_workspace_bytes")
    ws = (_nms_ws_side if side else _nms_ws).get(dev, nbytes.value)
    keep = torch.empty((S, max_seg_len), dtype=torch.int32, device=dev)
    cnt = torch.empty((S,), dtype=torch.int32, device=dev)
    with torch.cuda.device(dev), _Timed("nms", 2, {"bytes": 20.0 * boxes_sorted.shape[0]}, dev):
        check(lib().upsnet_nms_segmented(ptr(boxes_sorted), ptr(seg_offsets), S, max_seg_len, float(thresh),
                                         ptr(keep), ptr(cnt), ptr(ws), ws.numel(), stream_ptr(dev)), "nms")
    return keep, cnt


def rpn_decode(bbox_preds, top_idx, shapes, strides, base_anchors, A, im_h, im_w):
    L = len(bbox_preds)
    dev = bbox_preds[0].device
    require_cuda(*bbox_preds, *top_idx, base_anchors)
    assert base_anchors.dtype == torch.float64 and base_anchors.is_contiguous()
    bbox_preds = [f32c(b) for b in bbox_preds]
    top_idx = [t.contiguous() for t in top_idx]
    assert all(t.dtype == torch.int64 for t in top_idx)
    ks = [int(t.numel()) for t in top_idx]
    out = torch.empty((sum(ks), 4), dtype=torch.float32, device=dev)
    vp, ci = C.c_void_p, C.c_int
    with torch.cuda.device(dev), _Timed("rpn_decode", 1, {"bytes": 56.0 * sum(ks)}, dev):
        check(lib().upsnet_rpn_decode((vp * L)(*[b.data_ptr() for b in bbox_preds]), (vp * L)(*[t.data_ptr() for t in top_idx]),
                                      (ci * L)(*ks), (ci * L)(*[int(s[0]) for s in shapes]), (ci * L)(*[int(s[1]) for s in shapes]),
                                      (ci * L)(*[int(s) for s in strides]), ptr(base_anchors), L, int(A), float(im_h), float(im_w),
                                      ptr(out), stream_ptr(dev)), "rpn_decode")
    return out


_topk_ws = None


def rpn_topk(probs, A, pre_nms_top_n):
    global _topk_ws
    L = len(probs)
    dev = probs[0].device
    require_cuda(*probs)
    probs = [f32c(pr) for pr in probs]
    ks = [min(int(pre_nms_top_n), int(pr.numel())) for pr in probs]
    out_s = torch.empty((sum(ks),), dtype=torch.float32, device=dev)
    out_i = torch.empty((sum(ks),), dtype=torch.int64, device=dev)
    if _topk_ws is None:
        _topk_ws = _Workspace()
    nbytes = C.c_size_t(0)
    check(lib().upsnet_rpn_topk_workspace_bytes(L, C.byref(nbytes)), "rpn_topk_workspace_bytes")
    ws = _topk_ws.get(dev, nbytes.value)
    vp, ci = C.c_void_p, C.c_int
    with torch.cuda.device(dev), _Timed("rpn_topk", 7, {"bytes": 4.0 * 6 * sum(pr.numel() for pr in probs)}, dev):
        check(lib().upsnet_rpn_topk((vp * L)(*[pr.data_ptr() for pr in probs]), (ci * L)(*[int(pr.shape[-2]) for pr in probs]),
                                    (ci * L)(*[int(pr.shape[-1]) for pr in probs]), L, int(A), int(pre_nms_top_n),
                                    ptr(out_s), ptr(out_i), ptr(ws), ws.numel(), stream_ptr(dev)), "rpn_topk")
    return out_s, out_i, ks


def rpn_collect(keep, cnt, offs, boxes, scores, post_nms_top_n):
    require_cuda(keep, cnt, offs, boxes, scores)
    dev = boxes.device
    S, M = keep.shape
    post = int(post_nms_top_n)
    rois = torch.empty((post, 5), dtype=torch.float32, device=dev)
    out_s = torch.empty((post,), dtype=torch.float32, device=dev)
    ok = torch.empty((post,), dtype=torch.bool, device=dev)
    with torch.cuda.device(dev), _Timed("rpn_collect", 1, {"bytes": 28.0 * post}, dev):
        check(lib().upsnet_rpn_collect(ptr(keep), ptr(cnt), ptr(offs), ptr(f32c(boxes)), ptr(f32c(scores)), S, M, post,
                                       ptr(rois), ptr(out_s), ptr(ok), stream_ptr(dev)), "rpn_collect")
    return rois, out_s, ok


def maskroi_prepare(rois, roi_valid, bbox_delta, cls_prob, class_agnostic, score_thresh, weights, im_h, im_w):
    require_cuda(rois, roi_valid, bbox_delta, cls_prob)
    rois, bbox_delta, cls_prob = f32c(rois), f32c(bbox_delta), f32c(cls_prob)
    assert roi_valid.dtype == torch.bool and roi_valid.is_contiguous()
    R, Cn = cls_prob.shape
    n = R * (Cn - 1)
    dev = rois.device
    nseg = 1 if class_agnostic else Cn - 1
    sc = torch.empty((n,), dtype=torch.float32, device=dev)
    cls = torch.empty((n,), dtype=torch.int32, device=dev)
    bx = torch.empty((n, 4), dtype=torch.float32, device=dev)
    offs = torch.empty((nseg + 1,), dtype=torch.int32, device=dev)
    w4 = (C.c_float * 4)(*[float(w) for w in weights])
    with torch.cuda.device(dev), _Timed("maskroi", 1, {"bytes": 4.0 * (rois.numel() + bbox_delta.numel() + cls_prob.numel())}, dev):
        check(lib().upsnet_maskroi_prepare(ptr(rois), ptr(roi_valid), ptr(bbox_delta), ptr(cls_prob), R, Cn,
                                           1 if class_agnostic else 0, float(score_thresh), w4, float(im_h), float(im_w),
                                           ptr(sc), ptr(cls), ptr(bx), ptr(offs), stream_ptr(dev)), "maskroi_prepare")
    return sc, cls, bx, offs


def maskroi_finish(keep, cnt, offs, sc, cls, bx, top_n, cap):
    require_cuda(keep, cnt, offs, sc, cls, bx)
    dev = sc.device
    nseg, M = keep.shape
    out_sc = torch.empty((cap,), dtype=torch.float32, device=dev)
    out_bx = torch.empty((cap, 5), dtype=torch.float32, device=dev)
    out_cls = torch.empty((cap,), dtype=torch.int64, device=dev)
    n_out = torch.empty((2,), dtype=torch.int32, device=dev)
    with torch.cuda.device(dev), _Timed("maskroi", 1, {"bytes": 32.0 * cap}, dev):
        check(lib().upsnet_maskroi_finish(ptr(keep), ptr(cnt), ptr(offs), ptr(sc), ptr(cls), ptr(bx), nseg, M, int(top_n),
                                          int(cap), ptr(out_sc), ptr(out_bx), ptr(out_cls), ptr(n_out), stream_ptr(dev)),
              "maskroi_finish")
    return out_sc, out_bx, out_cls, n_out[0], n_out[1]


def nms(boxes, scores, thresh):
    require_cuda(boxes, scores)
    n = boxes.shape[0]
    if n == 0:
        return torch.empty((0,), dtype=torch.int64, device=boxes.device)
    _, order = torch.sort(scores.float(), descending=True, stable=True)
    seg = torch.tensor([0, n], dtype=torch.int32, device=boxes.device)
    keep, cnt = nms_segmented(boxes.float()[order], seg, n, thresh)
    k = int(cnt.item())
    return order[keep[0, :k].long()]


def gpu_nms(dets, thresh, device_id=0):
    dets = np.ascontiguousarray(dets, dtype=np.float32)
    if dets.shape[0] == 0:
        return []
    d = torch.from_numpy(dets).to(torch.device("cuda", device_id))
    return nms(d[:, :4], d[:, 4], thresh).cpu().tolist()


def gpu_nms_wrapper(thresh, device_id):
    def _nms(dets):
        return gpu_nms(dets, thresh, device_id)
    return _nms


def _needs_grad(*tensors):
    return torch.is_grad_enabled() and any(isinstance(t, torch.Tensor) and t.requires_grad for t in tensors)


def _check_dg_for_grad(deformable_groups):
    if deformable_groups != 1:
        raise NotImplementedError("DeformConv / ModDeformConv backward supports deformable_groups=1 only (got %d); run "
                                  "the forward under torch.no_grad() or with parameters that do not require grad"
                                  % deformable_groups)


class DeformConv(nn.Module):

    def __init__(self, in_channels, out_channels, kernel_size, stride=1, padding=0, dilation=1, groups=1,
                 deformable_groups=1, bias=True):
        super().__init__()
        assert in_channels % groups == 0, 'in_channels must be divisible by groups'
        assert out_channels % groups == 0, 'out_channels must be divisible by groups'
        assert out_channels % deformable_groups == 0, 'out_channels must be divisible by deformable groups'
        self.in_channels, self.out_channels = in_channels, out_channels
        self.kernel_size, self.stride = _pair(kernel_size), _pair(stride)
        self.padding, self.dilation = _pair(padding), _pair(dilation)
        self.groups, self.deformable_groups = groups, deformable_groups
        dev = torch.device("cuda") if torch.cuda.is_available() else torch.device("cpu")
        self.weight = Parameter(torch.empty(out_channels, in_channels // groups, *self.kernel_size, device=dev))
        if bias:
            self.bias = Parameter(torch.empty(out_channels, device=dev))
        else:
            self.register_parameter('bias', None)
        self.reset_parameters()

    def reset_parameters(self):
        n = self.in_channels
        for k in self.kernel_size:
            n *= k
        stdv = 1. / math.sqrt(n)
        self.weight.data.uniform_(-stdv, stdv)
        if self.bias is not None:
            self.bias.data.uniform_(-stdv, stdv)

    def forward(self, data, offset):
        if _needs_grad(data, offset, self.weight, self.bias):
            _check_dg_for_grad(self.deformable_groups)
            from .training import DeformConvFunction
            return DeformConvFunction.apply(data, offset, self.weight, self.bias, self.stride, self.padding, self.dilation)
        return deform_conv(data, offset, self.weight, self.bias, self.stride, self.padding, self.dilation,
                           self.deformable_groups)


class DeformConvWithOffset(nn.Module):

    def __init__(self, in_channels, out_channels, kernel_size, stride=1, padding=0, dilation=1, groups=1,
                 deformable_groups=1, bias=True):
        super().__init__()
        self.conv_offset = nn.Conv2d(in_channels, kernel_size * kernel_size * 2 * deformable_groups,
                                     kernel_size=3, stride=1, padding=1)
        self.conv_offset.weight.data.zero_()
        self.conv_offset.bias.data.zero_()
        self.conv = DeformConv(in_channels, out_channels, kernel_size=kernel_size, stride=stride,
                               padding=padding, dilation=dilation, groups=groups,
                               deformable_groups=deformable_groups, bias=bias)

    def forward(self, x):
        if _needs_grad(x, self.conv_offset.weight, self.conv_offset.bias):
            from .training import OffsetConvFunction
            return self.conv(x, OffsetConvFunction.apply(x, self.conv_offset.weight, self.conv_offset.bias))
        offset = conv2d(x, self.conv_offset.weight, self.conv_offset.bias, 1, 1, 1, out_format="nchw")
        return self.conv(x, offset)


class ModDeformConv(DeformConv):

    def forward(self, data, offset_mask):
        offset_1, offset_2, mask = torch.chunk(offset_mask, 3, dim=1)
        offset = torch.cat((offset_1, offset_2), dim=1)
        mask = torch.sigmoid(mask) * 2
        if _needs_grad(data, offset_mask, self.weight, self.bias):
            _check_dg_for_grad(self.deformable_groups)
            from .training import ModDeformConvFunction
            return ModDeformConvFunction.apply(data, offset, mask, self.weight, self.bias, self.stride, self.padding, self.dilation)
        return deform_conv(data, offset, self.weight, self.bias, self.stride, self.padding, self.dilation,
                           self.deformable_groups, mask=mask)


ModulatedDeformConv = ModDeformConv


class ModDeformConvWithOffsetMask(nn.Module):

    def __init__(self, in_channels, out_channels, kernel_size, stride=1, padding=0, dilation=1, groups=1,
                 deformable_groups=1, bias=True):
        super().__init__()
        self.conv_offset_mask = nn.Conv2d(in_channels, kernel_size * kernel_size * 3 * deformable_groups,
                                          kernel_size=3, stride=1, padding=1)
        self.conv_offset_mask.weight.data.zero_()
        self.conv_offset_mask.bias.data.zero_()
        self.conv = ModDeformConv(in_channels, out_channels, kernel_size=kernel_size, stride=stride,
                                  padding=padding, dilation=dilation, groups=groups,
                                  deformable_groups=deformable_groups, bias=bias)

    def forward(self, x):
        if _needs_grad(x, self.conv_offset_mask.weight, self.conv_offset_mask.bias):
            from .training import OffsetConvFunction
            return self.conv(x, OffsetConvFunction.apply(x, self.conv_offset_mask.weight, self.conv_offset_mask.bias))
        om = conv2d(x, self.conv_offset_mask.weight, self.conv_offset_mask.bias, 1, 1, 1, out_format="nchw")
        return self.conv(x, om)


class RoIAlignFunction:

    def __init__(self, pooled_height, pooled_width, spatial_scale, sampling_ratio=2):
        self.pooled_width, self.pooled_height = int(pooled_width), int(pooled_height)
        self.spatial_scale, self.sampling_ratio = float(spatial_scale), sampling_ratio

    def __call__(self, features, rois):
        if not features.is_cuda:
            raise Exception('not implemented')
        if torch.is_grad_enabled() and features.requires_grad:
            from .training import RoIAlignFunction as _F
            return _F.apply(features, rois, self.pooled_height, self.pooled_width, self.spatial_scale, self.sampling_ratio)
        return roi_align(features, rois, self.pooled_height, self.pooled_width, self.spatial_scale,
                         self.sampling_ratio)


class RoIAlign(nn.Module):
# ... 430 lines not shown
```

Before: 117.2.

## Deduplicate mask-branch ROIs and bound mask convs by device-side row count

Adds a single-block kernel that merges the detection and panoptic box lists into a compact row set, dropping panoptic boxes that exactly match detection boxes and recording where each panoptic box maps. The mask branch ROI align and implicit-GEMM convolutions now read a device-side count so that blocks and tiles beyond the valid rows exit early, instead of processing the full padded capacity of both lists. This removes redundant mask-head work on padding and duplicates while keeping the CUDA graph static. It adds a serial O(n1*n2) comparison kernel, an index_select gather, and the device count is read inside the persistent GEMM scheduler.

New measurement: 126.8, median of 6. 8.2% higher.

```diff
diff --git a/include/upsnet_b200.h b/include/upsnet_b200.h
--- a/include/upsnet_b200.h
+++ b/include/upsnet_b200.h
@@ -40,7 +40,7 @@
 int upsnet_roi_align_fpn_forward(const void *const feats[4], const int Hs[4], const int Ws[4],
                                  const float scales[4], int B, int C, int layout, int dtype,
                                  const float *rois, int R, int PH, int PW, int sampling_ratio,
-                                 void *out, int *levels_out, void *stream);
+                                 void *out, int *levels_out, const int *n_dev, void *stream);
 
 int upsnet_nms_workspace_bytes(int S, int max_seg_len, size_t *bytes);
 int upsnet_nms_segmented(const float *boxes, const int *seg_offsets, int S, int max_seg_len,
@@ -68,7 +68,7 @@
                          const void *packed, const float *bias, const void *residual, void *y,
                          int N, int H, int W, int Cin, int Cout, int kh, int kw, int stride_h,
                          int stride_w, int pad_h, int pad_w, int dil_h, int dil_w, int out_layout,
-                         int x_dtype, int y_dtype, int epi_flags, int precision, void *stream);
+                         int x_dtype, int y_dtype, int epi_flags, int precision, const int *n_dev, void *stream);
 int upsnet_tma_set_tile_n(int bn);
 
 int upsnet_dcn_packed_weight_bytes(int Cout, int Cin, int kh, int kw, size_t *bytes);
@@ -134,6 +134,9 @@
 int upsnet_maskroi_finish(const int *keep, const int *keep_cnt, const int *seg_offsets, const float *sc,
                           const int *cls, const float *bx, int nseg, int max_seg_len, int top_n, int cap,
                           float *out_sc, float *out_bx, long long *out_cls, int *n_out, void *stream);
+
+int upsnet_mask_rows(const float *b1, const int *n1, int cap1, const float *b2, const int *n2, int cap2, float *rows,
+                     int *u, int *pan_row, void *stream);
 
 int upsnet_unified_pan_workspace_bytes(int num_seg_classes, size_t *bytes);
 int upsnet_unified_pan_result(const long long *seg, const long long *pan, const long long *cls_inds, int k,
diff --git a/upsnet_b200/_lib.py b/upsnet_b200/_lib.py
--- a/upsnet_b200/_lib.py
+++ b/upsnet_b200/_lib.py
@@ -38,7 +38,7 @@
         L.upsnet_version.argtypes = [C.POINTER(i)]
         L.upsnet_roi_align_forward.argtypes = [vp, i, i, i, i, i, i, vp, i, i, i, i, f, vp, vp]
         L.upsnet_roi_align_fpn_forward.argtypes = [C.POINTER(vp), C.POINTER(i), C.POINTER(i), C.POINTER(f),
-                                                   i, i, i, i, vp, i, i, i, i, vp, vp, vp]
+                                                   i, i, i, i, vp, i, i, i, i, vp, vp, vp, vp]
         L.upsnet_nms_workspace_bytes.argtypes = [i, i, C.POINTER(sz)]
         L.upsnet_nms_segmented.argtypes = [vp, vp, i, i, f, vp, vp, vp, sz, vp]
         L.upsnet_nms_host.argtypes = [vp, vp, vp, i, i, f, i]
@@ -46,7 +46,7 @@
         L.upsnet_conv2d_forward.argtypes = [vp] * 5 + [i] * 15 + [vp]
         L.upsnet_igemm_packed_weight_bytes.argtypes = [i, i, i, i, C.POINTER(sz)]
         L.upsnet_igemm_pack_weight.argtypes = [vp, i, i, i, i, vp, vp]
-        L.upsnet_igemm_forward.argtypes = [vp] * 7 + [i] * 18 + [vp]
+        L.upsnet_igemm_forward.argtypes = [vp] * 7 + [i] * 18 + [vp, vp]
         L.upsnet_dcn_packed_weight_bytes.argtypes = [i, i, i, i, C.POINTER(sz)]
         L.upsnet_dcn_pack_weight.argtypes = [vp, i, i, i, i, vp, vp]
         L.upsnet_dcn_pair_forward.argtypes = [vp] * 6 + [i] * 12 + [vp]
@@ -61,6 +61,7 @@
                                         C.POINTER(i), vp, i, i, f, f, vp, vp]
         L.upsnet_maskroi_prepare.argtypes = [vp, vp, vp, vp, i, i, i, f, C.POINTER(f), f, f, vp, vp, vp, vp, vp]
         L.upsnet_maskroi_finish.argtypes = [vp] * 6 + [i] * 4 + [vp] * 5
+        L.upsnet_mask_rows.argtypes = [vp, vp, i, vp, vp, i, vp, vp, vp, vp]
         L.upsnet_maxpool2d_nhwc.argtypes = [vp, vp] + [i] * 8 + [vp]
         L.upsnet_upsample_bilinear_nchw.argtypes = [vp, vp, i, i, i, i, vp]
         L.upsnet_rpn_topk_workspace_bytes.argtypes = [i, C.POINTER(sz)]
@@ -100,7 +101,7 @@
     "upsnet_nms_workspace_bytes", "upsnet_nms_segmented", "upsnet_nms_host", "upsnet_dcn_forward",
     "upsnet_conv2d_forward", "upsnet_igemm_packed_weight_bytes", "upsnet_igemm_pack_weight",
     "upsnet_igemm_forward", "upsnet_panoptic_workspace_bytes", "upsnet_panoptic_workspace_min_bytes", "upsnet_panoptic_head", "upsnet_panoptic_head_up4", "upsnet_mask_removal",
-    "upsnet_rpn_decode", "upsnet_maskroi_prepare", "upsnet_maskroi_finish", "upsnet_maxpool2d_nhwc", "upsnet_upsample_bilinear_nchw", "upsnet_rpn_topk_workspace_bytes", "upsnet_rpn_topk", "upsnet_rpn_collect", "upsnet_stem_workspace_bytes",
+    "upsnet_rpn_decode", "upsnet_maskroi_prepare", "upsnet_maskroi_finish", "upsnet_mask_rows", "upsnet_maxpool2d_nhwc", "upsnet_upsample_bilinear_nchw", "upsnet_rpn_topk_workspace_bytes", "upsnet_rpn_topk", "upsnet_rpn_collect", "upsnet_stem_workspace_bytes",
     "upsnet_stem_packed_weight_bytes", "upsnet_stem_pack_weight", "upsnet_stem_forward",
     "upsnet_dcn_im2col", "upsnet_dcn_col2im", "upsnet_dcn_col2im_coord", "upsnet_roi_align_backward",
     "upsnet_dcn_packed_weight_bytes", "upsnet_dcn_pack_weight", "upsnet_dcn_pair_forward", "upsnet_dcn_set_tile_n", "upsnet_tma_set_tile_n",
diff --git a/upsnet_b200/csrc/capi.cu b/upsnet_b200/csrc/capi.cu
--- a/upsnet_b200/csrc/capi.cu
+++ b/upsnet_b200/csrc/capi.cu
@@ -90,7 +90,7 @@
                                     void* y, int N, int H, int W, int Cin, int Cout, int kh, int kw,
                                     int stride_h, int stride_w, int pad_h, int pad_w, int dil_h,
                                     int dil_w, int out_layout, int x_dtype, int y_dtype, int epi_flags,
-                                    int precision, void* stream) {
+                                    int precision, const int* n_dev, void* stream) {
   if (!x_nhwc || !packed || !y) return UPSNET_E_BADARG;
   if (N <= 0 || Cin <= 0 || H <= 0 || W <= 0 || Cout <= 0 || kh <= 0 || kw <= 0 || stride_h <= 0 ||
       stride_w <= 0 || pad_h < 0 || pad_w < 0 || dil_h <= 0 || dil_w <= 0)
@@ -101,6 +101,7 @@
   if ((size_t)H * W >= (1ull << 31)) return UPSNET_E_UNSUPPORTED;
   ups::TcParams p{};
   p.x = x_nhwc; p.offset = offset; p.mask = mask; p.bias = bias; p.residual = residual; p.y = y;
+  p.n_dev = n_dev;
   p.N = N; p.H = H; p.W = W; p.Cin = Cin; p.Cout = Cout; p.kh = kh; p.kw = kw; p.sh = stride_h;
   p.sw = stride_w; p.ph = pad_h; p.pw = pad_w; p.dh = dil_h; p.dw = dil_w;
   p.Ho = ups::conv_out_size(H, pad_h, dil_h, kh, stride_h);
diff --git a/upsnet_b200/csrc/detection.cu b/upsnet_b200/csrc/detection.cu
--- a/upsnet_b200/csrc/detection.cu
+++ b/upsnet_b200/csrc/detection.cu
@@ -649,3 +649,63 @@
   UPS_CHECK_LAUNCH();
   return 0;
 }
+
+namespace ups {
+
+constexpr int kRowThreads = 128;
+
+__global__ void __launch_bounds__(kRowThreads)
+mask_rows_kernel(const float* __restrict__ b1, const int* __restrict__ n1p, int cap1, const float* __restrict__ b2,
+                 const int* __restrict__ n2p, int cap2, float* __restrict__ rows, int* __restrict__ u_out,
+                 int* __restrict__ pan_row) {
+  __shared__ int s_cnt[kRowThreads / 32];
+  const int n1 = min(max(*n1p, 0), cap1), n2 = min(max(*n2p, 0), cap2);
+  const int tid = threadIdx.x, lane = tid & 31, warp = tid >> 5;
+  const uint32_t* d = reinterpret_cast<const uint32_t*>(b1);
+  for (int k = tid; k < n1 * 5; k += kRowThreads) rows[k] = b1[k];
+  int base = n1;
+  for (int j0 = 0; j0 < cap2; j0 += kRowThreads) {
+    const int j = j0 + tid;
+    int src = 0;
+    bool fresh = false;
+    if (j < n2) {
+      const uint32_t* c = reinterpret_cast<const uint32_t*>(b2) + (size_t)j * 5;
+      const uint32_t c0 = c[0], c1 = c[1], c2 = c[2], c3 = c[3], c4 = c[4];
+      src = -1;
+      for (int i = 0; i < n1; ++i) {
+        const uint32_t* e = d + (size_t)i * 5;
+        if (e[0] == c0 && e[1] == c1 && e[2] == c2 && e[3] == c3 && e[4] == c4) { src = i; break; }
+      }
+      fresh = src < 0;
+    }
+    const unsigned bal = __ballot_sync(0xffffffffu, fresh);
+    if (lane == 0) s_cnt[warp] = __popc(bal);
+    __syncthreads();
+    int off = base, tot = 0;
+#pragma unroll
+    for (int w = 0; w < kRowThreads / 32; ++w) {
+      if (w < warp) off += s_cnt[w];
+      tot += s_cnt[w];
+    }
+    if (fresh) {
+      src = off + __popc(bal & ((1u << lane) - 1u));
+      for (int k = 0; k < 5; ++k) rows[(size_t)src * 5 + k] = b2[(size_t)j * 5 + k];
+    }
+    if (j < cap2) pan_row[j] = src;
+    base += tot;
+    __syncthreads();
+  }
+  for (int k = base * 5 + tid; k < (cap1 + cap2) * 5; k += kRowThreads) rows[k] = 0.f;
+  if (tid == 0) *u_out = base;
+}
+
+}
+
+extern "C" int upsnet_mask_rows(const float* b1, const int* n1, int cap1, const float* b2, const int* n2, int cap2,
+                                float* rows, int* u, int* pan_row, void* stream) {
+  if (!b1 || !n1 || !b2 || !n2 || !rows || !u || !pan_row || cap1 <= 0 || cap2 <= 0) return UPSNET_E_BADARG;
+  if ((long long)cap1 + cap2 > (1 << 20)) return UPSNET_E_UNSUPPORTED;
+  ups::mask_rows_kernel<<<1, ups::kRowThreads, 0, (cudaStream_t)stream>>>(b1, n1, cap1, b2, n2, cap2, rows, u, pan_row);
+  UPS_CHECK_LAUNCH();
+  return 0;
+}
diff --git a/upsnet_b200/csrc/igemm_tma.cu b/upsnet_b200/csrc/igemm_tma.cu
--- a/upsnet_b200/csrc/igemm_tma.cu
+++ b/upsnet_b200/csrc/igemm_tma.cu
@@ -21,6 +21,7 @@
   int kw, KHW, ph, pw, dh, dw;
   int bw, bh, bn;
   int tiles_w, tiles_h, tiles_n, n_tiles;
+  const int* n_dev;
   int BN, stages, relu, has_res;
   int res_up2;
   int direct, y_bf16, out_nhwc;
@@ -107,7 +108,8 @@
   const int tid = threadIdx.x, warp = tid >> 5, lane = tid & 31;
   const int cchunks = g.Cin / 64;
   const int num_kb = g.KHW * cchunks;
-  const long long m_tiles = (long long)g.tiles_w * g.tiles_h * g.tiles_n;
+  const int tiles_n = g.n_dev ? (min(max(*g.n_dev, 0), g.N) + g.bn - 1) / g.bn : g.tiles_n;
+  const long long m_tiles = (long long)g.tiles_w * g.tiles_h * tiles_n;
   const long long num_tiles = m_tiles * g.n_tiles;
   const uint32_t box_bytes = (uint32_t)(g.bw * g.bh * g.bn) * 128u;
 
@@ -535,6 +537,7 @@
   g.N = p.N; g.Ho = p.Ho; g.Wo = p.Wo; g.Cout = p.Cout; g.Cin = p.Cin;
   g.kw = p.kw; g.KHW = p.kh * p.kw; g.ph = p.ph; g.pw = p.pw; g.dh = p.dh; g.dw = p.dw;
   g.relu = p.relu; g.has_res = p.residual ? 1 : 0; g.res_up2 = p.res_up2 ? 1 : 0; g.sig_from = p.sig_from;
+  g.n_dev = p.n_dev;
   tma_pick_box(p.N, p.Ho, p.Wo, p.kh, p.kw, p.dh, p.dw, g.res_up2 != 0, &g.bw, &g.bh, &g.bn);
   g.tiles_w = (p.Wo + g.bw - 1) / g.bw;
   g.tiles_h = (p.Ho + g.bh - 1) / g.bh;
diff --git a/upsnet_b200/csrc/roi_align.cu b/upsnet_b200/csrc/roi_align.cu
--- a/upsnet_b200/csrc/roi_align.cu
+++ b/upsnet_b200/csrc/roi_align.cu
@@ -249,10 +249,11 @@
 __global__ void __launch_bounds__(256)
 roi_align_nhwc_pair_roi_kernel(FpnFeats f, int C, const float* __restrict__ rois, int R, int PH, int PW, int sr,
                                __nv_bfloat16* __restrict__ out, long long roi_stride, int pix_stride, long long lo_off,
-                               int* __restrict__ levels_out) {
+                               int* __restrict__ levels_out, const int* __restrict__ n_dev) {
   __shared__ int4 s_off[kRoiMaxSamples];
   __shared__ float4 s_w[kRoiMaxSamples];
   const int n = blockIdx.x;
+  if (n_dev && n >= *n_dev) return;
   const float* r = rois + (size_t)n * 5;
   const int b = (int)roundf(r[0]);
   const float rx1 = r[1], ry1 = r[2], rx2 = r[3], ry2 = r[4];
@@ -323,10 +324,11 @@
 }
 
 static int launch_roi_align(const FpnFeats& f, int B, int C, int layout, int dtype, const float* rois, int R,
-                            int PH, int PW, int sr, void* out_v, int* levels_out,
+                            int PH, int PW, int sr, void* out_v, int* levels_out, const int* n_dev,
                             cudaStream_t stream) {
   if (R < 0 || C <= 0 || PH <= 0 || PW <= 0 || B <= 0) return UPSNET_E_BADARG;
   if (R == 0) return 0;
+  if (n_dev && dtype != UPSNET_DTYPE_PAIR) return UPSNET_E_UNSUPPORTED;
   if (dtype == UPSNET_DTYPE_PAIR) {
     if (layout != UPSNET_LAYOUT_NHWC && layout != UPSNET_LAYOUT_FLAT_PAIR) return UPSNET_E_UNSUPPORTED;
     if (sr <= 0 || (C & 7) || (long long)PH * PW * sr * sr > kRoiMaxSamples || (((uintptr_t)out_v) & 15)) return UPSNET_E_UNSUPPORTED;
@@ -335,7 +337,7 @@
     const long long plane = (long long)PH * PW * C;
     const bool flat = layout == UPSNET_LAYOUT_FLAT_PAIR;
     roi_align_nhwc_pair_roi_kernel<<<R, 256, 0, stream>>>(f, C, rois, R, PH, PW, sr, (__nv_bfloat16*)out_v, 2 * plane,
-                                                          flat ? C : 2 * C, flat ? plane : (long long)C, levels_out);
+                                                          flat ? C : 2 * C, flat ? plane : (long long)C, levels_out, n_dev);
     UPS_CHECK_LAUNCH();
     return 0;
   }
@@ -392,7 +394,7 @@
   if (!feat || !out || (!rois && R > 0)) return UPSNET_E_BADARG;
   ups::FpnFeats f{};
   f.p[0] = feat; f.H[0] = H; f.W[0] = W; f.scale[0] = spatial_scale; f.nlevels = 1;
-  return ups::launch_roi_align(f, B, C, layout, dtype, rois, R, PH, PW, sampling_ratio, out, nullptr,
+  return ups::launch_roi_align(f, B, C, layout, dtype, rois, R, PH, PW, sampling_ratio, out, nullptr, nullptr,
                                (cudaStream_t)stream);
 }
 
@@ -400,7 +402,7 @@
                                             const int Ws[4], const float scales[4], int B, int C,
                                             int layout, int dtype, const float* rois, int R, int PH, int PW,
                                             int sampling_ratio, void* out, int* levels_out,
-                                            void* stream) {
+                                            const int* n_dev, void* stream) {
   if (!feats || !Hs || !Ws || !scales || !out || (!rois && R > 0)) return UPSNET_E_BADARG;
   ups::FpnFeats f{};
   for (int l = 0; l < 4; ++l) {
@@ -408,6 +410,6 @@
     f.p[l] = feats[l]; f.H[l] = Hs[l]; f.W[l] = Ws[l]; f.scale[l] = scales[l];
   }
   f.nlevels = 4;
-  return ups::launch_roi_align(f, B, C, layout, dtype, rois, R, PH, PW, sampling_ratio, out, levels_out,
+  return ups::launch_roi_align(f, B, C, layout, dtype, rois, R, PH, PW, sampling_ratio, out, levels_out, n_dev,
                                (cudaStream_t)stream);
 }
diff --git a/upsnet_b200/csrc/tc_params.cuh b/upsnet_b200/csrc/tc_params.cuh
--- a/upsnet_b200/csrc/tc_params.cuh
+++ b/upsnet_b200/csrc/tc_params.cuh
@@ -43,6 +43,7 @@
   int res_up2;
   int no_tma;
   int tile_w, tile_h;
+  const int* n_dev;
 };
 
 size_t tc_packed_weight_bytes(int Cout, int Cin, int kh, int kw);
diff --git a/upsnet_b200/model.py b/upsnet_b200/model.py
--- a/upsnet_b200/model.py
+++ b/upsnet_b200/model.py
@@ -315,31 +315,37 @@
         b1 = self.mask_deconv1[0].bias.repeat(4).detach().contiguous()
         self._f = (w1, b1, cout)
 
-    def forward(self, feat, rois):
-        x = self.roi_pooling(feat, rois)
+    def forward(self, feat, rois, n_dev=None):
+        bound = {} if n_dev is None else {"n_dev": n_dev}
+        if n_dev is None or not isinstance(feat[0], ops.Pair):
+            x = self.roi_pooling(feat, rois)
+        else:
+            r = self.roi_pooling
+            x = ops.fpn_roi_align(list(feat), rois, r.pooled_height, r.pooled_width, r.spatial_scale, layout="auto", **bound)
         for i in range(1, 5):
             c = getattr(self, "mask_conv%d" % i)[0]
-            x = ops.conv2d(x, c.weight, c.bias, padding=1, relu=True)
+            x = ops.conv2d(x, c.weight, c.bias, padding=1, relu=True, **bound)
         w1, b1, cout = self._f
         if isinstance(x, ops.Pair):
-            yv = ops.conv2d(x, w1, b1, relu=True, pair_group=cout)
+            yv = ops.conv2d(x, w1, b1, relu=True, pair_group=cout, **bound)
             n, _, h, w4 = yv.shape
             w = w4 // 4
-            z = ops.conv2d(yv, self.mask_score.weight, self.mask_score.bias, out_format="nhwc", out_dtype=torch.float32)
+            z = ops.conv2d(yv, self.mask_score.weight, self.mask_score.bias, out_format="nhwc", out_dtype=torch.float32,
+                           **bound)
             K = z.shape[1]
             z = z.permute(0, 2, 3, 1).reshape(n, h, w, 2, 2, K)
             return z.permute(0, 5, 1, 3, 2, 4).reshape(n, K, 2 * h, 2 * w)
-        y = ops.conv2d(x, w1, b1, relu=True)
+        y = ops.conv2d(x, w1, b1, relu=True, **bound)
         n, _, h, w = y.shape
         if y.is_contiguous(memory_format=torch.channels_last) and y.dim() == 4:
             yv = y.permute(0, 2, 3, 1).reshape(n, h, w * 4, cout).permute(0, 3, 1, 2)
             z = ops.conv2d(yv, self.mask_score.weight, self.mask_score.bias, out_format="nhwc",
-                           out_dtype=torch.float32)
+                           out_dtype=torch.float32, **bound)
             K = z.shape[1]
             z = z.permute(0, 2, 3, 1).reshape(n, h, w, 2, 2, K)
             return z.permute(0, 5, 1, 3, 2, 4).reshape(n, K, 2 * h, 2 * w)
         y = y.reshape(n, 2, 2, cout, h, w).permute(0, 3, 4, 1, 5, 2).reshape(n, cout, 2 * h, 2 * w)
-        return ops.conv2d(y, self.mask_score.weight, self.mask_score.bias, out_format="nchw")
+        return ops.conv2d(y, self.mask_score.weight, self.mask_score.bias, out_format="nchw", **bound)
 
 
 class FCNSubNet(nn.Module):
@@ -476,6 +482,7 @@
         self.static_engine = True
         self.use_cuda_graph = True
         self.overlap_heads = True
+        self.dedup_mask_rows = True
         self._side = {}
         self._graphs = {}
         self.max_graphs = 6
@@ -609,10 +616,16 @@
             cur.wait_event(done2)
         else:
             s2, b2, c2, n2 = self.mask_roi_panoptic_static(rois, roi_valid, bbox_pred, cls_prob, im_info)
-        logits = self.mask_branch(feats, torch.cat([b1, b2], 0)).float()
+        ms = self.cfg.mask_size
+        if self.dedup_mask_rows and x.is_cuda:
+            rows, u, pan_row = ops.mask_rows(b1, n1, b2, n2)
+            logits = self.mask_branch(feats, rows, n_dev=u).float()
+            K = logits.shape[1]
+            mask_score = logits.view(-1, ms, ms).index_select(0, pan_row.long() * K + c2).view(-1, 1, ms, ms)
+        else:
+            logits = self.mask_branch(feats, torch.cat([b1, b2], 0)).float()
+            mask_score = logits[b1.shape[0]:].gather(1, c2.view(-1, 1, 1, 1).expand(-1, -1, ms, ms))
         mask_prob = torch.sigmoid(logits[:b1.shape[0]])
-        ms = self.cfg.mask_size
-        mask_score = logits[b1.shape[0]:].gather(1, c2.view(-1, 1, 1, 1).expand(-1, -1, ms, ms))
         if fork:
             cur.wait_event(done)
         keep, labels, sem, k = ops.panoptic_fuse(fcn_score if fcn_score is not None else fcn_output, b2[:, 1:], s2, mask_score, c2,
@@ -659,7 +672,7 @@
         if not (self.use_cuda_graph and x.is_cuda):
             return self._forward_static(x, im_info), None
         key = (tuple(x.shape), str(x.device), ops._PRECISION["conv"], bool(getattr(self, "keep_intermediates", False)),
-               tuple(float(v) for v in im_info), lane)
+               bool(self.dedup_mask_rows), tuple(float(v) for v in im_info), lane)
         ent = self._graphs.get(key)
         if ent is None:
             static_x = torch.empty(x.shape, dtype=torch.float32, device=x.device)
diff --git a/upsnet_b200/operators.py b/upsnet_b200/operators.py
--- a/upsnet_b200/operators.py
+++ b/upsnet_b200/operators.py
@@ -233,8 +233,14 @@
     return (Cin % 64 == 0 or (Cin <= 8 and not deform)) and dg == 1 and kh * kw <= 49
 
 
+def _count(n_dev):
+    if n_dev is not None:
+        assert n_dev.dtype == torch.int32 and n_dev.is_cuda and n_dev.numel() == 1
+    return n_dev
+
+
 def _igemm_tc(kind, x, offset, mask, weight, bias, residual, stride, padding, dilation, relu, prec, out_format,
-              out_dtype=None, residual_up2=False, pair_group=0, sigmoid_from=None):
+              out_dtype=None, residual_up2=False, pair_group=0, sigmoid_from=None, n_dev=None):
     sh, sw = stride; ph, pw = padding; dh, dw = dilation
     N, Cin, H, W = x.shape
     Cout, _, kh, kw = weight.shape
@@ -302,7 +308,7 @@
         check(lib().upsnet_igemm_forward(ptr(xs), ptr(offset), ptr(mask), ptr(packed), ptr(bias), ptr(res),
                                          ptr(store), N, H, W, Cin, Cout, kh, kw, sh, sw, ph, pw, dh, dw,
                                          _lib.LAYOUT_NHWC if nhwc_out else _lib.LAYOUT_NCHW, x_dt, y_dt, flags,
-                                         prec, stream_ptr(dev)), kind)
+                                         prec, ptr(_count(n_dev)), stream_ptr(dev)), kind)
     if pair_out:
         if pair_group:
             return Pair(store.view(N, Ho, Wo * (Cout // pair_group), 2 * pair_group))
@@ -311,7 +317,7 @@
 
 
 def conv2d(x, weight, bias=None, stride=1, padding=0, dilation=1, residual=None, relu=False, precision=None,
-           out_format=None, out_dtype=None, residual_up2=False, pair_group=0, sigmoid_from=None):
+           out_format=None, out_dtype=None, residual_up2=False, pair_group=0, sigmoid_from=None, n_dev=None):
     require_cuda(x, weight, bias, residual)
     prec = _PRECISION["conv"] if precision is None else precision
     if prec != _lib.PREC_FP32_SIMT and _tc_ok(weight.shape[1], weight.shape[2], weight.shape[3], 1):
@@ -319,7 +325,7 @@
             residual, residual_up2 = torch.nn.functional.interpolate(as_float(residual), scale_factor=2, mode="nearest"), False
         return _igemm_tc("conv2d", x, None, None, weight, None if bias is None else f32c(bias), residual,
                          _pair(stride), _pair(padding), _pair(dilation), relu, prec, out_format, out_dtype,
-                         residual_up2, pair_group, sigmoid_from)
+                         residual_up2, pair_group, sigmoid_from, n_dev)
     if sigmoid_from is not None:
         y = conv2d(x, weight, bias, stride, padding, dilation, residual, relu, precision, out_format, out_dtype, residual_up2)
         y[:, sigmoid_from:] = torch.sigmoid(y[:, sigmoid_from:])
@@ -477,7 +483,7 @@
 
 
 def fpn_roi_align(feats, rois, pooled_height, pooled_width, spatial_scales, sampling_ratio=2, layout="nchw",
-                  return_levels=False):
+                  return_levels=False, n_dev=None):
     assert len(feats) == 4 and len(spatial_scales) == 4
     require_cuda(rois, *feats)
     rois = f32c(rois)
@@ -497,7 +503,8 @@
             with torch.cuda.device(rois.device), _Timed("roi_align_fpn", 1, {"bytes": 2.0 * out.numel()}, rois.device):
                 check(lib().upsnet_roi_align_fpn_forward(fp, hs, ws, sc, B, Cc, _lib.LAYOUT_FLAT_PAIR if flat else _lib.LAYOUT_NHWC,
                                                          _lib.DTYPE_PAIR, ptr(rois), R, pooled_height, pooled_width,
-                                                         sampling_ratio, ptr(out), ptr(None), stream_ptr(rois.device)),
+                                                         sampling_ratio, ptr(out), ptr(None), ptr(_count(n_dev)),
+                                                         stream_ptr(rois.device)),
                       "fpn_roi_align")
         return Pair(out)
     if layout == "auto":
@@ -520,13 +527,14 @@
         Hs = [f.shape[1] for f in feats]; Ws = [f.shape[2] for f in feats]
         out = torch.empty((R, pooled_height, pooled_width, Cc), device=rois.device, dtype=odt)
         lay = _lib.LAYOUT_NHWC
+    assert n_dev is None, "fpn_roi_align: the roi count bound is implemented for pair features"
     levels = torch.empty((R,), device=rois.device, dtype=torch.int32) if return_levels else None
     fp = (C.c_void_p * 4)(*[f.data_ptr() for f in feats])
     hs = (C.c_int * 4)(*Hs); ws = (C.c_int * 4)(*Ws)
     sc = (C.c_float * 4)(*[float(s) for s in spatial_scales])
     with torch.cuda.device(rois.device), _Timed("roi_align_fpn", 1, {"bytes": 4.0 * out.numel()}, rois.device):
         check(lib().upsnet_roi_align_fpn_forward(fp, hs, ws, sc, B, Cc, lay, 1 if bf16 else 0, ptr(rois), R, pooled_height,
-                                                 pooled_width, sampling_ratio, ptr(out), ptr(levels),
+                                                 pooled_width, sampling_ratio, ptr(out), ptr(levels), ptr(None),
                                                  stream_ptr(rois.device)), "fpn_roi_align")
     return (out, levels) if return_levels else out
 
@@ -680,6 +688,20 @@
                                           int(cap), ptr(out_sc), ptr(out_bx), ptr(out_cls), ptr(n_out), stream_ptr(dev)),
               "maskroi_finish")
     return out_sc, out_bx, out_cls, n_out[0], n_out[1]
+
+
+def mask_rows(b1, n1, b2, n2):
+    require_cuda(b1, n1, b2, n2)
+    dev = b1.device
+    cap1, cap2 = b1.shape[0], b2.shape[0]
+    b1, b2 = f32c(b1), f32c(b2)
+    rows = torch.empty((cap1 + cap2, 5), dtype=torch.float32, device=dev)
+    u = torch.empty((), dtype=torch.int32, device=dev)
+    pan_row = torch.empty((cap2,), dtype=torch.int32, device=dev)
+    with torch.cuda.device(dev), _Timed("maskroi", 1, {"bytes": 40.0 * (cap1 + cap2)}, dev):
+        check(lib().upsnet_mask_rows(ptr(b1), ptr(_count(n1)), cap1, ptr(b2), ptr(_count(n2)), cap2, ptr(rows), ptr(u),
+                                     ptr(pan_row), stream_ptr(dev)), "mask_rows")
+    return rows, u, pan_row
 
 
 def nms(boxes, scores, thresh):
```
